# Huzo/Distributed-Machine-Learning-using-CNN-CIFAR-10-dataset-

Measured on AMD Instinct MI355X. Metric: images/sec (whole node) CIFAR-10 CNN training at 1/2/4/8 MI355X, higher is better.
Workload: dtype bf16; 1 GPU; global_batch=256, per_gpu_batch=256, parallelism=dp1, impl=fused+hipgraph, comm_dtype=bf16, graph_warmup_steps=256, steps_per_graph=32

## Files before the change

csrc/bindings/torch_ops.cpp:

```cpp
#include <torch/extension.h>
#include <c10/hip/HIPStream.h>
#include <c10/hip/HIPGuard.h>

#include <vector>

#include "../kernels/api.h"
#include "../kernels/api_comm.h"
#include "check.h"

namespace {

using namespace dmlc_bind;

uint8_t* xraw_ptr(const c10::optional<Tensor>& xraw, int64_t B) {
  if (!xraw.has_value()) return nullptr;
  check(*xraw, "xraw", at::kByte, {B, 3072});
  return xraw->data_ptr<uint8_t>();
}


void conv1_fwd(const Tensor& data, const Tensor& idx, const c10::optional<Tensor>& counter, int64_t period,
               int64_t cy, int64_t cx, const Tensor& w1f, const Tensor& b1, const Tensor& out, const Tensor& am,
               const c10::optional<Tensor>& amax, const c10::optional<Tensor>& xraw) {
  const int64_t B = out.size(0);
// ... 316 lines not shown
      TORCH_CHECK(P.ksplit == 1 && P.nvalid == P.N && P.N % 4 == 0 && P.ldc % 4 == 0 && !P.bias && !P.relu,
                  "gemm ", i, ": the fused SGD epilogue needs ksplit 1, full 16-B rows, no bias / ReLU");
      TORCH_CHECK(!bias.get(i).has_value(), "gemm ", i, ": the fused SGD epilogue takes no bias");
      check_min(*shadow, "shadow", at::kBFloat16, P.s_par + (int64_t)P.M * P.ldc);
      P.S = shadow->data_ptr();
      G.lr0 = (float)sched[0]; G.decay = (float)sched[1]; G.decay_steps = (float)sched[2];
      G.staircase = sched[3] != 0.0; G.warmup = (float)sched[4]; G.grad_scale = (float)sched[5];
    }
    P.A = A[i].data_ptr(); P.B = Bm[i].data_ptr(); P.C = C[i].data_ptr();
    P.bias = nullptr;
    const c10::optional<Tensor> bo = bias.get(i);
    if (bo.has_value()) {
      check_min(*bo, "bias", at::kFloat, P.nvalid);
      P.bias = bo->data_ptr<float>();
    }
  }
  for (int i = 0; i < n; ++i) {
    if (G.p[i].c_mode == 3) { G.p[i].A = A[i].data_ptr(); G.p[i].C = C[i].data_ptr(); G.p[i].bias = nullptr; }
  }
  c10::DeviceGuard guard(A[0].device());
  CHECK_HIP(dmlc_gemm_grouped(&G, stream_of(A[0])));
}

void head(const Tensor& h1part, const Tensor& b1, const Tensor& w2t, const Tensor& b2, const Tensor& w3t,
          const Tensor& b3, const Tensor& w3d, const Tensor& w2d, const Tensor& labels, const Tensor& idx,
          const c10::optional<Tensor>& counter, int64_t period, double inv_batch, bool relu_logits, bool train,
          const Tensor& h1, const Tensor& h2, const Tensor& dl, const Tensor& dh1, const Tensor& dh2,
          const Tensor& loss_part, const Tensor& correct_part, const c10::optional<Tensor>& logits_out,
          int64_t nvalid, const c10::optional<Tensor>& step, const c10::optional<Tensor>& step_copy) {
  TORCH_CHECK(h1part.dim() == 3 && h1part.size(2) == 384, "h1part must be [nsplit,B,384]");
  const int64_t nsplit = h1part.size(0), B = h1part.size(1);
  TORCH_CHECK(B % 16 == 0 && B > 0, "head: batch must be a positive multiple of 16");
  TORCH_CHECK(loss_part.numel() >= 1 && B % loss_part.numel() == 0, "head: loss partials must divide the batch");
  const int64_t rows = B / loss_part.numel();
  TORCH_CHECK(rows == 2 || rows == 4, "head: B / loss_part.numel() (rows per workgroup) must be 2 or 4");
  check(h1part, "h1part", at::kFloat, {nsplit, B, 384});
  check_numel(b1, "b1", at::kFloat, 384);
  check(w2t, "w2t", at::kBFloat16, {192, 384});
  check_numel(b2, "b2", at::kFloat, 192);
  check(w3t, "w3t", at::kBFloat16, {16, 192});
  check_numel(b3, "b3", at::kFloat, 10);
  check(w3d, "w3d", at::kBFloat16, {192, 32});
  check(w2d, "w2d", at::kBFloat16, {384, 192});
  dev(labels, "labels");
  TORCH_CHECK(labels.scalar_type() == at::kInt && labels.dim() == 1, "labels must be int32 [N]");
  check(loss_part, "loss_part", at::kFloat, {B / rows});
  check(correct_part, "correct_part", at::kInt, {B / rows});
  if (train) {
    check(h1, "h1", at::kBFloat16, {B, 384});
    check(h2, "h2", at::kBFloat16, {B, 192});
    check(dl, "dl", at::kBFloat16, {B, 16});
    check(dh1, "dh1", at::kBFloat16, {B, 384});
    check(dh2, "dh2", at::kBFloat16, {B, 192});
  }
  c10::DeviceGuard guard(h1part.device());
  DmlcHeadArgs a;
  a.h1part = h1part.data_ptr<float>(); a.nsplit = (int)nsplit;
  a.b1 = b1.data_ptr<float>(); a.w2t = w2t.data_ptr(); a.b2 = b2.data_ptr<float>();
  a.w3t = w3t.data_ptr(); a.b3 = b3.data_ptr<float>(); a.w3d = w3d.data_ptr(); a.w2d = w2d.data_ptr();
  a.labels = labels.data_ptr<int>(); a.src = index_src(idx, counter, period, B);
  check_order_fits(a.src, labels.size(0));
  if (nvalid < 0) nvalid = B;
  TORCH_CHECK(nvalid >= 1 && nvalid <= B, "head: nvalid must be in [1, B]");
  a.nvalid = (int)nvalid;
  a.B = (int)B; a.rows = (int)rows; a.inv_batch = (float)inv_batch; a.relu_logits = relu_logits; a.train = train;
  a.h1 = train ? h1.data_ptr() : nullptr; a.h2 = train ? h2.data_ptr() : nullptr; a.dl = train ? dl.data_ptr() : nullptr;
  a.dh1 = train ? dh1.data_ptr() : nullptr; a.dh2 = train ? dh2.data_ptr() : nullptr;
  a.loss_part = loss_part.data_ptr<float>(); a.correct_part = correct_part.data_ptr<int>();
  a.logits_out = nullptr;
  if (logits_out.has_value()) {
    check(*logits_out, "logits_out", at::kFloat, {B, 10});
    a.logits_out = logits_out->data_ptr<float>();
  }
  a.step = nullptr; a.step_copy = nullptr;
  TORCH_CHECK(step.has_value() == step_copy.has_value(), "head: step and step_copy go together");
  if (step.has_value()) {
    check_numel(*step, "step", at::kLong, 1);
    check_numel(*step_copy, "step_copy", at::kLong, 1);
    a.step = step->data_ptr<int64_t>(); a.step_copy = step_copy->data_ptr<int64_t>();
  }
  CHECK_HIP(dmlc_head(&a, stream_of(h1part)));
}

void fc_chain(const Tensor& p2, const Tensor& fc1n, const Tensor& h1part, const Tensor& b1, const Tensor& w2t,
              const Tensor& b2, const Tensor& w3t, const Tensor& b3, const Tensor& w3d, const Tensor& labels,
              const Tensor& idx, const c10::optional<Tensor>& counter, int64_t period, double inv_batch,
              bool relu_logits, const Tensor& h1, const Tensor& h2, const Tensor& dl, const Tensor& dh1,
              const Tensor& dh2, const Tensor& loss_part, const Tensor& correct_part, const Tensor& dp2,
              const Tensor& gw1, const Tensor& gw2, const Tensor& gw3, const Tensor& gb1, const Tensor& gb2,
              const Tensor& gb3, bool fuse_sgd, at::ArrayRef<double> sched, int64_t nvalid, const Tensor& step,
              const c10::optional<Tensor>& step_copy, const Tensor& sync, const Tensor& err, bool dw_tasks,
              const c10::optional<Tensor>& am2, const c10::optional<Tensor>& w2d, const c10::optional<Tensor>& dp1,
              const c10::optional<Tensor>& dy2, const c10::optional<Tensor>& fc2n) {
  const int64_t B = p2.size(0);
  TORCH_CHECK(B >= 16 && B <= 256 && B % 16 == 0, "fc_chain: batch must be a multiple of 16 in [16, 256]");
  check(p2, "p2", at::kBFloat16, {B, 2304});
  check(fc1n, "fc1n", at::kBFloat16, {2, 2304, 384});
  check(h1part, "h1part", at::kFloat, {8, B, 384});
  check_numel(b1, "b1", at::kFloat, 384);
  check(w2t, "w2t", at::kBFloat16, {192, 384});
  check_numel(b2, "b2", at::kFloat, 192);
  check(w3t, "w3t", at::kBFloat16, {16, 192});
  check_numel(b3, "b3", at::kFloat, 10);
  check(w3d, "w3d", at::kBFloat16, {192, 32});
  dev(labels, "labels");
  TORCH_CHECK(labels.scalar_type() == at::kInt && labels.dim() == 1, "labels must be int32 [N]");
  check(h1, "h1", at::kBFloat16, {B, 384});
  check(h2, "h2", at::kBFloat16, {B, 192});
  check(dl, "dl", at::kBFloat16, {B, 16});
  check(dh1, "dh1", at::kBFloat16, {B, 384});
  check(dh2, "dh2", at::kBFloat16, {B, 192});
  check(loss_part, "loss_part", at::kFloat, {B / 4});
  check(correct_part, "correct_part", at::kInt, {B / 4});
  check(dp2, "dp2", at::kBFloat16, {B, 2304});
  const bool g16 = gw1.scalar_type() == at::kBFloat16;
  TORCH_CHECK(!g16 || !fuse_sgd, "fc_chain: bf16 gradient views only without the fused SGD");
  const auto gt = g16 ? at::kBFloat16 : at::kFloat;
  check_numel(gw1, "gw1", gt, 2304 * 384);
  check_numel(gw2, "gw2", gt, 384 * 192);
  check_numel(gw3, "gw3", gt, 192 * 10);
  check_numel(gb1, "gb1", gt, 384);
  check_numel(gb2, "gb2", gt, 192);
  check_numel(gb3, "gb3", gt, 10);
  check_numel(step, "step", at::kLong, 1);
  check_min(sync, "sync", at::kInt, 212 * 32);
  check_min(err, "err", at::kInt, 1);
  TORCH_CHECK(sched.size() == 6, "fc_chain: sched = {lr0, decay, decay_steps, staircase, warmup, grad_scale}");
  if (nvalid < 0) nvalid = B;
  TORCH_CHECK(nvalid >= 1 && nvalid <= B, "fc_chain: nvalid must be in [1, B]");
  c10::DeviceGuard guard(p2.device());
  DmlcFcArgs a;
  memset(&a, 0, sizeof(a));
  a.B = (int)B; a.nvalid = (int)nvalid; a.mtiles = (int)((B + 63) / 64);
  a.p2 = p2.data_ptr(); a.w1 = fc1n.data_ptr(); a.h1part = h1part.data_ptr<float>();
  a.b1 = b1.data_ptr<float>(); a.w2t = w2t.data_ptr(); a.b2 = b2.data_ptr<float>();
  a.w3t = w3t.data_ptr(); a.b3 = b3.data_ptr<float>(); a.w3d = w3d.data_ptr();
  a.labels = labels.data_ptr<int>(); a.src = index_src(idx, counter, period, B);
  check_order_fits(a.src, labels.size(0));
  a.inv_batch = (float)inv_batch; a.relu_logits = relu_logits;
  a.h1 = h1.data_ptr(); a.h2 = h2.data_ptr(); a.dl = dl.data_ptr(); a.dh1 = dh1.data_ptr(); a.dh2 = dh2.data_ptr();
  a.loss_part = loss_part.data_ptr<float>(); a.correct_part = correct_part.data_ptr<int>();
  a.dp2 = dp2.data_ptr();
  a.gw1 = (float*)gw1.data_ptr(); a.gw2 = (float*)gw2.data_ptr(); a.gw3 = (float*)gw3.data_ptr();
  a.gb1 = (float*)gb1.data_ptr(); a.gb2 = (float*)gb2.data_ptr(); a.gb3 = (float*)gb3.data_ptr();
  a.grad_bf16 = g16 ? 1 : 0;
  a.fuse_sgd = fuse_sgd ? 1 : 0;
  a.dw_tasks = dw_tasks ? 1 : 0;
  if (fc2n.has_value()) {
    TORCH_CHECK(fuse_sgd && dw_tasks, "fc_chain: the fc SGD in the chain needs fuse_sgd and the dW tiles");
    check(*fc2n, "fc2n", at::kBFloat16, {384, 192});
    a.fuse_sgd = 2;
    a.mw2 = gw2.data_ptr<float>(); a.mw3 = gw3.data_ptr<float>();
    a.mb1 = gb1.data_ptr<float>(); a.mb2 = gb2.data_ptr<float>(); a.mb3 = gb3.data_ptr<float>();
    a.fc2n = fc2n->data_ptr(); a.fc2t = w2t.data_ptr(); a.fc3t = w3t.data_ptr(); a.fc3d = w3d.data_ptr();
  }
  a.lr0 = (float)sched[0]; a.decay = (float)sched[1]; a.decay_steps = (float)sched[2];
  a.staircase = sched[3] != 0.0; a.warmup = (float)sched[4]; a.grad_scale = (float)sched[5];
  a.step = step.data_ptr<int64_t>();
  a.step_copy = nullptr;
  if (step_copy.has_value()) {
    check_numel(*step_copy, "step_copy", at::kLong, 1);
    a.step_copy = step_copy->data_ptr<int64_t>();
  }
  a.sync = reinterpret_cast<unsigned int*>(sync.data_ptr<int>());
  a.err = reinterpret_cast<unsigned int*>(err.data_ptr<int>());
  const bool dg_on = am2.has_value();
  TORCH_CHECK(dg_on == w2d.has_value() && dg_on == dp1.has_value() && dg_on == dy2.has_value(),
              "fc_chain: am2, w2d, dp1, dy2 come together");
  DmlcConv2DgradArgs g;
  memset(&g, 0, sizeof(g));
  if (dg_on) {
    check(*am2, "am2", at::kByte, {B, 6, 6, 64});
    check(*w2d, "w2d", at::kBFloat16, {64, 1600});
    check(*dp1, "dp1", at::kBFloat16, {B, 12, 12, 64});
    check(*dy2, "dy2", at::kBFloat16, {B, 144, 64});
    g.dp2 = dp2.data_ptr(); g.am2 = am2->data_ptr<uint8_t>(); g.wd = w2d->data_ptr();
    g.dp1 = dp1->data_ptr(); g.dy2 = dy2->data_ptr(); g.B = (int)B;
    g.split = B <= 128 ? 1 : 0;
  }
  CHECK_HIP(dmlc_fc_chain(&a, dg_on ? &g : nullptr, stream_of(p2)));
}

static DmlcSgdArgs make_sgd(const Tensor& master, const Tensor& grad, int64_t mode, double grad_scale, at::IntArrayRef off,
         const Tensor& part1, const Tensor& partb1, const Tensor& part2, const Tensor& partb2, const Tensor& w1f,
         const Tensor& w2f, const Tensor& w2d, const Tensor& fc1n, const Tensor& fc2t, const Tensor& fc2n,
         const Tensor& fc3t, const Tensor& fc3d, const Tensor& step, double lr0, double decay, double decay_steps,
         bool staircase, const Tensor& ticket, const Tensor& loss_part, const Tensor& correct_part,
         const Tensor& stats, const c10::optional<Tensor>& w2f8, const c10::optional<Tensor>& amax_w,
         const c10::optional<Tensor>& scale_w, int64_t roles, bool finalize, int64_t batch,
         const c10::optional<Tensor>& bidx, const c10::optional<Tensor>& order, double warmup, bool fc1_fused,
         const c10::optional<Tensor>& step_rd, const c10::optional<Tensor>& xnext,
         const c10::optional<Tensor>& xdata) {
  TORCH_CHECK(roles >= 0 && roles <= 2, "sgd roles must be 0..2");
  TORCH_CHECK(warmup >= 0.0, "sgd: warmup must be >= 0");
  TORCH_CHECK(mode >= 0 && mode <= 3, "sgd mode must be 0..3");
  TORCH_CHECK(off.size() == 10, "off must have 10 entries");
  static const int64_t numel[10] = {4800, 64, 102400, 64, 884736, 384, 73728, 192, 1920, 10};
  for (int i = 0; i < 10; ++i) {
    TORCH_CHECK(off[i] >= 0 && (i == 0 || off[i] >= off[i - 1] + numel[i - 1]), "bad param offsets");
  }
  const int64_t end = off[9] + 10;
  check_min(master, "master", at::kFloat, end);
  const bool g16 = grad.scalar_type() == at::kBFloat16;
  check_min(grad, "grad", g16 ? at::kBFloat16 : at::kFloat, end);
  TORCH_CHECK(!g16 || mode == 1 || mode == 2, "sgd: a bf16 gradient only in modes 1 / 2 (data parallel)");
  const int64_t g1 = part1.size(0), g2 = part2.size(0);
  check(part1, "part1", at::kFloat, {g1, 80, 64});
  check(partb1, "partb1", at::kFloat, {g1, 64});
  check(part2, "part2", at::kFloat, {g2, 1600, 64});
  check(partb2, "partb2", at::kFloat, {g2, 64});
  TORCH_CHECK(loss_part.numel() >= 1, "loss partials missing");
  const int64_t B = batch;
  TORCH_CHECK(B >= 1 && B <= 4 * loss_part.numel(), "sgd: batch (valid rows) exceeds the head's rows");
  check(w1f, "w1f", at::kBFloat16, {64, 96});
  check(w2f, "w2f", at::kBFloat16, {64, 1600});
  check(w2d, "w2d", at::kBFloat16, {64, 1600});
  check(fc1n, "fc1n", at::kBFloat16, {2, 2304, 384});
  TORCH_CHECK(!fc1_fused || mode == 0, "sgd: fc1_fused only in mode 0 (single GPU)");
  check(fc2t, "fc2t", at::kBFloat16, {192, 384});
  check(fc2n, "fc2n", at::kBFloat16, {384, 192});
  check(fc3t, "fc3t", at::kBFloat16, {16, 192});
  check(fc3d, "fc3d", at::kBFloat16, {192, 32});
  check_numel(step, "step", at::kLong, 1);
  check_numel(ticket, "ticket", at::kInt, DMLC_TICKET_WORDS);
  dev(loss_part, "loss_part"); dev(correct_part, "correct_part");
  TORCH_CHECK(loss_part.scalar_type() == at::kFloat && correct_part.scalar_type() == at::kInt &&
                  loss_part.numel() == correct_part.numel(), "loss/correct partials mismatch");
  dev(stats, "stats");
  TORCH_CHECK(stats.scalar_type() == at::kFloat && stats.dim() == 2 && stats.size(1) == 4, "stats must be [R,4] fp32");
  DmlcSgdArgs a;
  a.master = master.data_ptr<float>();
  a.grad = g16 ? nullptr : grad.data_ptr<float>();
  a.grad16 = g16 ? grad.data_ptr() : nullptr;
  a.mode = (int)mode; a.grad_scale = (float)grad_scale;
  for (int i = 0; i < 10; ++i) a.off[i] = (int)off[i];
  a.part1 = part1.data_ptr<float>(); a.partb1 = partb1.data_ptr<float>(); a.g1 = (int)g1;
  a.part2 = part2.data_ptr(); a.g2 = (int)g2;
  a.partb2 = partb2.data_ptr<float>(); a.B = (int)B;
  a.w1f = w1f.data_ptr(); a.w2f = w2f.data_ptr(); a.w2d = w2d.data_ptr(); a.fc1n = fc1n.data_ptr();
  a.fc2t = fc2t.data_ptr(); a.fc2n = fc2n.data_ptr(); a.fc3t = fc3t.data_ptr(); a.fc3d = fc3d.data_ptr();
  a.step = step.data_ptr<int64_t>(); a.lr0 = (float)lr0;
  a.step_rd = a.step;
  if (step_rd.has_value()) {
    check_numel(*step_rd, "step_rd", at::kLong, 1);
    a.step_rd = step_rd->data_ptr<int64_t>();
  } a.decay = (float)decay;
  a.decay_steps = (float)decay_steps; a.staircase = staircase; a.warmup = (float)warmup; a.fc1_fused = fc1_fused ? 1 : 0;
  a.ticket = reinterpret_cast<unsigned int*>(ticket.data_ptr<int>());
  a.loss_part = loss_part.data_ptr<float>(); a.correct_part = correct_part.data_ptr<int>();
  a.nhead = (int)loss_part.numel();
  a.stats = stats.data_ptr<float>(); a.stats_len = (int)stats.size(0);
  a.w2f8 = nullptr; a.w2d8 = nullptr; a.amax_w = nullptr; a.scale_w = nullptr;
  a.roles = (int)roles; a.finalize = finalize ? 1 : 0;
  if (w2f8.has_value()) {
    TORCH_CHECK(amax_w.has_value() && scale_w.has_value(), "fp8 shadow needs amax_w and scale_w");
    if (w2f8->dim() == 3) check(*w2f8, "w2f8", at::kByte, {2, 64, 1600});
    else check(*w2f8, "w2f8", at::kByte, {64, 1600});
    check_numel(*amax_w, "amax_w", at::kFloat, 2 * 400);
    check_numel(*scale_w, "scale_w", at::kFloat, 2);
    a.w2f8 = w2f8->data_ptr<uint8_t>(); a.amax_w = amax_w->data_ptr<float>(); a.scale_w = scale_w->data_ptr<float>();
    if (w2f8->dim() == 3) a.w2d8 = a.w2f8 + 64 * 1600;
  }
  a.bidx = nullptr; a.bidx_n = 0;
  memset(&a.next, 0, sizeof(a.next));
  if (bidx.has_value()) {
    TORCH_CHECK(order.has_value(), "sgd: bidx needs the order descriptor");
    dev(*bidx, "bidx");
    TORCH_CHECK(bidx->scalar_type() == at::kInt && bidx->dim() == 1 && bidx->numel() >= 1 &&
                    bidx->numel() <= 4096, "bidx must be int32 [Bpad <= 4096]");
    TORCH_CHECK(!order->is_cuda() && order->scalar_type() == at::kLong && order->numel() == 6,
                "sgd: order must be the host int64 [6] descriptor");
    const int64_t* d = order->data_ptr<int64_t>();
    TORCH_CHECK(d[2] >= 1 && d[4] >= 1, "sgd: bad order descriptor");
    a.next = index_src(*order, step, d[0] / (d[2] * d[4]), bidx->numel());
    TORCH_CHECK(a.next.idx_base == nullptr, "sgd: order must be the host descriptor");
    a.bidx = bidx->data_ptr<int>(); a.bidx_n = (int)bidx->numel();
  }
  a.xnext = nullptr; a.xdata = nullptr;
  if (xnext.has_value()) {
    TORCH_CHECK(xdata.has_value() && a.bidx, "sgd: xnext needs the dataset and bidx");
    check(*xnext, "xnext", at::kByte, {a.bidx_n, 3072});
    check_data(*xdata);
    TORCH_CHECK(a.next.n <= xdata->size(0), "sgd: the order's rows exceed the dataset");
    a.xnext = xnext->data_ptr<uint8_t>(); a.xdata = xdata->data_ptr<uint8_t>();
  }
  return a;
}

#define DMLC_SGD_PARAMS                                                                                  \
  const Tensor &master, const Tensor &grad, int64_t mode, double grad_scale, at::IntArrayRef off,          \
      const Tensor &part1, const Tensor &partb1, const Tensor &part2, const Tensor &partb2, const Tensor &w1f, \
      const Tensor &w2f, const Tensor &w2d, const Tensor &fc1n, const Tensor &fc2t, const Tensor &fc2n,     \
      const Tensor &fc3t, const Tensor &fc3d, const Tensor &step, double lr0, double decay, double decay_steps, \
      bool staircase, const Tensor &ticket, const Tensor &loss_part, const Tensor &correct_part,            \
      const Tensor &stats, const c10::optional<Tensor> &w2f8, const c10::optional<Tensor> &amax_w,          \
      const c10::optional<Tensor> &scale_w, int64_t roles, bool finalize, int64_t batch,                    \
      const c10::optional<Tensor> &bidx, const c10::optional<Tensor> &order, double warmup, bool fc1_fused,  \
      const c10::optional<Tensor> &step_rd, const c10::optional<Tensor> &xnext, const c10::optional<Tensor> &xdata
#define DMLC_SGD_ARGS                                                                                     \
  master, grad, mode, grad_scale, off, part1, partb1, part2, partb2, w1f, w2f, w2d, fc1n, fc2t, fc2n, fc3t, fc3d, \
      step, lr0, decay, decay_steps, staircase, ticket, loss_part, correct_part, stats, w2f8, amax_w, scale_w,  \
      roles, finalize, batch, bidx, order, warmup, fc1_fused, step_rd, xnext, xdata

void xgmi_allreduce_sgd(int64_t ctx, int64_t blocks, bool bf16_wire, DMLC_SGD_PARAMS) {
  TORCH_CHECK(blocks >= 0 && blocks <= DMLC_XGMI_MAX_BLOCKS, "xgmi_allreduce_sgd: blocks must be in [0,512]");
  TORCH_CHECK(mode == 2 && roles == 0 && finalize && !fc1_fused && !w2f8.has_value() && step_rd.has_value(),
              "xgmi_allreduce_sgd: apply mode (2) over every role, bf16 shadows, the head's step copy");
  DmlcSgdArgs a = make_sgd(DMLC_SGD_ARGS);
  TORCH_CHECK(!a.grad16, "xgmi_allreduce_sgd: the exchange buffer is fp32");
  c10::DeviceGuard guard(master.device());
  CHECK_HIP(dmlc_xgmi_allreduce_sgd((int)ctx, (int)blocks, bf16_wire ? 1 : 0, &a, stream_of(master)));
}

void sgd(DMLC_SGD_PARAMS) {
  DmlcSgdArgs a = make_sgd(DMLC_SGD_ARGS);
  c10::DeviceGuard guard(master.device());
  CHECK_HIP(dmlc_sgd(&a, stream_of(master)));
}

void wgrad_sgd(const Tensor& data, const Tensor& idx, const c10::optional<Tensor>& counter, int64_t period, int64_t cy,
               int64_t cx, const Tensor& dp1, const Tensor& am1, const Tensor& p1, const Tensor& dy2,
               int64_t groups2, const Tensor& xraw, const Tensor& bar, DMLC_SGD_PARAMS,
               const c10::optional<at::TensorList> fc_acts, bool fc_sgd_done, const c10::optional<at::TensorList> fp8) {
  DmlcWgradArgs a = make_wgrad(data, idx, counter, period, cy, cx, dp1, am1, part1, partb1, p1, dy2, part2, partb2,
                               groups2, xraw, fp8);
  TORCH_CHECK((mode == 0 && fc1_fused && step_rd.has_value() && roles == 0 && finalize &&
               grad_scale == 1.0) || (mode == 1 && roles == 0),
              "wgrad_sgd: the single-GPU mode-0 step (fc1 epilogue, the head's step copy) or mode 1 (reduce only)");
  check_numel(bar, "bar", at::kInt, DMLC_WBAR_WORDS);
  a.sgd = make_sgd(DMLC_SGD_ARGS);
  a.apply = 1;
  a.bar = reinterpret_cast<unsigned int*>(bar.data_ptr<int>());
  a.helpers = (a.w1.B > 128 || !fc_acts.has_value()) ? 1 : 0;
  a.fc_in_launch = 0;
  a.fc_done = fc_sgd_done ? 1 : 0;
  TORCH_CHECK(!fc_sgd_done || (mode == 0 && !fc_acts.has_value()), "wgrad_sgd: fc_sgd_done is the chain's mode-0 step");
  memset(&a.fc, 0, sizeof(a.fc));
  if (fc_acts.has_value()) {
    const at::TensorList t = *fc_acts;
    TORCH_CHECK(t.size() == 6 && mode == 0 && fc1_fused, "wgrad_sgd: fc_acts = {p2, h1, h2, dl, dh1, dh2} in mode 0");
    const int64_t B = t[0].size(0);
    TORCH_CHECK(B >= 16 && B <= 256 && B % 16 == 0, "wgrad_sgd: fc tiles need a batch in [16, 256]");
    check(t[0], "p2", at::kBFloat16, {B, 2304});
    check(t[1], "h1", at::kBFloat16, {B, 384});
    check(t[2], "h2", at::kBFloat16, {B, 192});
    check(t[3], "dl", at::kBFloat16, {B, 16});
    check(t[4], "dh1", at::kBFloat16, {B, 384});
    check(t[5], "dh2", at::kBFloat16, {B, 192});
    check(fc2n, "fc2n", at::kBFloat16, {384, 192});
    check(fc2t, "fc2t", at::kBFloat16, {192, 384});
    DmlcFcArgs& f = a.fc;
    f.B = (int)B; f.nvalid = (int)B; f.mtiles = (int)((B + 63) / 64);
    f.p2 = t[0].data_ptr(); f.w1 = fc1n.data_ptr();
    f.h1 = t[1].data_ptr(); f.h2 = t[2].data_ptr(); f.dl = t[3].data_ptr(); f.dh1 = t[4].data_ptr();
    f.dh2 = t[5].data_ptr();
    float* m = master.data_ptr<float>();
    f.gw1 = m + off[4]; f.mb1 = m + off[5]; f.mw2 = m + off[6]; f.mb2 = m + off[7]; f.mw3 = m + off[8];
    f.mb3 = m + off[9];
    f.fc2n = fc2n.data_ptr(); f.fc2t = fc2t.data_ptr(); f.fc3t = fc3t.data_ptr(); f.fc3d = fc3d.data_ptr();
    f.fuse_sgd = 2; f.dw_tasks = 1;
    f.lr0 = (float)lr0; f.decay = (float)decay; f.decay_steps = (float)decay_steps; f.staircase = staircase;
    f.warmup = (float)warmup; f.grad_scale = (float)grad_scale;
    f.err = a.bar + 10 * 32;
    a.fc_in_launch = 1;
  }
  c10::DeviceGuard guard(dp1.device());
  CHECK_HIP(dmlc_wgrad(&a, stream_of(dp1)));
}

}

TORCH_LIBRARY(dmlc, m) {
  m.def("conv1_fwd(Tensor data, Tensor idx, Tensor? counter, int period, int cy, int cx, Tensor w1f, Tensor b1, "
        "Tensor(a!) out, Tensor(b!) am, Tensor(c!)? amax=None, Tensor(d!)? xraw=None) -> ()");
  m.def("conv2_fwd_fp8(Tensor inp, Tensor w8, Tensor b2, Tensor amax_x, Tensor scale_w, Tensor? counter, "
        "Tensor(a!) out, Tensor(b!) am, Tensor(c!)? x8out=None, Tensor(d!)? sx_out=None) -> ()");
  m.def("fp8_roundtrip(Tensor x, Tensor(a!) y, float scale) -> ()");
  m.def("conv2_fwd(Tensor inp, Tensor w2f, Tensor b2, Tensor(a!) out, Tensor(b!) am) -> ()");
  m.def("conv12_fwd(Tensor data, Tensor idx, Tensor? counter, int period, int cy, int cx, Tensor w1f, Tensor b1, "
        "Tensor(a!) p1, Tensor(b!) am1, Tensor w2f, Tensor b2, Tensor(c!) p2, Tensor(d!) am2, "
        "Tensor(e!)? xraw=None, bool xraw_in=False, Tensor(f!)? split_flags=None, Tensor(g!)? err=None) -> ()");
  m.def("conv2_dgrad(Tensor dp2, Tensor am2, Tensor w2d, Tensor(a!) dp1, Tensor(b!) dy2) -> ()");
  m.def("conv1_fwd_split(Tensor data, Tensor idx, Tensor? counter, int period, int cy, int cx, Tensor w1f, Tensor b1, "
        "Tensor(a!) out, Tensor(b!) am, Tensor(c!)? xraw, int nsplit) -> ()");
  m.def("conv2_fwd_split(Tensor inp, Tensor w2f, Tensor b2, Tensor(a!) out, Tensor(b!) am) -> ()");
  m.def("conv2_dgrad_split(Tensor dp2, Tensor am2, Tensor w2d, Tensor(a!) dp1, Tensor(b!) dy2) -> ()");
  m.def("conv2_dgrad_fp8(Tensor dp2, Tensor am2, Tensor w2d8, Tensor scale_w, Tensor(a!) dp1, Tensor(b!) dy2, "
        "Tensor(c!)? dy8out=None, Tensor(d!)? sy_img=None) -> ()");
  m.def("wgrad(Tensor data, Tensor idx, Tensor? counter, int period, int cy, int cx, Tensor dp1, Tensor am1, "
        "Tensor(a!) part1, Tensor(b!) partb1, Tensor p1, Tensor dy2, Tensor(c!) part2, Tensor(d!) partb2, "
        "int groups2, Tensor? xraw=None, Tensor[]? fp8=None) -> ()");
  m.def("gemm_grouped(Tensor[] A, Tensor[] B, Tensor(a!)[] C, Tensor?[] bias, int[] params, Tensor? step=None, "
        "Tensor(b!)? shadow=None, float[] sched=[]) -> ()");
  m.def("head(Tensor h1part, Tensor b1, Tensor w2t, Tensor b2, Tensor w3t, Tensor b3, Tensor w3d, Tensor w2d, "
        "Tensor labels, Tensor idx, Tensor? counter, int period, float inv_batch, bool relu_logits, bool train, "
        "Tensor(a!) h1, Tensor(b!) h2, Tensor(c!) dl, Tensor(d!) dh1, Tensor(e!) dh2, Tensor(f!) loss_part, "
        "Tensor(g!) correct_part, Tensor(h!)? logits_out, int nvalid=-1, Tensor? step=None, Tensor(i!)? step_copy=None) -> ()");
  m.def("fc_chain(Tensor p2, Tensor(a!) fc1n, Tensor(b!) h1part, Tensor b1, Tensor w2t, Tensor b2, Tensor w3t, "
        "Tensor b3, Tensor w3d, Tensor labels, Tensor idx, Tensor? counter, int period, float inv_batch, "
        "bool relu_logits, Tensor(c!) h1, Tensor(d!) h2, Tensor(e!) dl, Tensor(f!) dh1, Tensor(g!) dh2, "
        "Tensor(h!) loss_part, Tensor(i!) correct_part, Tensor(j!) dp2, Tensor(k!) gw1, Tensor(l!) gw2, "
        "Tensor(m!) gw3, Tensor(n!) gb1, Tensor(o!) gb2, Tensor(p!) gb3, bool fuse_sgd, float[] sched, "
        "int nvalid, Tensor step, Tensor(q!)? step_copy, Tensor(r!) sync, Tensor(s!) err, bool dw_tasks=True, "
        "Tensor? am2=None, Tensor? w2d=None, Tensor(t!)? dp1=None, Tensor(u!)? dy2=None, Tensor(v!)? fc2n=None) -> ()");
  m.def("wgrad_sgd(Tensor data, Tensor idx, Tensor? counter, int period, int cy, int cx, Tensor dp1, Tensor am1, "
        "Tensor p1, Tensor dy2, int groups2, Tensor xraw, Tensor(z!) bar, "
        "Tensor(a!) master, Tensor(b!) grad, int mode, float grad_scale, int[] off, Tensor(r!) part1, Tensor(s!) partb1, "
        "Tensor(t!) part2, Tensor(u!) partb2, Tensor(c!) w1f, Tensor(d!) w2f, Tensor(e!) w2d, Tensor(f!) fc1n, "
        "Tensor(g!) fc2t, Tensor(h!) fc2n, Tensor(i!) fc3t, Tensor(j!) fc3d, Tensor(k!) step, float lr0, float decay, "
        "float decay_steps, bool staircase, Tensor(l!) ticket, Tensor loss_part, Tensor correct_part, "
        "Tensor(m!) stats, Tensor(n!)? w2f8, Tensor(o!)? amax_w, Tensor(p!)? scale_w, int roles, "
        "bool finalize, int batch, Tensor(q!)? bidx=None, Tensor? order=None, float warmup=0.0, "
        "bool fc1_fused=False, Tensor? step_rd=None, Tensor(v!)? xnext=None, Tensor? xdata=None, "
        "Tensor[]? fc_acts=None, bool fc_sgd_done=False, Tensor[]? fp8=None) -> ()");
  m.def("sgd(Tensor(a!) master, Tensor(b!) grad, int mode, float grad_scale, int[] off, Tensor part1, Tensor partb1, "
        "Tensor part2, Tensor partb2, Tensor(c!) w1f, Tensor(d!) w2f, Tensor(e!) w2d, Tensor(f!) fc1n, "
        "Tensor(g!) fc2t, Tensor(h!) fc2n, Tensor(i!) fc3t, Tensor(j!) fc3d, Tensor(k!) step, float lr0, float decay, "
        "float decay_steps, bool staircase, Tensor(l!) ticket, Tensor loss_part, Tensor correct_part, "
        "Tensor(m!) stats, Tensor(n!)? w2f8, Tensor(o!)? amax_w, Tensor(p!)? scale_w, int roles, "
        "bool finalize, int batch, Tensor(q!)? bidx=None, Tensor? order=None, float warmup=0.0, "
        "bool fc1_fused=False, Tensor? step_rd=None, Tensor(v!)? xnext=None, Tensor? xdata=None) -> ()");
  m.def("xgmi_allreduce_sgd(int ctx, int blocks, bool bf16_wire, Tensor(a!) master, Tensor(b!) grad, int mode, "
        "float grad_scale, int[] off, Tensor part1, Tensor partb1, "
        "Tensor part2, Tensor partb2, Tensor(c!) w1f, Tensor(d!) w2f, Tensor(e!) w2d, Tensor(f!) fc1n, "
        "Tensor(g!) fc2t, Tensor(h!) fc2n, Tensor(i!) fc3t, Tensor(j!) fc3d, Tensor(k!) step, float lr0, float decay, "
        "float decay_steps, bool staircase, Tensor(l!) ticket, Tensor loss_part, Tensor correct_part, "
        "Tensor(m!) stats, Tensor(n!)? w2f8, Tensor(o!)? amax_w, Tensor(p!)? scale_w, int roles, "
        "bool finalize, int batch, Tensor(q!)? bidx=None, Tensor? order=None, float warmup=0.0, "
        "bool fc1_fused=False, Tensor? step_rd=None, Tensor(v!)? xnext=None, Tensor? xdata=None) -> ()");
}

TORCH_LIBRARY_IMPL(dmlc, CUDA, m) {
  m.impl("conv1_fwd", &conv1_fwd);
  m.impl("conv2_fwd", &conv2_fwd);
  m.impl("conv12_fwd", &conv12_fwd);
  m.impl("conv2_fwd_fp8", &conv2_fwd_fp8);
  m.impl("fp8_roundtrip", &fp8_roundtrip);
  m.impl("conv2_dgrad", &conv2_dgrad);
  m.impl("conv1_fwd_split", &conv1_fwd_split);
  m.impl("conv2_fwd_split", &conv2_fwd_split);
  m.impl("conv2_dgrad_split", &conv2_dgrad_split);
  m.impl("conv2_dgrad_fp8", &conv2_dgrad_fp8);
  m.impl("wgrad", &wgrad);
  m.impl("gemm_grouped", &gemm_grouped);
  m.impl("head", &head);
  m.impl("fc_chain", &fc_chain);
  m.impl("sgd", &sgd);
  m.impl("xgmi_allreduce_sgd", &xgmi_allreduce_sgd);
  m.impl("wgrad_sgd", &wgrad_sgd);
}
```

csrc/kernels/api.h:

```cpp
#pragma once
#include <hip/hip_runtime.h>
#include <stdint.h>

#define DMLC_TICKET_WORDS (9 * 32)

extern "C" {

struct DmlcIndexSrc {
  const int* idx_base;
  const int64_t* counter;
  int period;
  int n, half_bits, world, rank, bvalid;
  uint32_t seed;
};

struct DmlcConv1FwdArgs {
  const uint8_t* data;
  DmlcIndexSrc src;
  int B, cy, cx;
  const void* w;
  const float* bias;
  void* out;
  uint8_t* am;
  float* amax;
// ... 117 lines not shown
  int B, nvalid, mtiles;
  const void* p2;
  void* w1;
  float* h1part;
  const float* b1;
  const void* w2t; const float* b2;
  const void* w3t; const float* b3;
  const void* w3d;
  const int* labels;
  DmlcIndexSrc src;
  float inv_batch; int relu_logits;
  void* h1; void* h2; void* dl; void* dh1; void* dh2;
  float* loss_part; int* correct_part;
  void* dp2;
  float* gw1;
  float* gw2; float* gw3; float* gb1; float* gb2; float* gb3;
  int fuse_sgd;
  float* mw2; float* mw3; float* mb1; float* mb2; float* mb3;
  void* fc2n; void* fc2t; void* fc3t; void* fc3d;
  int dw_tasks;
  float lr0, decay, decay_steps, warmup, grad_scale; int staircase;
  const int64_t* step; int64_t* step_copy;
  unsigned int* sync;
  unsigned int* err;
  int grad_bf16;
};

struct DmlcSgdArgs {
  float* master;
  float* grad;
  int mode;
  float grad_scale;
  int off[10];
  const float* part1; const float* partb1; int g1;
  const void* part2; int g2;
  const float* partb2; int B;
  void* w1f; void* w2f; void* w2d; void* fc1n; void* fc2t; void* fc2n; void* fc3t; void* fc3d;
  int64_t* step; float lr0; float decay; float decay_steps; int staircase;
  const int64_t* step_rd;
  float warmup;
  unsigned int* ticket;
  const float* loss_part; const int* correct_part; int nhead;
  float* stats; int stats_len;
  int nblocks;
  uint8_t* w2f8; float* amax_w; float* scale_w;
  uint8_t* w2d8;
  int roles;
  int finalize;
  int* bidx; int bidx_n;
  DmlcIndexSrc next;
  int fc1_fused;
  uint8_t* xnext; const uint8_t* xdata;
  void* grad16;
};

#define DMLC_WBAR_WORDS (20 * 32)
struct DmlcWgradArgs {
  DmlcConv1WgradArgs w1;
  DmlcConv2WgradArgs w2;
  int apply;
  unsigned int* bar;
  int helpers;
  DmlcSgdArgs sgd;
  int fc_in_launch;
  DmlcFcArgs fc;
  int fc_done;
};

hipError_t dmlc_conv1_fwd(const DmlcConv1FwdArgs* a, hipStream_t s);
hipError_t dmlc_conv2_fwd(const DmlcConv2FwdArgs* a, hipStream_t s);
hipError_t dmlc_conv12_fwd(const DmlcConv1FwdArgs* a1, const DmlcConv2FwdArgs* a2, hipStream_t s);
hipError_t dmlc_conv1_fwd_split(const DmlcConv1FwdArgs* a, int nsplit, hipStream_t s);
hipError_t dmlc_conv12_fwd_split(const DmlcConv1FwdArgs* a1, const DmlcConv2FwdArgs* a2, unsigned* flags,
                                 unsigned* err, hipStream_t s);
hipError_t dmlc_conv2_fwd_split(const DmlcConv2FwdArgs* a, hipStream_t s);
hipError_t dmlc_conv2_dgrad_split(const DmlcConv2DgradArgs* a, hipStream_t s);
hipError_t dmlc_conv2_fwd_fp8(const DmlcConv2FwdFp8Args* a, hipStream_t s);
hipError_t dmlc_conv2_dgrad_fp8(const DmlcConv2DgradFp8Args* a, hipStream_t s);
hipError_t dmlc_fp8_roundtrip(const float* x, float* y, int n, float scale, hipStream_t s);
hipError_t dmlc_conv2_dgrad(const DmlcConv2DgradArgs* a, hipStream_t s);
hipError_t dmlc_wgrad(const DmlcWgradArgs* a, hipStream_t s);
hipError_t dmlc_gemm_grouped(DmlcGemmGroup* g, hipStream_t s);
hipError_t dmlc_fc_chain(const DmlcFcArgs* a, const DmlcConv2DgradArgs* dg, hipStream_t s);
hipError_t dmlc_head(const DmlcHeadArgs* a, hipStream_t s);
hipError_t dmlc_sgd(DmlcSgdArgs* a, hipStream_t s);

}
```

csrc/kernels/cnn_fc.hip:

```cpp
#include <string.h>

#include "fc_common.h"
#include "conv2_core.h"
#include "split_common.h"

namespace dmlc {

constexpr int W2_LD = 384, H1_LD = 392, H2_LD = 200, DL_LD = 40;
DEV int w2swz(int row, int col) {
  return row * W2_LD + (((col >> 3) ^ (2 * (row & 3) + 8 * ((row >> 3) & 1))) << 3) + (col & 7);
}
struct HL {
  static constexpr int W2 = 0;
  static constexpr int H1 = W2 + 192 * W2_LD * 2;
  static constexpr int H2 = H1 + (FC_RB + 1) * H1_LD * 2;
  static constexpr int DH2 = H2 + (FC_RB + 1) * H2_LD * 2;
  static constexpr int DL = DH2 + (FC_RB + 1) * H2_LD * 2;
  static constexpr int LG = DL + (FC_RB + 1) * DL_LD * 2;
  static constexpr int BYTES = LG + 16 * 17 * 4;
};
constexpr int FC_LDS = L_DP2_END > HL::BYTES ? L_DP2_END : HL::BYTES;
static_assert(FC_LDS <= 160 * 1024, "fc chain LDS exceeds a CU");
constexpr int FC_LDS_ALL = FC_LDS > (int)DG_LDS ? FC_LDS : (int)DG_LDS;
static_assert(FT == NT && FC_LDS_ALL <= 160 * 1024, "the dgrad runs in the chain's workgroups");
static_assert(FT == SP_NT && SP_LDS <= (size_t)FC_LDS_ALL, "... and so does the split dgrad");
static_assert(L_FWD_B + FC_KS * 64 * 2 <= FC_LDS && L_RED + 8 * 64 * 4 <= FC_LDS, "task images");

struct FwdRegs { uint4 a[5], b[5]; };
DEV void fwd_issue(const DmlcFcArgs& a, int t, bool has, int parity, FwdRegs& R, int tid) {
  const int s = t % FC_S, nt = (t / FC_S) % 6, mt = t / (6 * FC_S);
  const bf16* W1 = W1S(a) + (parity ? 884736 : 0);
  const int k0 = s * FC_KS;
#pragma unroll
  for (int i = 0; i < 5; ++i) {
    const int c = tid + i * FT;
    const int ra = c / 36, ka = c - ra * 36;
    const int rowa = 64 * mt + ra;
    const bool oka = has && c < 64 * 36 && rowa < a.B;
    R.a[i] = load_sel(reinterpret_cast<const uint4*>(P2(a) + (size_t)rowa * 2304 + k0 + 8 * ka),
                      reinterpret_cast<const uint4*>(P2(a)), oka);
    const int kb = c >> 3, cb = c & 7;
    const bool okb = has && c < FC_KS * 8;
    R.b[i] = load_sel(reinterpret_cast<const uint4*>(W1 + (size_t)(k0 + kb) * 384 + 64 * nt + 8 * cb),
                      reinterpret_cast<const uint4*>(W1), okb);
  }
}
DEV void fwd_task(const DmlcFcArgs& a, int t, const FwdRegs& R, char* smem, int tid) {
  bf16* sa = reinterpret_cast<bf16*>(smem + L_FWD_A);
  bf16* sb = reinterpret_cast<bf16*>(smem + L_FWD_B);
  const int s = t % FC_S, nt = (t / FC_S) % 6, mt = t / (6 * FC_S);
#pragma unroll
  for (int i = 0; i < 5; ++i) {
    const int c = tid + i * FT;
    if (c < 64 * 36) {
      const int ra = c / 36, ka = c - ra * 36;
      *reinterpret_cast<uint4*>(sa + ra * KST_A + 8 * ka) = R.a[i];
    }
    if (c < FC_KS * 8) *reinterpret_cast<uint4*>(sb + mz(c >> 3, 8 * (c & 7))) = R.b[i];
  }
  __syncthreads();
  const int w = wave_id(), lane = tid & 63, g = lane >> 4, li = lane & 15;
  const int h = w >> 2, wm = (w >> 1) & 1, wn = w & 1;
  Acc acc;
  acc.zero();
  const int kb = h ? 5 : 0, ke = h ? 9 : 5;
  for (int kk = kb; kk < ke; ++kk)
    acc.mma(kfrag(sa, KST_A, 32 * wm, kk, g, li), kfrag(sa, KST_A, 32 * wm + 16, kk, g, li),
            mfrag(sb, 32 * wn, kk, g, li), mfrag(sb, 32 * wn + 16, kk, g, li));
  __syncthreads();
  float* ct = reinterpret_cast<float*>(smem);
  if (h == 1) acc.to_lds(ct, CT_LD, 32 * wm, 32 * wn, g, li);
  __syncthreads();
  if (h == 0) acc.add_lds(ct, CT_LD, 32 * wm, 32 * wn, g, li);
  __syncthreads();
  const rsrc_t out = buf_rsrc(a.h1part);
#pragma unroll
  for (int u = 0; u < 2; ++u) {
    const int e = tid + u * FT, rr = e >> 4, cc = (e & 15) * 4;
    const int row = 64 * mt + rr;
    if (row < a.B) {
      const f32x4 v = *reinterpret_cast<const f32x4*>(ct + rr * CT_LD + cc);
      st_sc1(out, (uint32_t)(((size_t)s * a.B + row) * 384 + 64 * nt + cc) * 4, v);
    }
  }
  publish(cntA(a, mt, nt));
}

DEV bf16x4 relu_mask4(const f32x4& acc, const bf16x4& h) {
  return pack4((float)h[0] > 0.f ? acc[0] : 0.f, (float)h[1] > 0.f ? acc[1] : 0.f,
               (float)h[2] > 0.f ? acc[2] : 0.f, (float)h[3] > 0.f ? acc[3] : 0.f);
}

DEV void head_task(const DmlcFcArgs& a, int hb, char* smem, int tid) {
  bf16* w2s = reinterpret_cast<bf16*>(smem + HL::W2);
  bf16* h1s = reinterpret_cast<bf16*>(smem + HL::H1);
  bf16* h2s = reinterpret_cast<bf16*>(smem + HL::H2);
  bf16* dh2s = reinterpret_cast<bf16*>(smem + HL::DH2);
  bf16* dls = reinterpret_cast<bf16*>(smem + HL::DL);
  const int lane = tid & 63, w = wave_id(), g = lane >> 4, li = lane & 15, q = li >> 2, p = li & 3;
  constexpr int RB = FC_RB;
  const int r0 = hb * RB, mt = r0 >> 6;
  const bool rv = li < RB;
  const int rr = rv ? li : RB;
  DMLC_STAMP(DMLC_TK_HEAD, 0);
  DMLC_STAMP(DMLC_TK_CONV2_FWD, 0);

  int label = 0;
  if (w == 7 && lane < RB) label = a.labels[batch_index(a.src, a.B, r0 + lane)];
  {
    constexpr int WCH = 192 * 48 / FT;
    uint4 wv[WCH];
#pragma unroll
    for (int i = 0; i < WCH; ++i) wv[i] = *(reinterpret_cast<const uint4*>(a.w2t) + tid + i * FT);
#pragma unroll
    for (int i = 0; i < WCH; ++i) {
      const int c = tid + i * FT, n2 = c / 48, k8 = c - n2 * 48;
      *reinterpret_cast<uint4*>(w2s + w2swz(n2, k8 * 8)) = wv[i];
    }
  }
  float4 b2v[2];
  bf16x8 w3d[2];
#pragma unroll
  for (int j = 0; j < 2; ++j) {
    const int nt = w + 8 * j;
    const bool ok = nt < 12;
    b2v[j] = ok ? *reinterpret_cast<const float4*>(a.b2 + 16 * nt + 4 * g) : make_float4(0.f, 0.f, 0.f, 0.f);
    w3d[j] = ok ? glb_b128(reinterpret_cast<const bf16*>(a.w3d) + (16 * nt + li) * 32 + 8 * g) : bf16x8{};
  }
  bf16x8 w3f[6];
  float b3v[4] = {0.f, 0.f, 0.f, 0.f};
  if (w == 7) {
    const bf16* W = reinterpret_cast<const bf16*>(a.w3t) + li * 192 + 8 * g;
#pragma unroll
    for (int ks = 0; ks < 6; ++ks) w3f[ks] = glb_b128(W + ks * 32);
#pragma unroll
    for (int i = 0; i < 4; ++i) b3v[i] = load_sel(a.b3 + 4 * g + i, a.b3, 4 * g + i < 10);
  }
  const bool act = tid < RB * 96;
  const int ec = act ? tid : 0, r = ec / 96, n = (ec - r * 96) * 4;
  const float4 b1v = *reinterpret_cast<const float4*>(a.b1 + n);
  if (tid < 96) *reinterpret_cast<bf16x4*>(h1s + RB * H1_LD + tid * 4) = pack4(0.f, 0.f, 0.f, 0.f);
  else if (tid < 144) *reinterpret_cast<bf16x4*>(h2s + RB * H2_LD + (tid - 96) * 4) = pack4(0.f, 0.f, 0.f, 0.f);
  else if (tid < 192) *reinterpret_cast<bf16x4*>(dh2s + RB * H2_LD + (tid - 144) * 4) = pack4(0.f, 0.f, 0.f, 0.f);
  else if (tid < 200) *reinterpret_cast<bf16x4*>(dls + RB * DL_LD + (tid - 192) * 4) = pack4(0.f, 0.f, 0.f, 0.f);
  else if (tid < 200 + 2 * RB)
    *reinterpret_cast<uint4*>(dls + ((tid - 200) >> 1) * DL_LD + 16 + 8 * ((tid - 200) & 1)) = make_uint4(0, 0, 0, 0);

  DMLC_STAMP(DMLC_TK_HEAD, 1);
  consume(seamA(a, mt), a.err);
  DMLC_STAMP(DMLC_TK_HEAD, 2);
  {
    const rsrc_t part = buf_rsrc(a.h1part);
    float4 v[FC_S];
#pragma unroll
    for (int s = 0; s < FC_S; ++s)
      v[s] = ld_sc1(part, (uint32_t)(((size_t)s * a.B + r0 + r) * 384 + n) * 4);
    float4 acc = b1v;
#pragma unroll
    for (int s = 0; s < FC_S; ++s) { acc.x += v[s].x; acc.y += v[s].y; acc.z += v[s].z; acc.w += v[s].w; }
    if (act)
      *reinterpret_cast<bf16x4*>(h1s + r * H1_LD + n) =
          pack4(fmaxf(acc.x, 0.f), fmaxf(acc.y, 0.f), fmaxf(acc.z, 0.f), fmaxf(acc.w, 0.f));
  }
  lds_barrier();
  DMLC_STAMP(DMLC_TK_HEAD, 3);

#pragma unroll
  for (int j = 0; j < 2; ++j) {
    const int nt = w + 8 * j;
    if (nt >= 12) break;
    f32x4 acc = zero4();
#pragma unroll
    for (int ks = 0; ks < 12; ++ks)
      acc = mfma16(lds_b128(w2s + w2swz(16 * nt + li, 8 * g + 32 * ks)), lds_b128(h1s + rr * H1_LD + ks * 32 + 8 * g), acc);
    const float4 bb = b2v[j];
    const bf16x4 o = pack4(fmaxf(acc[0] + bb.x, 0.f), fmaxf(acc[1] + bb.y, 0.f), fmaxf(acc[2] + bb.z, 0.f),
                           fmaxf(acc[3] + bb.w, 0.f));
    if (rv) *reinterpret_cast<bf16x4*>(h2s + li * H2_LD + 16 * nt + 4 * g) = o;
  }
  lds_barrier();

  DMLC_STAMP(DMLC_TK_CONV2_FWD, 1);
  if (w == 7) {
    f32x4 acc = zero4();
#pragma unroll
    for (int ks = 0; ks < 6; ++ks) acc = mfma16(w3f[ks], lds_b128(h2s + rr * H2_LD + ks * 32 + 8 * g), acc);
    float v[4];
    float m = -INFINITY;
    int am = 16;
#pragma unroll
    for (int i = 0; i < 4; ++i) {
      v[i] = acc[i] + b3v[i];
      if (a.relu_logits) v[i] = fmaxf(v[i], 0.f);
      if (4 * g + i < 10 && v[i] > m) { m = v[i]; am = 4 * g + i; }
    }
#pragma unroll
    for (int o = 16; o <= 32; o <<= 1) {
      const float m2 = __shfl_xor(m, o);
      const int a2 = __shfl_xor(am, o);
      if (m2 > m || (m2 == m && a2 < am)) { m = m2; am = a2; }
    }
    float se = 0.f;
#pragma unroll
    for (int i = 0; i < 4; ++i) se += 4 * g + i < 10 ? __expf(v[i] - m) : 0.f;
    se += __shfl_xor(se, 16);
    se += __shfl_xor(se, 32);
    const float lse = m + __logf(se);
    const int lab = __shfl(label, li);
    const bool rowok = li < RB;
    const float vr = rowok && r0 + li < a.nvalid ? 1.f : 0.f;
    float loss = 0.f;
#pragma unroll
    for (int i = 0; i < 4; ++i) if (4 * g + i == lab) loss = vr * (lse - v[i]);
    const float corr = g == 0 ? vr * (am == lab ? 1.f : 0.f) : 0.f;
    if (rowok) {
      bf16x4 d4;
#pragma unroll
      for (int i = 0; i < 4; ++i) {
        const int c = 4 * g + i;
        float d = 0.f;
        if (c < 10) {
          d = (__expf(v[i] - lse) - (c == lab ? 1.f : 0.f)) * a.inv_batch * vr;
          if (a.relu_logits && !(v[i] > 0.f)) d = 0.f;
        }
        d4[i] = (bf16)d;
      }
      *reinterpret_cast<bf16x4*>(dls + li * DL_LD + 4 * g) = d4;
    }
    const float ls = wave_sum(rowok ? loss : 0.f), cs = wave_sum(corr);
    if (lane == 0) {
      a.loss_part[hb] = ls;
      a.correct_part[hb] = (int)(cs + 0.5f);
    }
  }
  lds_barrier();

  DMLC_STAMP(DMLC_TK_CONV2_FWD, 2);
#pragma unroll
  for (int j = 0; j < 2; ++j) {
    const int nt = w + 8 * j;
    if (nt >= 12) break;
    const f32x4 acc = mfma16(w3d[j], lds_b128(dls + rr * DL_LD + 8 * g), zero4());
    const int nn = 16 * nt + 4 * g;
    const bf16x4 o = relu_mask4(acc, *reinterpret_cast<const bf16x4*>(h2s + rr * H2_LD + nn));
    if (rv) *reinterpret_cast<bf16x4*>(dh2s + li * H2_LD + nn) = o;
  }
  lds_barrier();

  DMLC_STAMP(DMLC_TK_CONV2_FWD, 3);
  f32x4 dacc[3];
  bf16x4 hm[3];
#pragma unroll
  for (int j = 0; j < 3; ++j) {
    const int k0 = 16 * (w + 8 * j);
    f32x4 acc = zero4();
#pragma unroll
    for (int ks = 0; ks < 6; ++ks) {
      const bf16x8 af = tr_frag(w2s + w2swz(32 * ks + 8 * g + q, k0 + 4 * p), w2s + w2swz(32 * ks + 8 * g + 4 + q, k0 + 4 * p));
      acc = mfma16(af, lds_b128(dh2s + rr * H2_LD + ks * 32 + 8 * g), acc);
    }
    dacc[j] = acc;
    hm[j] = *reinterpret_cast<const bf16x4*>(h1s + rr * H1_LD + k0 + 4 * g);
  }
  __syncthreads();
  bf16* d1 = reinterpret_cast<bf16*>(smem + HL::W2);
#pragma unroll
  for (int j = 0; j < 3; ++j) {
    const int k0 = 16 * (w + 8 * j);
    if (rv) *reinterpret_cast<bf16x4*>(d1 + li * 384 + k0 + 4 * g) = relu_mask4(dacc[j], hm[j]);
  }
  lds_barrier();
  DMLC_STAMP(DMLC_TK_HEAD, 4);

  const rsrc_t rh1 = buf_rsrc(a.h1), rh2 = buf_rsrc(a.h2), rdh2 = buf_rsrc(a.dh2), rdl = buf_rsrc(a.dl),
               rdh1 = buf_rsrc(a.dh1);
  for (int c = tid; c < RB * 146; c += FT) {
    const int rw = c / 146, qq = c - rw * 146, b = r0 + rw;
    if (qq < 48) st16(rh1, (uint32_t)(b * 384 + 8 * qq) * 2, *reinterpret_cast<const uint4*>(h1s + rw * H1_LD + 8 * qq));
    else if (qq < 72) st16(rh2, (uint32_t)(b * 192 + 8 * (qq - 48)) * 2, *reinterpret_cast<const uint4*>(h2s + rw * H2_LD + 8 * (qq - 48)));
    else if (qq < 96) st16(rdh2, (uint32_t)(b * 192 + 8 * (qq - 72)) * 2, *reinterpret_cast<const uint4*>(dh2s + rw * H2_LD + 8 * (qq - 72)));
    else if (qq < 98) st16(rdl, (uint32_t)(b * 16 + 8 * (qq - 96)) * 2, *reinterpret_cast<const uint4*>(dls + rw * DL_LD + 8 * (qq - 96)));
    else st16(rdh1, (uint32_t)(b * 384 + 8 * (qq - 98)) * 2, *reinterpret_cast<const uint4*>(d1 + rw * 384 + 8 * (qq - 98)));
  }
  publish(cntB(a, mt, hb & 3));
  DMLC_STAMP(DMLC_TK_HEAD, 5);
}


#ifdef DMLC_EAGER_ARGS
#define late_fc() a
#define late_dg() dg
#else
#define late_fc() late_kernarg<DmlcFcArgs>(0)
#define late_dg() late_kernarg<DmlcConv2DgradArgs>(kernarg_second<DmlcFcArgs, DmlcConv2DgradArgs>())
#endif
__global__ __launch_bounds__(FT, 1) void k_fc_chain(DmlcFcArgs a, DmlcConv2DgradArgs dg) {
  extern __shared__ __attribute__((aligned(16))) char smem[];
  const int tid = threadIdx.x, blk = blockIdx.x;
  const int H = a.B / FC_RB;
  const int64_t step = a.step ? *a.step : 0;
  const int parity = (int)(step & 1);
  if (blk == 0 && tid == 0 && a.step_copy) *a.step_copy = step;
  __shared__ unsigned s_epoch;
  unsigned e0 = 0;
  if (tid == 0) e0 = ld_relaxed(epochW(a));
  if (blk < H) {
    head_task(a, blk, smem, tid);
    if (tid == 0) s_epoch = e0;
    const DmlcFcArgs& L = late_fc();
    const int G = FC_BLOCKS - H, nc = ctask_count(L);
    for (int t = G + blk; t < nc; t += H) {
      __syncthreads();
      PreRegs R;
      const CTask T = ctask(L, t);
      pre_issue(L, T, parity, R, tid);
      pre_store(L, T, R, smem, tid);
      c_task(L, T, R, step, smem, tid, s_epoch);
    }
    DMLC_STAMP(DMLC_TK_HEAD, 6);
  } else {
    DMLC_STAMP(DMLC_TK_GEMM, 0);
    const int j = blk - H;
    const int na = a.mtiles * 6 * FC_S;
    const bool has_a = j < na;
    if (has_a) {
      FwdRegs F;
      fwd_issue(a, j, true, parity, F, tid);
      fwd_task(a, j, F, smem, tid);
    }
    if (tid == 0) s_epoch = e0;
    DMLC_STAMP(DMLC_TK_GEMM, 1);
    const DmlcFcArgs& L = late_fc();
    const CTask T = ctask(L, j);
    if (T.kind >= 0) {
      PreRegs R;
      pre_issue(L, T, parity, R, tid);
      __syncthreads();
      pre_store(L, T, R, smem, tid);
      DMLC_STAMP(DMLC_TK_GEMM, 2);
      c_task(L, T, R, step, smem, tid, s_epoch);
      DMLC_STAMP(DMLC_TK_GEMM, 5);
    }
  }
  __syncthreads();
  const unsigned epoch = s_epoch;
  const DmlcFcArgs& L = late_fc();
  if (tid == 0) {
    wait_vm_all();
    if (last_arrival(L.sync + 32 * 10, blk, FC_BLOCKS)) {
      for (int w = SY_A; w < SY_D; ++w)
        __hip_atomic_store(L.sync + 32 * w, 0u, __ATOMIC_RELAXED, __HIP_MEMORY_SCOPE_AGENT);
      for (int k = 0; k < 72; ++k)
        __hip_atomic_store(cntD(L, epoch + 1, 0, 0) + 32 * k, 0u, __ATOMIC_RELAXED, __HIP_MEMORY_SCOPE_AGENT);
      __hip_atomic_store(epochW(L), epoch + 1, __ATOMIC_RELAXED, __HIP_MEMORY_SCOPE_AGENT);
    }
  }
  const DmlcConv2DgradArgs& D = late_dg();
  if (D.split) {
    if (blk < 2 * D.B) {
      int b, h;
      split_index<2>(blk, b, h);
      conv2_dgrad_split_image<true>(D, b, h, smem, seamD(L, epoch, b >> 6), L.err);
    }
  } else if (blk < D.B) {
    conv2_dgrad_image<true>(D, blk, smem, seamD(L, epoch, blk >> 6), L.err);
  }
  if (blk < H) DMLC_STAMP(DMLC_TK_HEAD, 7);
  else DMLC_STAMP(DMLC_TK_GEMM, 6);
}

}

using namespace dmlc;

extern "C" hipError_t dmlc_fc_chain(const DmlcFcArgs* a, const DmlcConv2DgradArgs* dg, hipStream_t s) {
  if (a->B < 16 || a->B > 256 || a->B % 16 != 0 || a->mtiles != (a->B + 63) / 64 || !a->sync || !a->err)
    return hipErrorInvalidValue;
  DmlcConv2DgradArgs d;
  memset(&d, 0, sizeof(d));
  if (dg) {
    if (dg->B != a->B || dg->dp2 != a->dp2 || !dg->am2 || !dg->wd || !dg->dp1 || !dg->dy2) return hipErrorInvalidValue;
    if (dg->split && (2 * dg->B > FC_BLOCKS || dg->B % 8)) return hipErrorInvalidValue;
    d = *dg;
  }
  static int cus = 0;
  if (!cus) {
    int dev = 0;
    if (hipGetDevice(&dev) != hipSuccess || hipDeviceGetAttribute(&cus, hipDeviceAttributeMultiprocessorCount, dev) != hipSuccess)
      return hipErrorInvalidValue;
  }
  if (cus < FC_BLOCKS) return hipErrorInvalidValue;
  DMLC_LDS_OPTIN(&k_fc_chain, FC_LDS_ALL);
  hipLaunchKernelGGL(k_fc_chain, dim3(FC_BLOCKS), dim3(FT), d.B ? FC_LDS_ALL : FC_LDS, s, *a, d);
  return hipGetLastError();
}
```

csrc/kernels/cnn_wgrad.hip:

```cpp
#include "w1_common.h"
#include "sgd_common.h"
#include "fc_common.h"

namespace dmlc {

constexpr size_t W1_LDS = (size_t)(W1_DYT + W1_XS + 9216) * 2 + 3072 + 9216;
static_assert(W1_FL_BYTES <= (W1_DYT + W1_XS) * 2, "flush buffer over dY1 + planes");

DEV void conv1_wgrad_block(const DmlcConv1WgradArgs& a, const int grp, char* smem, bool coh = false) {
  bf16* dyt = reinterpret_cast<bf16*>(smem);
  bf16* xs = dyt + W1_DYT;
  bf16* dps = xs + W1_XS;
  uint8_t* img = reinterpret_cast<uint8_t*>(dps + 9216);
  uint8_t* ams = img + 3072;
  const int tid = threadIdx.x, lane = tid & 63, w = wave_id();
  const int g = lane >> 4, li = lane & 15;
  const int ch = w & 1, ks = w >> 1;
  const int G = a.g1, b0 = grp, last = grp < a.B ? grp + (a.B - 1 - grp) / G * G : grp;
  DMLC_STAMP(DMLC_TK_W1, 0);

  w1_ones_plane15(xs, tid);

  f32x4 acc[2][5];
#pragma unroll
  for (int h = 0; h < 2; ++h)
#pragma unroll
    for (int t = 0; t < 5; ++t) acc[h][t] = zero4();

  const int cI = tid % 192, cD2 = 1024 + (tid & 127), cA1 = 512 + (tid & 63);
  uint4 vI, vD0, vD1, vD2, vA0, vA1;
  auto load = [&](int idx, int bb) {
    const uint4* si = reinterpret_cast<const uint4*>(a.xraw ? a.xraw + (size_t)bb * 3072 : a.data + (size_t)idx * 3072);
    const uint4* sd = reinterpret_cast<const uint4*>(reinterpret_cast<const bf16*>(a.dp1) + (size_t)bb * 9216);
    const uint4* sa = reinterpret_cast<const uint4*>(a.am1 + (size_t)bb * 9216);
    vI = si[cI];
    vD0 = sd[tid]; vD1 = sd[tid + 512]; vD2 = sd[cD2];
    vA0 = sa[tid]; vA1 = sa[cA1];
  };
  auto row_index = [&](int bb) { return a.xraw ? 0 : batch_index(a.src, a.B, bb); };
  load(row_index(b0 < last ? b0 : last), b0 < last ? b0 : last);
  int nidx = row_index(b0 + G < last ? b0 + G : last);
  for (int b = b0; b < a.B; b += G) {
    lds_barrier();
    reinterpret_cast<uint4*>(img)[cI] = vI;
    reinterpret_cast<uint4*>(dps)[tid] = vD0;
    reinterpret_cast<uint4*>(dps)[tid + 512] = vD1;
    reinterpret_cast<uint4*>(dps)[cD2] = vD2;
    reinterpret_cast<uint4*>(ams)[tid] = vA0;
    reinterpret_cast<uint4*>(ams)[cA1] = vA1;
    w1_zero_dy(dyt, tid);
    load(nidx, b + G < last ? b + G : last);
    nidx = row_index(b + 2 * G < last ? b + 2 * G : last);
    lds_barrier();
    if (b == b0) DMLC_STAMP(DMLC_TK_W1, 1);
    if (b == b0 + G) DMLC_STAMP(DMLC_TK_W1, 6);
    w1_planes(xs, img, a.cy, a.cx, tid);
    w1_pool_bwd(dyt, dps, ams, w, lane);
    if (b == b0) DMLC_STAMP(DMLC_TK_W1, 2);
    if (b == b0 + G) DMLC_STAMP(DMLC_TK_W1, 7);
    w1_mfma(dyt, xs, acc, ks, ch, g, li);
    if (b == b0) DMLC_STAMP(DMLC_TK_W1, 5);
  }
  __syncthreads();
  DMLC_STAMP(DMLC_TK_W1, 3);
  w1_flush(smem, acc, a.part1 + (size_t)grp * 80 * 64, a.partb1 + grp * 64, ks, ch, lane, tid, coh);
  DMLC_STAMP(DMLC_TK_W1, 4);
}

constexpr int W2T = 512;
constexpr int W2_LD = 64;
DEV int w2_dy_col(int row, int col) { return col ^ (16 * (((row >> 1) & 1) | ((row >> 2) & 2))); }
constexpr int W2_DY = 160 * W2_LD;
constexpr int W2_LDX = 16;
constexpr int W2_XT = 256 * W2_LDX;
constexpr int W2_ST = 68;
constexpr size_t W2_LDS_MAIN = (size_t)(W2_XT + W2_DY) * 2;
constexpr size_t W2_LDS_ST = (size_t)(W2T / 64) * 16 * W2_ST * 4;
constexpr size_t W2_LDS = W2_LDS_MAIN > W2_LDS_ST ? W2_LDS_MAIN : W2_LDS_ST;

DEV void w2_block_pos(const DmlcConv2WgradArgs& a, int blk, int base, int& c4, int& grp) {
  const bool xcd = a.g2 % 8 == 0 && base % 8 == 0;
  c4 = xcd ? (blk >> 3) & 3 : blk & 3;
  grp = xcd ? (blk & 7) + 8 * (blk >> 5) : blk >> 2;
}

typedef int w8x32 __attribute__((ext_vector_type(8)));
typedef int w8x2 __attribute__((ext_vector_type(2)));
constexpr int W8_XROWS = 272;
constexpr int W8_XIMG = W8_XROWS * 16;
constexpr int W8_YIMG = 192 * 64;
constexpr int W8_XU = 2 * W8_XIMG, W8_BUF = 2 * (W8_XIMG + W8_YIMG);
constexpr size_t W8_LDS = 2 * (size_t)W8_BUF + 64 * 4;
DEV int w8_ychunk(int r, int ct) { return ct ^ (((r >> 2) & 1) | (((r >> 3) & 1) << 1)); }
DEV w8x2 tr8(const uint8_t* p) { return __builtin_amdgcn_ds_read_tr8_b64_v2i32((LDS_AS w8x2*)(p)); }
DEV f32x4 mfma8(const w8x32& a, const w8x32& b, const f32x4& c, int sb) {
  return __builtin_amdgcn_mfma_scale_f32_16x16x128_f8f6f4(a, b, c, 0, 0, 0, 127, 0, sb);
}

DEV void w2_fp8_main(const DmlcConv2WgradArgs& a, int c4, int grp, char* smem, f32x4 (&acc)[13], float (&bsum)[8]) {
  uint8_t* lds = reinterpret_cast<uint8_t*>(smem);
  float* btile = reinterpret_cast<float*>(smem + 2 * W8_BUF);
  const int tid = threadIdx.x, lane = tid & 63, w = wave_id();
  const int g = lane >> 4, q = (lane & 15) >> 1, p = lane & 1, half = (lane >> 4) & 1;
  const int G = a.g2, nimg = grp < a.B ? (a.B - 1 - grp) / G + 1 : 0, nunits = (nimg + 1) >> 1;
  const bool bias = c4 == 0 && w >= 4;
  for (int i = tid; i < 2 * W8_BUF / 16; i += W2T) reinterpret_cast<uint4*>(lds)[i] = make_uint4(0u, 0u, 0u, 0u);

  uint4 vx, vy[3];
  float syv[2];
  int ey[2];
  auto img_of = [&](int u, int i) { return grp + G * (2 * u + i); };
  auto load = [&](int u, uint4& vx, uint4 (&vy)[3], float (&syv)[2]) __attribute__((always_inline)) {
#pragma unroll
    for (int i = 0; i < 2; ++i) {
      const int b = img_of(u, i);
      syv[i] = load_sel(a.sy_img + b, a.sy_img, b < a.B);
    }
    {
      const int i = tid >= 144, px = tid - 144 * i, b = img_of(u, i);
      vx = load_sel(reinterpret_cast<const uint4*>(a.x8 + ((size_t)b * 144 + px) * 64 + 16 * c4),
                    reinterpret_cast<const uint4*>(a.x8), tid < 288 && b < a.B);
    }
#pragma unroll
    for (int m = 0; m < 3; ++m) {
      const int s = tid + 512 * m, i = s >= 576, k = s - 576 * i, b = img_of(u, i);
// ... 3 lines not shown
  };
  auto store = [&](int buf, const uint4& vx, const uint4 (&vy)[3]) __attribute__((always_inline)) {
    uint8_t* X8 = lds + buf * W8_BUF;
    uint8_t* Y8 = X8 + W8_XU;
    if (tid < 288) {
      const int i = tid >= 144, px = tid - 144 * i, y = px / 12, x = px - 12 * y;
      *reinterpret_cast<uint4*>(X8 + i * W8_XIMG + ((y + 2) * 16 + x + 2) * 16) = vx;
    }
#pragma unroll
    for (int m = 0; m < 3; ++m) {
      if (m == 2 && tid >= 128) break;
      const int s = tid + 512 * m, i = s >= 576, k = s - 576 * i, px = k >> 2, y = px / 12, x = px - 12 * y;
      const int r = i * 192 + y * 16 + x;
      *reinterpret_cast<uint4*>(Y8 + r * 64 + 16 * w8_ychunk(r, k & 3)) = vy[m];
    }
  };
  auto scales = [&](const float (&syv)[2]) __attribute__((always_inline)) {
#pragma unroll
    for (int i = 0; i < 2; ++i) ey[i] = syv[i] > 0.f ? 127 - (int)log2f(syv[i]) : 127;
  };
  const int f = ((q >> 2) & 1) | ((g & 1) << 1);
  const int yl = (8 * g + q) * 64 + 8 * p, xl = (8 * g + q) * 16 + 8 * p;
  int xt[4];
#pragma unroll
  for (int t = 0; t < 3; ++t) xt[t] = xl + ((3 * w + t) / 5 * 16 + (3 * w + t) % 5) * 16;
  xt[3] = xl + (4 * 16 + 4) * 16;
  const w8x32 ones = {0x38383838, 0x38383838, 0x38383838, 0x38383838,
                      0x38383838, 0x38383838, 0x38383838, 0x38383838};
  f32x4 accb = zero4();
  __syncthreads();
  if (nunits > 0) load(0, vx, vy, syv);
  for (int u = 0; u < nunits; ++u) {
    const int buf = u & 1;
    store(buf, vx, vy);
    scales(syv);
    if (u + 1 < nunits) load(u + 1, vx, vy, syv);
    lds_barrier();
    if (u == 0) DMLC_STAMP(DMLC_TK_W2, 1);
    const uint8_t* Y8 = lds + buf * W8_BUF + W8_XU + yl;
    const uint8_t* X8 = lds + buf * W8_BUF;
#pragma unroll
    for (int c = 0; c < 3; ++c) {
      w8x32 bf[4], af[4];
#pragma unroll
      for (int j = 0; j < 4; ++j) {
        const int img = c == 2 || (c == 1 && j >= 2);
#pragma unroll
        for (int ct = 0; ct < 4; ++ct) {
          const w8x2 v = tr8(Y8 + 16 * (ct ^ f) + c * 8192 + j * 2048);
          bf[ct][2 * j] = v.x; bf[ct][2 * j + 1] = v.y;
        }
#pragma unroll
        for (int t = 0; t < 4; ++t) {
          if (t == 3 && w >= 4) break;
          const w8x2 v = tr8(X8 + xt[t] + c * 2048 + j * 512 + img * (W8_XIMG - 192 * 16));
          af[t][2 * j] = v.x; af[t][2 * j + 1] = v.y;
        }
      }
      const int sb = c == 0 ? ey[0] : c == 2 ? ey[1] : lane >= 32 ? ey[1] : ey[0];
#pragma unroll
      for (int t = 0; t < 3; ++t)
#pragma unroll
        for (int ct = 0; ct < 4; ++ct) acc[4 * t + ct] = mfma8(af[t], bf[ct], acc[4 * t + ct], sb);
      if (w < 4) {
        const w8x32 bw = w == 0 ? bf[0] : w == 1 ? bf[1] : w == 2 ? bf[2] : bf[3];
        acc[12] = mfma8(af[3], bw, acc[12], sb);
      } else if (bias) {
        const w8x32 bw = w == 4 ? bf[0] : w == 5 ? bf[1] : w == 6 ? bf[2] : bf[3];
        accb = mfma8(ones, bw, accb, sb);
      }
    }
    if (u == 0) DMLC_STAMP(DMLC_TK_W2, 4);
  }
  const float inv = 1.f / a.sx[0];
#pragma unroll
  for (int j = 0; j < 13; ++j) acc[j] *= inv;
  __syncthreads();
  if (bias && lane < 16) btile[16 * (w - 4) + lane] = accb[0];
  __syncthreads();
#pragma unroll
  for (int j = 0; j < 8; ++j) bsum[j] = c4 == 0 && tid < 8 ? btile[8 * tid + j] : 0.f;
}

DEV void conv2_wgrad_block(const DmlcConv2WgradArgs& a, const int blk, const int base, char* smem, bool coh = false) {
  bf16* xt = reinterpret_cast<bf16*>(smem);
  bf16* dyt = xt + W2_XT;
  const int tid = threadIdx.x, lane = tid & 63, w = wave_id();
  const int g = lane >> 4, li = lane & 15, q = li >> 2, p = li & 3;
  int c4, grp;
  w2_block_pos(a, blk, base, c4, grp);
  const int G = a.g2, b0 = grp, last = grp < a.B ? grp + (a.B - 1 - grp) / G * G : grp;
  DMLC_STAMP(DMLC_TK_W2, 0);

  f32x4 acc[13];
#pragma unroll
  for (int j = 0; j < 13; ++j) acc[j] = zero4();
  float bsum[8] = {0.f, 0.f, 0.f, 0.f, 0.f, 0.f, 0.f, 0.f};
  if (a.x8) {
    w2_fp8_main(a, c4, grp, smem, acc, bsum);
  } else {
  *reinterpret_cast<bf16x8*>(xt + tid * 8) = bf16x8{};
  if (tid < 128) *reinterpret_cast<bf16x8*>(dyt + (144 + (tid >> 3)) * W2_LD + (tid & 7) * 8) = bf16x8{};

  const int kx = tid % 288, pxl = kx >> 1, xy = pxl / 12;
  bf16* xdst = xt + ((xy + 2) * 16 + pxl - xy * 12 + 2) * W2_LDX + 8 * (kx & 1);
  const int kd[3] = {tid, tid + 512, 1024 + (tid & 127)};
  uint4 vx, vd[3];
  auto load = [&](int b) {
    const uint4* x = reinterpret_cast<const uint4*>(reinterpret_cast<const bf16*>(a.p1) + (size_t)b * 9216);
    const uint4* d = reinterpret_cast<const uint4*>(reinterpret_cast<const bf16*>(a.dy2) + (size_t)b * 9216);
    vx = x[pxl * 8 + 2 * c4 + (kx & 1)];
#pragma unroll
    for (int i = 0; i < 3; ++i) vd[i] = d[kd[i]];
  };

  int xa[5], xb[5];
#pragma unroll
  for (int s = 0; s < 5; ++s) {
    const int cA = min(32 * s + 8 * g + q, 143), cB = min(32 * s + 8 * g + q + 4, 143);
    xa[s] = ((cA / 12) * 16 + cA % 12) * W2_LDX + 4 * p;
    xb[s] = ((cB / 12) * 16 + cB % 12) * W2_LDX + 4 * p;
  }
  int toff[3];
#pragma unroll
  for (int j = 0; j < 3; ++j) toff[j] = ((3 * w + j) / 5 * 16 + (3 * w + j) % 5) * W2_LDX;
  constexpr int T24 = (4 * 16 + 4) * W2_LDX;

  load(b0 < last ? b0 : last);
  for (int b = b0; b < a.B; b += G) {
    lds_barrier();
    *reinterpret_cast<uint4*>(xdst) = vx;
#pragma unroll
    for (int i = 0; i < 3; ++i) {
      const int k = kd[i];
      *reinterpret_cast<uint4*>(dyt + (k >> 3) * W2_LD + w2_dy_col(k >> 3, (k & 7) * 8)) = vd[i];
      if (c4 == 0 && (i < 2 || tid < 128)) {
        const uint32_t d4[4] = {vd[i].x, vd[i].y, vd[i].z, vd[i].w};
#pragma unroll
        for (int j = 0; j < 4; ++j) { bsum[2 * j] += bf16_lo(d4[j]); bsum[2 * j + 1] += bf16_hi(d4[j]); }
      }
    }
    load(b + G < last ? b + G : last);
    lds_barrier();
    if (b == b0) DMLC_STAMP(DMLC_TK_W2, 1);
    bf16x8 BF[2][4], AF[2][4];
    auto frags = [&](int s, bf16x8 (&bf)[4], bf16x8 (&af)[4]) __attribute__((always_inline)) {
      const int rA = 32 * s + 8 * g + q, rB = rA + 4;
#pragma unroll
      for (int ct = 0; ct < 4; ++ct)
        bf[ct] = tr_frag(dyt + rA * W2_LD + w2_dy_col(rA, 16 * ct + 4 * p), dyt + rB * W2_LD + w2_dy_col(rB, 16 * ct + 4 * p));
#pragma unroll
      for (int j = 0; j < 3; ++j) af[j] = tr_frag(xt + xa[s] + toff[j], xt + xb[s] + toff[j]);
      if (w < 4) af[3] = tr_frag(xt + xa[s] + T24, xt + xb[s] + T24);
    };
    frags(0, BF[0], AF[0]);
#pragma unroll
    for (int s = 0; s < 5; ++s) {
      const int cur = s & 1;
      wait_lds();
      __builtin_amdgcn_sched_barrier(0);
      if (s + 1 < 5) frags(s + 1, BF[cur ^ 1], AF[cur ^ 1]);
      __builtin_amdgcn_sched_barrier(0);
#pragma unroll
      for (int j = 0; j < 3; ++j)
#pragma unroll
        for (int ct = 0; ct < 4; ++ct) acc[4 * j + ct] = mfma16(AF[cur][j], BF[cur][ct], acc[4 * j + ct]);
      if (w < 4) {
        const bf16x8 bw = w == 0 ? BF[cur][0] : w == 1 ? BF[cur][1] : w == 2 ? BF[cur][2] : BF[cur][3];
        acc[12] = mfma16(AF[cur][3], bw, acc[12]);
      }
      __builtin_amdgcn_sched_barrier(0);
    }
    if (b == b0) DMLC_STAMP(DMLC_TK_W2, 4);
  }
  }
  DMLC_STAMP(DMLC_TK_W2, 2);
  const size_t slab0 = (size_t)grp * 1600 * 64;
  auto put4 = [&](size_t e, const f32x4& v) {
    if (coh) st_sc1(buf_rsrc(a.part2), (uint32_t)(slab0 + e) * 4, v);
    else st_maybe_nt<kNtDefault>(reinterpret_cast<f32x4*>(reinterpret_cast<float*>(a.part2) + slab0 + e), v);
  };
  auto put1 = [&](size_t e, float v) {
    if (coh) st_sc1(buf_rsrc(a.part2), (uint32_t)(slab0 + e) * 4, v);
    else reinterpret_cast<float*>(a.part2)[slab0 + e] = v;
  };
  __syncthreads();
  if (c4 == 0) {
    float* red = reinterpret_cast<float*>(smem);
    block_chunk_sum(bsum, red, tid);
    __syncthreads();
    if (tid < 64) {
      float sb = 0.f;
#pragma unroll
      for (int k = 0; k < W2T / 64; ++k) sb += red[k * 64 + tid];
      if (coh) st_sc1(buf_rsrc(a.partb2), (uint32_t)(grp * 64 + tid) * 4, sb);
      else a.partb2[grp * 64 + tid] = sb;
    }
    __syncthreads();
  }
  DMLC_STAMP(DMLC_TK_W2, 5);
  float* st = reinterpret_cast<float*>(smem) + w * 16 * W2_ST;
#pragma unroll
  for (int j = 0; j < 3; ++j) {
#pragma unroll
    for (int ct = 0; ct < 4; ++ct)
#pragma unroll
      for (int i = 0; i < 4; ++i) st[(4 * g + i) * W2_ST + 16 * ct + li] = acc[4 * j + ct][i];
    lds_barrier();
#pragma unroll
    for (int k = 0; k < 4; ++k) {
      const int row = 4 * k + (lane >> 4), c16 = lane & 15;
      const f32x4 v = *reinterpret_cast<const f32x4*>(st + row * W2_ST + 4 * c16);
// ... 10 lines not shown

DEV unsigned* wbar(unsigned* b, int k) { return b + 32 * k; }

struct W2Fp8 { float sw; int nxt, slot; float* red; };
DEV float w2_fp8_scale(const DmlcSgdArgs& s, int64_t step) {
  const float* src = s.amax_w + (size_t)(step & 1) * C2_BLOCKS;
  float m = 0.f;
  for (int i = threadIdx.x & 63; i < C2_BLOCKS; i += 64) m = fmaxf(m, src[i]);
#pragma unroll
  for (int o = 32; o > 0; o >>= 1) m = fmaxf(m, __shfl_xor(m, o));
  return 224.f / fmaxf(m, 1e-20f);
}
DEV void w2_fp8_put(const DmlcWgradArgs& A, int slot, int nxt, float m, float* red) {
#pragma unroll
  for (int o = 32; o > 0; o >>= 1) m = fmaxf(m, __shfl_xor(m, o));
  if ((threadIdx.x & 63) == 0) red[threadIdx.x >> 6] = m;
  __syncthreads();
  if (threadIdx.x == 0) {
    float t = red[0];
    for (int k = 1; k < W2T / 64; ++k) t = fmaxf(t, red[k]);
    A.sgd.amax_w[(size_t)nxt * C2_BLOCKS + slot] = t;
  }
  __syncthreads();
}

DEV void conv2_reduce(const DmlcWgradArgs& A, int c4, int f_begin, int f_end, float lr, const W2Fp8& f8) {
  const DmlcSgdArgs& s = A.sgd;
  const int tid = threadIdx.x, sp = tid & 3, n = A.w2.g2;
  float wmax = 0.f;
  const rsrc_t part = buf_rsrc(A.w2.part2);
  for (int f0 = f_begin; f0 < f_end; f0 += W2T / 4) {
    const int f = f0 + (tid >> 2);
    const bool ok = f < f_end;
    const int fc = ok ? f : f_begin;
    const int krow = (fc >> 8) * 64 + 16 * c4 + ((fc >> 4) & 15), co = 4 * (fc & 15);
    const size_t e = (size_t)krow * 64 + co;
    const float4 w0 = *reinterpret_cast<const float4*>(s.master + s.off[2] + e);
    float4 acc = make_float4(0.f, 0.f, 0.f, 0.f);
    for (int q = sp; q < n; q += 8 * C2_SPLIT) {
      float4 v[8];
#pragma unroll
      for (int u = 0; u < 8; ++u)
        v[u] = ld_sc1(part, (uint32_t)((size_t)(q + u * C2_SPLIT < n ? q + u * C2_SPLIT : 0) * 102400 + e) * 4);
#pragma unroll
      for (int u = 0; u < 8; ++u) acc = add4(acc, q + u * C2_SPLIT < n ? v[u] : make_float4(0.f, 0.f, 0.f, 0.f));
    }
    float4 o[3];
#pragma unroll
    for (int j = 0; j < 3; ++j)
      o[j] = make_float4(__shfl_down(acc.x, j + 1), __shfl_down(acc.y, j + 1), __shfl_down(acc.z, j + 1),
                         __shfl_down(acc.w, j + 1));
    if (sp == 0 && ok) {
      const float4 t = add4(add4(add4(acc, o[0]), o[1]), o[2]);
      if (s.mode == 1) {
        grad_st4(s, s.off[2] + e, t);
      } else {
        const float4 w = sgd4(s.master + s.off[2] + e, w0, t, lr, s.grad_scale, true);
        conv2_shadow4(s, krow, co, w);
        if (s.w2f8) {
          const float sw = f8.sw;
          const uint32_t q = pk_fp8x4(w.x * sw, w.y * sw, w.z * sw, w.w * sw);
          uint8_t* w8 = s.w2f8 + krow;
          w8[(co + 0) * 1600] = (uint8_t)q; w8[(co + 1) * 1600] = (uint8_t)(q >> 8);
          w8[(co + 2) * 1600] = (uint8_t)(q >> 16); w8[(co + 3) * 1600] = (uint8_t)(q >> 24);
          if (s.w2d8)
            *reinterpret_cast<uint32_t*>(s.w2d8 + (size_t)(krow & 63) * 1600 + (24 - (krow >> 6)) * 64 + co) = q;
          wmax = fmaxf(wmax, fmaxf(fmaxf(fabsf(w.x), fabsf(w.y)), fmaxf(fabsf(w.z), fabsf(w.w))));
        }
      }
    }
  }
  if (s.w2f8 && s.mode == 0) w2_fp8_put(A, f8.slot, f8.nxt, wmax, f8.red);
}

DEV bool w2_helpers(const DmlcWgradArgs& A) { return A.helpers && A.w1.g1 >= 4 * A.w2.g2; }
DEV void w2_chunk(const DmlcWgradArgs& A, int grp, int& b, int& m, int& e) {
  const int per = (6400 + A.w2.g2 - 1) / A.w2.g2;
  b = grp * per;
  e = min(b + per, 6400);
  m = w2_helpers(A) ? min(b + (per + 1) / 2, e) : e;
}
DEV unsigned* w2_claim(const DmlcWgradArgs& A, int c4, int grp) { return A.bar + 11 * 32 + c4 * A.w2.g2 + grp; }

DEV void conv2_apply(const DmlcWgradArgs& A, int c4, int grp, char* smem, unsigned g0, int64_t step) {
  const DmlcSgdArgs& s = A.sgd;
  const int tid = threadIdx.x, n = A.w2.g2;
  int* flag = reinterpret_cast<int*>(smem);
  wait_vm_all();
  __syncthreads();
  if (tid == 0) {
    bar_arrive(wbar(A.bar, 2 + c4), wbar(A.bar, 6 + c4), g0, (unsigned)n);
    bar_wait(wbar(A.bar, 6 + c4), g0, wbar(A.bar, 10));
  }
  __syncthreads();
  DMLC_STAMP(DMLC_TK_W2, 6);
  const float lr = lr_of(s, step);
  int b, m, e;
  w2_chunk(A, grp, b, m, e);
  const int slot = 2 * (c4 * n + grp), nxt = (int)((step & 1) ^ 1);
  W2Fp8 f8 = {s.w2f8 ? w2_fp8_scale(s, step) : 0.f, nxt, slot, reinterpret_cast<float*>(smem + 64)};
  if (s.w2f8 && s.mode == 0 && c4 == 0 && grp == 0) {
    for (int i = 8 * n + tid; i < C2_BLOCKS; i += W2T) s.amax_w[(size_t)nxt * C2_BLOCKS + i] = 0.f;
    if (tid == 0) { s.scale_w[0] = f8.sw; s.scale_w[1] = f8.sw; }
  }
  conv2_reduce(A, c4, b, m, lr, f8);
  if (m < e) {
    if (tid == 0)
      flag[0] = __hip_atomic_fetch_max(w2_claim(A, c4, grp), g0 + 1u, __ATOMIC_RELAXED, __HIP_MEMORY_SCOPE_AGENT) < g0 + 1u;
    __syncthreads();
    f8.slot = slot + 1;
    if (flag[0]) DMLC_STAMP(DMLC_TK_HEAD, 6);
    if (flag[0]) conv2_reduce(A, c4, m, e, lr, f8);
    __syncthreads();
  } else if (s.w2f8 && s.mode == 0 && tid == 0) {
    s.amax_w[(size_t)nxt * C2_BLOCKS + slot + 1] = 0.f;
  }
  if (c4 == 0 && grp == 0) conv_bias(s, 1, lr, reinterpret_cast<float4*>(smem), tid, true);
  DMLC_STAMP(DMLC_TK_W2, 7);
}

DEV void conv2_help(const DmlcWgradArgs& A, int j, char* smem, unsigned hg0, int64_t step) {
  int c4, grp;
  w2_block_pos(A.w2, j, A.w1.g1, c4, grp);
  int* flag = reinterpret_cast<int*>(smem);
  __syncthreads();
  if (threadIdx.x == 0) {
    unsigned gen = hg0;
    for (int it = 0; it < 64 && (gen = bar_gen(wbar(A.bar, 6 + c4))) == hg0; ++it) __builtin_amdgcn_s_sleep(2);
    flag[0] = gen != hg0 &&
              __hip_atomic_fetch_max(w2_claim(A, c4, grp), gen, __ATOMIC_RELAXED, __HIP_MEMORY_SCOPE_AGENT) < gen;
  }
  __syncthreads();
  if (flag[0]) {
    DMLC_STAMP(DMLC_TK_SGD, 5);
    int b, m, e;
    w2_chunk(A, grp, b, m, e);
    const W2Fp8 f8 = {A.sgd.w2f8 ? w2_fp8_scale(A.sgd, step) : 0.f, (int)((step & 1) ^ 1),
                      2 * (c4 * A.w2.g2 + grp) + 1, reinterpret_cast<float*>(smem + 64)};
    conv2_reduce(A, c4, m, e, lr_of(A.sgd, step), f8);
  }
}

DEV void conv1_arrive(const DmlcWgradArgs& A, unsigned g0) {
  wait_vm_all();
  __syncthreads();
  if (threadIdx.x == 0) bar_arrive(wbar(A.bar, 0), wbar(A.bar, 1), g0, (unsigned)A.w1.g1);
}
DEV void conv1_apply(const DmlcWgradArgs& A, int grp, char* smem, unsigned g0, int64_t step, bool arrived = false) {
  const DmlcSgdArgs& s = A.sgd;
  const int tid = threadIdx.x, n = A.w1.g1;
  float4* lds = reinterpret_cast<float4*>(smem);
  if (!arrived) conv1_arrive(A, g0);
  else __syncthreads();
  const float lr = lr_of(s, step);
  const int nfc = s.mode == 1 || A.fc_in_launch || A.fc_done ? 0 : fc_role_count(s);
  for (int r = grp; r < nfc; r += n) {
    fc_role(s, r, lr, step, lds, tid);
    lds_barrier();
  }
  if (s.mode == 0 && grp == 0 && tid < 64) publish_step(s, step, lr, tid);
  if (s.mode == 0 && s.bidx) {
    const int r = grp * W1T + tid;
    if (r < s.bidx_n) s.bidx[r] = order_row(s.next, step + 1, r);
  }
  DMLC_STAMP(DMLC_TK_SGD, 0);
  if (tid == 0) bar_wait(wbar(A.bar, 1), g0, wbar(A.bar, 10));
  __syncthreads();
  DMLC_STAMP(DMLC_TK_SGD, 1);
  const int per = (1200 + n - 1) / n, ol = tid & 15, sp = tid >> 4;
  const rsrc_t part1 = buf_rsrc(A.w1.part1);
  for (int f0 = 0; f0 < per; f0 += 16) {
    const int oo = f0 + ol, o = grp * per + oo;
    const bool ok = oo < per && o < 1200;
    const int oc = ok ? o : 0, row = oc >> 4, co = 4 * (oc & 15);
    const int ci = row % 3, khw = row / 3, kh = khw / 5, kw = khw - kh * 5;
    const uint32_t p = (uint32_t)(kh * 16 + kw * 3 + ci) * 64 + co;
    const size_t e = (size_t)row * 64 + co;
    const float4 w0 = *reinterpret_cast<const float4*>(s.master + s.off[0] + e);
    float4 acc = make_float4(0.f, 0.f, 0.f, 0.f);
    for (int q = sp; q < n; q += C1_LOADS * C1_SPLIT) {
      float4 v[C1_LOADS];
#pragma unroll
      for (int u = 0; u < C1_LOADS; ++u)
        v[u] = ld_sc1(part1, (p + (uint32_t)(q + u * C1_SPLIT < n ? q + u * C1_SPLIT : 0) * 80 * 64) * 4);
#pragma unroll
      for (int u = 0; u < C1_LOADS; ++u) acc = add4(acc, q + u * C1_SPLIT < n ? v[u] : make_float4(0.f, 0.f, 0.f, 0.f));
    }
    lds[tid] = acc;
    lds_barrier();
    if (tid < 16 && ok) {
      float4 t = lds[ol];
#pragma unroll
      for (int k = 1; k < C1_SPLIT; ++k) t = add4(t, lds[k * 16 + ol]);
      if (s.mode == 1) grad_st4(s, s.off[0] + e, t);
      else conv1_shadow4(s, row, co, sgd4(s.master + s.off[0] + e, w0, t, lr, s.grad_scale, true));
    }
    lds_barrier();
  }
#ifndef DMLC_C1_BIAS_ON_1
  if (grp == n - 1) conv_bias(s, 0, lr, lds, tid, true);
#else
  if (grp == (n > 1 ? 1 : 0)) conv_bias(s, 0, lr, lds, tid, true);
#endif
  DMLC_STAMP(DMLC_TK_SGD, 2);
}

#ifdef DMLC_EAGER_ARGS
#define late_args() a
#else
#define late_args() late_kernarg<DmlcWgradArgs>(0)
#endif

constexpr size_t WG_LDS = W1_LDS > W2_LDS ? W1_LDS : W2_LDS;
static_assert(WG_LDS >= W8_LDS, "the fp8 conv2 body's double buffer fits the launch's LDS");
static_assert(WG_LDS >= (size_t)L_RED + 8 * 64 * 4 && WG_LDS >= 40960 + 64 * 136 * 2,
              "the fc dW tiles reuse the weight-gradient launch's LDS");
static_assert(W1T == FT, "the fc dW tiles run with the weight-gradient launch's block size");
static_assert(WG_LDS >= SGD_LDS4 * 16, "apply mode reuses the block's LDS for the SGD roles");
__global__ __launch_bounds__(W1T, 1) void k_wgrad(DmlcWgradArgs a) {
  extern __shared__ __attribute__((aligned(16))) char smem[];
  const bool conv1 = (int)blockIdx.x < a.w1.g1;
  int c4 = 0, grp = 0;
  if (!conv1) w2_block_pos(a.w2, blockIdx.x - a.w1.g1, a.w1.g1, c4, grp);
  unsigned g0 = 0, hg0 = 0;
  int64_t step = 0;
  const bool helper = a.apply && conv1 && w2_helpers(a) && (int)blockIdx.x < 4 * a.w2.g2;
  if (a.apply) {
    if (threadIdx.x == 0) g0 = bar_gen(wbar(a.bar, conv1 ? 1 : 6 + c4));
    if (helper && threadIdx.x == 0) {
      int hc4, hgrp;
      w2_block_pos(a.w2, blockIdx.x, a.w1.g1, hc4, hgrp);
      hg0 = bar_gen(wbar(a.bar, 6 + hc4));
    }
    step = *a.sgd.step_rd;
  }
  if (conv1) {
    conv1_wgrad_block(a.w1, blockIdx.x, smem, a.apply != 0);
    const DmlcWgradArgs& L = late_args();
    if (a.apply && L.fc_in_launch) {
      const int parity = (int)(step & 1);
      if (blockIdx.x >= FC_DW_TASKS) conv1_arrive(L, g0);
      for (int d = blockIdx.x; d < FC_DW_TASKS; d += L.w1.g1) {
        const CTask T = dw_ctask(d);
        PreRegs R;
        pre_issue(L.fc, T, parity, R, threadIdx.x);
        const bool first = d == (int)blockIdx.x;
        dw_task<false>(L.fc, T, R, step, smem, threadIdx.x, [&]() {
          if (first) conv1_arrive(L, g0);
        });
      }
      DMLC_STAMP(DMLC_TK_SGD, 3);
      conv1_apply(L, blockIdx.x, smem, g0, step, true);
    } else if (a.apply) {
      conv1_apply(L, blockIdx.x, smem, g0, step);
    }
    if (helper) conv2_help(L, blockIdx.x, smem, hg0, step);
    if (a.apply && L.sgd.mode == 0 && L.sgd.xnext)
      for (int r = blockIdx.x; r < L.sgd.bidx_n; r += L.w1.g1) copy_next_row(L.sgd, step, r, threadIdx.x);
    DMLC_STAMP(DMLC_TK_SGD, 4);
  } else {
    conv2_wgrad_block(a.w2, blockIdx.x - a.w1.g1, a.w1.g1, smem, a.apply != 0);
    if (a.apply) conv2_apply(late_args(), c4, grp, smem, g0, step);
  }
}
static_assert(W1T == W2T, "k_wgrad runs both bodies with one block size");

}

using namespace dmlc;

extern "C" {

hipError_t dmlc_wgrad(const DmlcWgradArgs* a, hipStream_t s) {
  DMLC_LDS_OPTIN(&k_wgrad, WG_LDS);
  const int blocks = a->w1.g1 + 4 * a->w2.g2;
  if (a->apply) {
    static int cus = 0;
    if (!cus) {
      int dev = 0;
      if (hipGetDevice(&dev) != hipSuccess || hipDeviceGetAttribute(&cus, hipDeviceAttributeMultiprocessorCount, dev) != hipSuccess)
        return hipErrorInvalidValue;
    }
    const DmlcSgdArgs& g = a->sgd;
    const bool ok_mode = g.mode == 0 ? (g.step_rd != g.step && g.fc1_fused && (!g.w2f8 || (g.amax_w && g.scale_w) ) &&
                                        8 * a->w2.g2 <= 400)
                                     : g.mode == 1;
    if (a->fc_in_launch && (g.mode != 0 || !g.fc1_fused || a->fc.fuse_sgd != 2 || a->fc.B < 16 || a->fc.B > 256 ||
                            !a->fc.p2 || !a->fc.dh1 || !a->fc.mw2 || !a->fc.fc2t))
      return hipErrorInvalidValue;
    if (a->w1.g1 < 1 || a->w1.g1 > cus || 4 * a->w2.g2 > cus || !a->bar || !a->w1.xraw ||
        !ok_mode || g.part1 != a->w1.part1 ||
        g.part2 != a->w2.part2 || g.g1 != a->w1.g1 || g.g2 != a->w2.g2 || g.bidx_n > a->w1.g1 * W1T)
      return hipErrorInvalidValue;
  }
  hipLaunchKernelGGL(k_wgrad, dim3(blocks), dim3(W1T), WG_LDS, s, *a);
  return hipGetLastError();
}

}
```

csrc/kernels/common.h:

```cpp
#pragma once
#include <hip/hip_runtime.h>
#include <stdint.h>

namespace dmlc {

typedef __bf16 bf16;
typedef __bf16 bf16x8 __attribute__((ext_vector_type(8)));
typedef __bf16 bf16x4 __attribute__((ext_vector_type(4)));
typedef short s16x4 __attribute__((ext_vector_type(4)));
typedef short s16x8 __attribute__((ext_vector_type(8)));
typedef float f32x4 __attribute__((ext_vector_type(4)));

#define DEV static __device__ __forceinline__
#define MDEV __device__ __forceinline__
#define LDS_AS __attribute__((address_space(3)))

DEV f32x4 mfma16(const bf16x8& a, const bf16x8& b, const f32x4& c) {
  return __builtin_amdgcn_mfma_f32_16x16x32_bf16(a, b, c, 0, 0, 0);
}

DEV f32x4 zero4() { f32x4 z = {0.f, 0.f, 0.f, 0.f}; return z; }

DEV int wave_id() { return __builtin_amdgcn_readfirstlane(threadIdx.x >> 6); }

// ... 88 lines not shown
constexpr int kLdPol = 0;
#else
constexpr int kLdPol = kSC1;
#endif
DEV float4 ld_sc1(rsrc_t r, uint32_t off) {
  const f32x4 v = __builtin_bit_cast(f32x4, __builtin_amdgcn_raw_buffer_load_b128(r, off, 0, kLdPol));
  return make_float4(v[0], v[1], v[2], v[3]);
}
DEV void wait_vm_all() { __builtin_amdgcn_s_waitcnt(0x0F70); }

#ifdef DMLC_NO_WT_STORES
constexpr bool kWtStores = false;
#else
constexpr bool kWtStores = true;
#endif
DEV const void* uni(const void* p) {
  const uint64_t v = reinterpret_cast<uint64_t>(p);
  const uint32_t lo = __builtin_amdgcn_readfirstlane((uint32_t)v), hi = __builtin_amdgcn_readfirstlane((uint32_t)(v >> 32));
  return reinterpret_cast<const void*>(((uint64_t)hi << 32) | lo);
}
DEV void st_out16(void* base, uint32_t byte_off, const uint4& v) {
  if constexpr (kWtStores)
    __builtin_amdgcn_raw_buffer_store_b128(__builtin_bit_cast(u32x4, v), buf_rsrc(base), byte_off, 0, kSC1);
  else
    st_maybe_nt<kNtDefault>(reinterpret_cast<uint4*>(reinterpret_cast<char*>(base) + byte_off), v);
}
DEV void st_out8(void* base, uint32_t byte_off, const uint2& v) {
  if constexpr (kWtStores)
    __builtin_amdgcn_raw_buffer_store_b64(__builtin_bit_cast(u32x2, v), buf_rsrc(base), byte_off, 0, kSC1);
  else
    st_maybe_nt<kNtDefault>(reinterpret_cast<uint2*>(reinterpret_cast<char*>(base) + byte_off), v);
}

#ifndef DMLC_SPIN_LIMIT
#define DMLC_SPIN_LIMIT (1u << 20)
#endif

DEV unsigned bar_gen(unsigned* gen) { return __hip_atomic_load(gen, __ATOMIC_RELAXED, __HIP_MEMORY_SCOPE_AGENT); }
DEV void bar_arrive(unsigned* cnt, unsigned* gen, unsigned g0, unsigned n) {
  if (__hip_atomic_fetch_add(cnt, 1u, __ATOMIC_RELAXED, __HIP_MEMORY_SCOPE_AGENT) == n - 1) {
    __hip_atomic_store(cnt, 0u, __ATOMIC_RELAXED, __HIP_MEMORY_SCOPE_AGENT);
    __hip_atomic_store(gen, g0 + 1u, __ATOMIC_RELAXED, __HIP_MEMORY_SCOPE_AGENT);
  }
}
DEV void bar_wait(unsigned* gen, unsigned g0, unsigned* err) {
  for (unsigned it = 0; bar_gen(gen) == g0; ++it) {
    if (it >= DMLC_SPIN_LIMIT) {
      __hip_atomic_fetch_or(err, 1u, __ATOMIC_RELAXED, __HIP_MEMORY_SCOPE_AGENT);
      break;
    }
    __builtin_amdgcn_s_sleep(2);
  }
}

DEV float wave_sum(float v) {
#pragma unroll
  for (int o = 32; o > 0; o >>= 1) v += __shfl_xor(v, o);
  return v;
}

DEV bool last_arrival(unsigned int* tk, int blk, int nblk) {
  const int g = blk & 7;
  const unsigned gsize = (unsigned)((nblk - g + 7) >> 3);
  unsigned int* gc = tk + g * 32;
  if (__hip_atomic_fetch_add(gc, 1u, __ATOMIC_RELAXED, __HIP_MEMORY_SCOPE_AGENT) != gsize - 1) return false;
  __hip_atomic_store(gc, 0u, __ATOMIC_RELAXED, __HIP_MEMORY_SCOPE_AGENT);
  const unsigned ngroups = (unsigned)(nblk < 8 ? nblk : 8);
  unsigned int* top = tk + 8 * 32;
  if (__hip_atomic_fetch_add(top, 1u, __ATOMIC_RELAXED, __HIP_MEMORY_SCOPE_AGENT) != ngroups - 1) return false;
  __hip_atomic_store(top, 0u, __ATOMIC_RELAXED, __HIP_MEMORY_SCOPE_AGENT);
  return true;
}

struct Seam { unsigned* p; int n; unsigned target; };
DEV void seam_wait(const Seam& s, int lane, unsigned* err, unsigned errbit, int lane_target = -1) {
  const bool on = lane < s.n;
  unsigned* q = s.p + 32 * (on ? lane : 0);
  const unsigned t = lane_target >= 0 ? (unsigned)lane_target : s.target;
  for (unsigned it = 0;; ++it) {
    const bool ok = !on || __hip_atomic_load(q, __ATOMIC_RELAXED, __HIP_MEMORY_SCOPE_AGENT) >= t;
    if (__all(ok)) break;
    if (it >= DMLC_SPIN_LIMIT) {
      if (lane == 0) __hip_atomic_fetch_or(err, errbit, __ATOMIC_RELAXED, __HIP_MEMORY_SCOPE_AGENT);
      break;
    }
    __builtin_amdgcn_s_sleep(1);
  }
}

DEV uint32_t mix32(uint32_t x) {
  x ^= x >> 16; x *= 0x7feb352du;
  x ^= x >> 15; x *= 0x846ca68bu;
  x ^= x >> 16;
  return x;
}

DEV uint32_t order_perm(uint32_t pos, uint32_t n, int half_bits, uint32_t seed, uint32_t epoch) {
  const uint32_t ek = mix32(mix32(seed ^ 0x5bd1e995u) ^ mix32(epoch * 0x85ebca77u + 0x632be5abu));
  const uint32_t mask = (1u << half_bits) - 1u;
  uint32_t x = pos;
  do {
    uint32_t l = x >> half_bits, r = x & mask;
#pragma unroll
    for (int k = 0; k < 4; ++k) {
      const uint32_t t = l ^ (mix32(r ^ (ek + (uint32_t)k * 0x9e3779b9u)) & mask);
      l = r;
      r = t;
    }
    x = (l << half_bits) | r;
  } while (x >= n);
  return x;
}

template <class Src>
DEV int order_row(const Src& s, int64_t step, int b) {
  const uint32_t epoch = (uint32_t)(step / s.period);
  const int64_t j = step - (int64_t)epoch * s.period;
  const int bb = b < s.bvalid ? b : s.bvalid - 1;
  const uint32_t pos = (uint32_t)((j * s.world + s.rank) * s.bvalid + bb);
  return (int)order_perm(pos, (uint32_t)s.n, s.half_bits, s.seed, epoch);
}

template <class Src>
DEV int batch_index(const Src& s, int B, int b) {
  if (s.idx_base) {
    int row = 0;
    if (s.counter) row = (int)(*s.counter % (int64_t)s.period);
    return s.idx_base[row * B + b];
  }
  return order_row(s, *s.counter, b);
}

DEV int swz128(int pix, int chunk) { return pix * 64 + ((chunk ^ (pix & 7)) << 3); }
DEV int swzpad(int pix, int chunk) { return pix * 64 + ((chunk ^ ((pix + 4 * (pix >> 4)) & 7)) << 3); }

inline hipError_t lds_optin(const void* f, size_t bytes, bool& done) {
  if (done) return hipSuccess;
  const hipError_t e = hipFuncSetAttribute(f, hipFuncAttributeMaxDynamicSharedMemorySize, (int)bytes);
  done = e == hipSuccess;
  return e;
}
#define DMLC_LDS_OPTIN(fn, bytes)                                                                   \
  do {                                                                                              \
    static bool optin_done_ = false;                                                                \
    const hipError_t optin_e_ = ::dmlc::lds_optin(reinterpret_cast<const void*>(fn), (bytes), optin_done_); \
    if (optin_e_ != hipSuccess) return optin_e_;                                                    \
  } while (0)

}

#define DMLC_TK_CONV1_FWD 0
#define DMLC_TK_CONV2_FWD 1
#define DMLC_TK_GEMM 2
#define DMLC_TK_HEAD 3
#define DMLC_TK_DGRAD 4
#define DMLC_TK_W1 5
#define DMLC_TK_W2 6
#define DMLC_TK_SGD 7
#define DMLC_TK_N 8
#define DMLC_TK_BLOCKS 1024
#define DMLC_TK_SLOTS 8
#ifdef DMLC_TIMING
extern __device__ unsigned long long dmlc_timing_buf[DMLC_TK_N * DMLC_TK_BLOCKS * DMLC_TK_SLOTS];
#define DMLC_STAMP(k, slot)                                                                          \
  do {                                                                                               \
    if (threadIdx.x == 0 && blockIdx.x < DMLC_TK_BLOCKS)                                             \
// ... 31 lines not shown
```

csrc/kernels/conv2_core.h:

```cpp
#pragma once
#include "w1_common.h"

namespace dmlc {


constexpr int WS_ELEMS = 64 * 320;
constexpr size_t WS_BYTES = 2 * WS_ELEMS * 2;

DEV void ws_dma(const bf16* Wg, int kh, bf16* buf, int w, int lane) {
#pragma unroll
  for (int i = 0; i < 5; ++i) {
    const int j = w * 5 + i;
    const int P = j * 64 + lane, row = P / 40, pc = P - row * 40, lc = pc ^ (row & 7);
    __builtin_amdgcn_global_load_lds(Wg + row * 1600 + kh * 320 + lc * 8, (LDS_AS void*)(buf + j * 512), 16, 0, 0);
  }
}

DEV const bf16* slice_buf(const bf16* s0, const bf16* ws, int kh) { return kh == 0 ? s0 : ws + (kh & 1) * WS_ELEMS; }

struct Slice5 { uint4 a, b, c, d, e; };
DEV uint4 ws_chunk(const bf16* Wg, int kh, int w, int lane, int i) {
  const int P = (w * 5 + i) * 64 + lane, row = P / 40, pc = P - row * 40, lc = pc ^ (row & 7);
  return *reinterpret_cast<const uint4*>(Wg + row * 1600 + kh * 320 + lc * 8);
}
DEV Slice5 ws_fetch(const bf16* Wg, int kh, int w, int lane) {
  return Slice5{ws_chunk(Wg, kh, w, lane, 0), ws_chunk(Wg, kh, w, lane, 1), ws_chunk(Wg, kh, w, lane, 2),
                ws_chunk(Wg, kh, w, lane, 3), ws_chunk(Wg, kh, w, lane, 4)};
}
DEV void ws_put(bf16* buf, int w, int lane, Slice5 v) {
  uint4* p = reinterpret_cast<uint4*>(buf) + w * 5 * 64 + lane;
  p[0] = v.a; p[64] = v.b; p[128] = v.c; p[192] = v.d; p[256] = v.e;
}

template <bool EXTRA>
DEV void conv2_core(const bf16* Wg, const bf16* xin, bf16* ws, f32x4 (&acc)[2][2], f32x4& accx, int pg, int cp,
                    int xsel, int g, int li, int tid, const bf16* s0, int tk = -1) {
  constexpr int NPX = EXTRA ? 3 : 2;
  const int w = wave_id(), lane = tid & 63, sw = li & 7;
  int xo[NPX][8][2];
#pragma unroll
  for (int t = 0; t < NPX; ++t) {
    const int px = 16 * (t < 2 ? pg + 4 * t : 8) + li;
    const int y = px / 12, x = px - y * 12;
    const int pb = y * 16 + x, key0 = (x + 4 * y) & 7;
#pragma unroll
    for (int d = 0; d < 8; ++d)
#pragma unroll
      for (int s = 0; s < 2; ++s) xo[t][d][s] = pb * 64 + (((4 * s + g) ^ ((key0 + d) & 7)) << 3);
  }
  int ao[2];
#pragma unroll
  for (int s = 0; s < 2; ++s) ao[s] = (32 * cp + li) * 320 + (((4 * s + g) ^ sw) << 3);
#pragma unroll
  for (int t = 0; t < 2; ++t) { acc[0][t] = zero4(); acc[1][t] = zero4(); }
  accx = zero4();
  if (!s0) ws_dma(Wg, 0, ws, w, lane);
  const bf16* sb0 = s0 ? s0 : ws;
  __syncthreads();
  auto load_chunk = [&](int kh, int j, bf16x8& a0, bf16x8& a1, bf16x8 (&bx)[NPX]) {
    const int kw = j >> 1, s = j & 1;
    const bf16* wr = slice_buf(sb0, ws, kh) + kw * 64 + ao[s];
    a0 = lds_b128(wr);
    a1 = lds_b128(wr + 16 * 320);
#pragma unroll
    for (int t = 0; t < NPX; ++t) bx[t] = lds_b128(xin + xo[t][(kw + 4 * kh) & 7][s] + (kh * 16 + kw) * 64);
  };
#pragma unroll
  for (int kh = 0; kh < 5; ++kh) {
    if (kh < 4) ws_dma(Wg, kh + 1, ws + ((kh + 1) & 1) * WS_ELEMS, w, lane);
    bf16x8 A0[2], A1[2], BX[2][NPX];
    load_chunk(kh, 0, A0[0], A1[0], BX[0]);
#pragma unroll
    for (int j = 0; j < 10; ++j) {
      const int cur = j & 1;
      wait_lds();
      __builtin_amdgcn_sched_barrier(0);
      if (j + 1 < 10) load_chunk(kh, j + 1, A0[cur ^ 1], A1[cur ^ 1], BX[cur ^ 1]);
      __builtin_amdgcn_sched_barrier(0);
#pragma unroll
      for (int t = 0; t < 2; ++t) {
        acc[0][t] = mfma16(A0[cur], BX[cur][t], acc[0][t]);
        acc[1][t] = mfma16(A1[cur], BX[cur][t], acc[1][t]);
      }
      if constexpr (EXTRA) accx = mfma16(xsel ? A1[cur] : A0[cur], BX[cur][NPX - 1], accx);
      __builtin_amdgcn_sched_barrier(0);
    }
    if (kh < 4) __syncthreads();
    if (tk >= 0 && (kh == 0 || kh == 2)) DMLC_STAMP(tk, 5 + kh / 2);
  }
  if (tk >= 0) DMLC_STAMP(tk, 7);
}

template <class F>
DEV void conv2_tiles(const bf16* Wg, const bf16* xin, bf16* ws, int w, int g, int li, int tid, const bf16* s0,
                     F&& fn, int tk = -1) {
  const int cp = w & 1, pg = w >> 1;
  f32x4 acc[2][2], accx;
  if (w < 4) {
    conv2_core<true>(Wg, xin, ws, acc, accx, pg, cp, pg, g, li, tid, s0, tk);
    fn(2 * cp + pg, 8, accx);
  } else {
    conv2_core<false>(Wg, xin, ws, acc, accx, pg, cp, 0, g, li, tid, s0, tk);
  }
#pragma unroll
  for (int t = 0; t < 2; ++t) { fn(2 * cp, pg + 4 * t, acc[0][t]); fn(2 * cp + 1, pg + 4 * t, acc[1][t]); }
}

constexpr size_t DG_LDS = (C2_XIN + C2_OUT) * 2 + 2304 * 3 + WS_BYTES;

template <bool IN_LAUNCH>
DEV void conv2_dgrad_image(const DmlcConv2DgradArgs& a, int b, char* smem, Seam seam = Seam{nullptr, 0, 0u},
                           unsigned* err = nullptr) {
  bf16* dyp = reinterpret_cast<bf16*>(smem);
  bf16* outs = dyp + C2_XIN;
  bf16* dp2 = outs + C2_OUT;
  uint8_t* am2 = reinterpret_cast<uint8_t*>(dp2 + 2304);
  bf16* ws = reinterpret_cast<bf16*>(am2 + 2304);
  const int tid = threadIdx.x, lane = tid & 63, w = wave_id();
  const int g = lane >> 4, li = lane & 15;
  DMLC_STAMP(DMLC_TK_DGRAD, 0);
  if (!IN_LAUNCH) stage16<288>(dp2, reinterpret_cast<const bf16*>(a.dp2) + (size_t)b * 2304, tid);
  stage16<144>(am2, a.am2 + (size_t)b * 2304, tid);
  const Slice5 s0v = ws_fetch(reinterpret_cast<const bf16*>(a.wd), 0, w, lane);
  bf16* dy2 = reinterpret_cast<bf16*>(a.dy2) + (size_t)b * 9216;

  for (int s = tid; s < 2048; s += NT) {
    const int pix = s >> 3, c = s & 7;
    const int r = pix >> 4, col = pix & 15;
    if (r < 2 || r >= 14 || col < 2 || col >= 14) *reinterpret_cast<bf16x8*>(dyp + swzpad(pix, c)) = bf16x8{};
  }
  if (IN_LAUNCH) {
    if (tid < 64) seam_wait(seam, tid, err, 2u);
    lds_barrier();
    if (tid < 288)
      reinterpret_cast<uint4*>(dp2)[tid] = __builtin_bit_cast(
          uint4, __builtin_amdgcn_raw_buffer_load_b128(buf_rsrc(a.dp2), (uint32_t)(b * 2304 + 8 * tid) * 2, 0, kSC1));
  }
  lds_barrier();
  DMLC_STAMP(DMLC_TK_DGRAD, 1);
  static_assert(36 * 8 <= NT, "one pool-bwd task per thread");
  const int win = tid >> 3, pc = tid & 7, py = win / 6, px = win - py * 6;
  bf16x8 dv[4];
  if (tid < 36 * 8) {
    float o[4][8];
    pool_bwd_2x2<6>(dp2, am2, py, px, pc, o);
#pragma unroll
    for (int k = 0; k < 4; ++k) {
      const int y = 2 * py + (k >> 1), x = 2 * px + (k & 1);
      dv[k] = to_bf16x8(o[k]);
      *reinterpret_cast<bf16x8*>(dyp + swzpad((y + 2) * 16 + x + 2, pc)) = dv[k];
    }
  }
  ws_put(ws, w, lane, s0v);
  if (tid < 36 * 8) {
#pragma unroll
    for (int k = 0; k < 4; ++k) {
      const int y = 2 * py + (k >> 1), x = 2 * px + (k & 1);
      st_out16(dy2, (uint32_t)((y * 12 + x) * 64 + pc * 8) * 2, __builtin_bit_cast(uint4, dv[k]));
    }
  }
  lds_barrier();
  DMLC_STAMP(DMLC_TK_DGRAD, 2);

  conv2_tiles(reinterpret_cast<const bf16*>(a.wd), dyp, ws, w, g, li, tid, ws, [&](int ct, int t, const f32x4& acc) {
    const int px = 16 * t + li, cb = 16 * ct + 4 * g;
    const bf16x4 v = pack4(acc[0], acc[1], acc[2], acc[3]);
    *reinterpret_cast<bf16x4*>(outs + swz128(px, cb >> 3) + ((cb >> 2) & 1) * 4) = v;
  });
  __syncthreads();
  DMLC_STAMP(DMLC_TK_DGRAD, 3);
  bf16* dp1 = reinterpret_cast<bf16*>(a.dp1) + (size_t)b * 9216;
  for (int s = tid; s < 1152; s += NT) {
    const int p = s >> 3, c = s & 7;
    st_out16(dp1, (uint32_t)(p * 64 + c * 8) * 2, __builtin_bit_cast(uint4, lds_b128(outs + swz128(p, c))));
  }
  DMLC_STAMP(DMLC_TK_DGRAD, 4);
}

}
```

csrc/kernels/sgd_common.h:

```cpp
#pragma once
#include "common.h"
#include "api.h"

namespace dmlc {

constexpr int SEG_NUMEL[10] = {4800, 64, 102400, 64, 884736, 384, 73728, 192, 1920, 10};
constexpr int C2_SPLIT = 4, C2_ROWS = 256 / C2_SPLIT / 16;
constexpr int C2_BLOCKS = 1600 / C2_ROWS;
constexpr int C1_SPLIT = 32;
constexpr int C1_LOADS = 5;
constexpr int C1_BLOCKS = 150;
constexpr int FC_F4_PER_THREAD = 4;
constexpr int FC2_ROWS = 64, FC2_COLS = 48;
constexpr int FC2_BLOCKS = (384 / FC2_ROWS) * (192 / FC2_COLS);
constexpr int FC_TAIL = 192 + 1920 + 10;
constexpr int FC_TAIL_BLOCKS = (FC_TAIL + 255) / 256;
constexpr int SGD_LDS4 = 512;
static_assert(FC2_COLS * (FC2_ROWS + 8) * 2 / 16 <= SGD_LDS4, "fc2 transpose tile exceeds the role LDS");

__host__ __device__ inline int fc1_first(const DmlcSgdArgs& a) { return a.fc1_fused ? a.off[5] : a.off[4]; }
__host__ __device__ inline int fc1_blocks(const DmlcSgdArgs& a) {
  return ((a.off[6] - fc1_first(a)) / 4 + 256 * FC_F4_PER_THREAD - 1) / (256 * FC_F4_PER_THREAD);
}
__host__ __device__ inline int fc_role_count(const DmlcSgdArgs& a) { return fc1_blocks(a) + FC2_BLOCKS + FC_TAIL_BLOCKS; }
// ... 109 lines not shown
#pragma unroll
  for (int u = 0; u < FC_F4_PER_THREAD; ++u) {
    const int i = i4[u] * 4;
    if (i4[u] >= end4) continue;
    float4 v = w[u];
    if (apply) {
      v.x -= f * g[u].x; v.y -= f * g[u].y; v.z -= f * g[u].z; v.w -= f * g[u].w;
      reinterpret_cast<float4*>(a.master)[i4[u]] = v;
    }
    if (i < a.off[5])
      *reinterpret_cast<bf16x4*>(shadow + (i - a.off[4])) = pack4(v.x, v.y, v.z, v.w);
  }
}

DEV void fc2_block(const DmlcSgdArgs& a, int blk, float lr, bf16* tl , int tid) {
  constexpr int LD = FC2_ROWS + 8, C4 = FC2_COLS / 4;
  constexpr int F4 = FC2_ROWS * C4 / 256;
  const bool apply = a.mode != 3, act = tid < 256;
  const float f = lr * a.grad_scale;
  const int k0 = (blk / (192 / FC2_COLS)) * FC2_ROWS, n0 = (blk % (192 / FC2_COLS)) * FC2_COLS;
  if (act) {
    float4 w[F4], g[F4];
#pragma unroll
    for (int u = 0; u < F4; ++u) {
      const int j4 = u * 256 + tid, kk = j4 / C4, n = n0 + 4 * (j4 - kk * C4);
      const size_t e = (size_t)a.off[6] + (size_t)(k0 + kk) * 192 + n;
      w[u] = *reinterpret_cast<const float4*>(a.master + e);
      g[u] = grad_ld4(a, e);
    }
#pragma unroll
    for (int u = 0; u < F4; ++u) {
      const int j4 = u * 256 + tid, kk = j4 / C4, nn = 4 * (j4 - kk * C4);
      float4 v = w[u];
      if (apply) {
        v.x -= f * g[u].x; v.y -= f * g[u].y; v.z -= f * g[u].z; v.w -= f * g[u].w;
        *reinterpret_cast<float4*>(a.master + a.off[6] + (size_t)(k0 + kk) * 192 + n0 + nn) = v;
      }
      *reinterpret_cast<bf16x4*>(reinterpret_cast<bf16*>(a.fc2n) + (size_t)(k0 + kk) * 192 + n0 + nn) =
          pack4(v.x, v.y, v.z, v.w);
      tl[(nn + 0) * LD + kk] = (bf16)v.x; tl[(nn + 1) * LD + kk] = (bf16)v.y;
      tl[(nn + 2) * LD + kk] = (bf16)v.z; tl[(nn + 3) * LD + kk] = (bf16)v.w;
    }
  }
  lds_barrier();
  if (!act) return;
  for (int c = tid; c < FC2_COLS * (FC2_ROWS / 8); c += 256) {
    const int nn = c / (FC2_ROWS / 8), k8 = c - nn * (FC2_ROWS / 8);
    *reinterpret_cast<bf16x8*>(reinterpret_cast<bf16*>(a.fc2t) + (size_t)(n0 + nn) * 384 + k0 + 8 * k8) =
        *reinterpret_cast<const bf16x8*>(tl + nn * LD + 8 * k8);
  }
}

DEV void fc_tail_block(const DmlcSgdArgs& a, int blk, float lr, int tid) {
  if (tid >= 256) return;
  const int j = blk * 256 + tid;
  if (j >= FC_TAIL) return;
  const int i = a.off[7] + j;
  float v = a.master[i];
  if (a.mode != 3) {
    v -= lr * a.grad_scale * grad_ld1(a, i);
    a.master[i] = v;
  }
  if (i >= a.off[8] && i < a.off[8] + 1920) {
    const int q = i - a.off[8], k = q / 10, n = q - k * 10;
    reinterpret_cast<bf16*>(a.fc3t)[n * 192 + k] = (bf16)v;
    reinterpret_cast<bf16*>(a.fc3d)[k * 32 + n] = (bf16)v;
  }
}

DEV void fc_role(const DmlcSgdArgs& a, int r, float lr, int64_t step, float4* lds, int tid) {
  const int nfc1 = fc1_blocks(a);
  if (r < nfc1) fc1_block(a, r, lr, step, tid);
  else if ((r -= nfc1) < FC2_BLOCKS) fc2_block(a, r, lr, reinterpret_cast<bf16*>(lds), tid);
  else fc_tail_block(a, r - FC2_BLOCKS, lr, tid);
}

DEV void copy_next_row(const DmlcSgdArgs& a, int64_t step, int row, int tid) {
  if (tid >= 192) return;
  const int src = order_row(a.next, step + 1, row);
  reinterpret_cast<uint4*>(a.xnext + (size_t)row * 3072)[tid] =
      reinterpret_cast<const uint4*>(a.xdata + (size_t)src * 3072)[tid];
}

DEV void publish_step(const DmlcSgdArgs& a, int64_t step, float lr, int lane) {
  float loss = 0.f, corr = 0.f;
  for (int q = lane; q < a.nhead; q += 64) { loss += a.loss_part[q]; corr += (float)a.correct_part[q]; }
  loss = wave_sum(loss);
  corr = wave_sum(corr);
  if (lane == 0) {
    float* st = a.stats + (size_t)(step % a.stats_len) * 4;
    st[0] = (float)(step + 1);
    st[1] = loss / (float)a.B;
    st[2] = corr / (float)a.B;
    st[3] = lr;
    *a.step = step + 1;
  }
}

}
```

distributed-machine-learning-using-cnn-cifar-10-dataset-_amd/_build.py:

```python
from __future__ import annotations

import concurrent.futures as cf
import glob
import hashlib
import os
import shutil
import subprocess
import sys
import sysconfig

PKG_DIR = os.path.dirname(os.path.abspath(__file__))
REPO = os.path.dirname(PKG_DIR)
CSRC = os.path.join(REPO, "csrc")
LIB_DIR = os.path.join(PKG_DIR, "_lib")
OBJ_DIR = os.path.join(REPO, "build", "obj")
ARCH = os.environ.get("PYTORCH_ROCM_ARCH", "gfx950")
ROCM = os.environ.get("ROCM_PATH", "/opt/rocm")

TIMING = os.environ.get("DMLC_TIMING") == "1"
_VAR = os.environ.get("DMLC_VARIANT", "")
VARIANT, VARIANT_FLAGS = (_VAR.split(":", 1)[0], _VAR.split(":", 1)[1].split()) if _VAR else ("", [])
_SUFFIX = "_timing" if TIMING else (f"_{VARIANT}" if VARIANT else "")
HIP_LIB = os.path.join(LIB_DIR, f"libdmlc_hip{_SUFFIX}.so")
RT_LIB = os.path.join(LIB_DIR, "_dmlc_rt" + (sysconfig.get_config_var("EXT_SUFFIX") or ".so"))


def _torch_paths():
    import torch.utils.cpp_extension as ce
    import torch
    inc = ce.include_paths()
    lib = os.path.join(os.path.dirname(torch.__file__), "lib")
    abi = int(torch._C._GLIBCXX_USE_CXX11_ABI)
    return inc, lib, abi


def _hash(paths, flags) -> str:
    h = hashlib.sha256()
    for p in sorted(paths):
        with open(p, "rb") as f:
            h.update(p.encode())
            h.update(f.read())
    h.update(" ".join(flags).encode())
    return h.hexdigest()[:16]


def _run(cmd):
    if os.environ.get("DMLC_BUILD_VERBOSE"):
        print(" ".join(cmd), flush=True)
    r = subprocess.run(cmd, stdout=subprocess.PIPE, stderr=subprocess.STDOUT, text=True)
    if r.returncode != 0:
        raise RuntimeError(f"build command failed ({r.returncode}):\n{' '.join(cmd)}\n{r.stdout}")
    return r.stdout


def _compile(src, deps, out, cmd_prefix, flags):
    stamp = out + ".stamp"
    key = _hash([src] + deps, cmd_prefix + flags)
    if os.path.exists(out) and os.path.exists(stamp) and open(stamp).read() == key:
        return False
    os.makedirs(os.path.dirname(out), exist_ok=True)
    _run(cmd_prefix + flags + ["-c", src, "-o", out])
    with open(stamp, "w") as f:
        f.write(key)
    return True


def _link(objs, out, cmd):
    stamp = out + ".stamp"
    key = _hash(objs, cmd)
    if os.path.exists(out) and os.path.exists(stamp) and open(stamp).read() == key:
        return False
    tmp = out + ".tmp"
    _run(cmd + objs + ["-o", tmp])
    os.replace(tmp, out)
    with open(stamp, "w") as f:
        f.write(key)
    return True


def build(hip: bool = True, rt: bool = True, jobs: int | None = None) -> dict:
    inc, torch_lib, abi = _torch_paths()
    py_inc = sysconfig.get_paths()["include"]
    jobs = jobs or min(8, os.cpu_count() or 4)
    os.makedirs(LIB_DIR, exist_ok=True)
    torch_flags = ["-std=c++17", "-O2", "-fPIC", f"-D_GLIBCXX_USE_CXX11_ABI={abi}", "-D__HIP_PLATFORM_AMD__",
                   "-DUSE_ROCM", "-DTORCH_EXTENSION_NAME=dmlc", f"-I{ROCM}/include", f"-I{py_inc}"]
    torch_flags += [f"-I{p}" for p in inc]
    torch_link = [f"-L{torch_lib}", f"-Wl,-rpath,{torch_lib}", "-lc10", "-ltorch_cpu", "-ltorch"]
    headers = glob.glob(os.path.join(CSRC, "kernels", "*.h"))
    out = {"hip": None, "rt": None}
    jobs_list = []
    hip_objs, rt_objs = [], []
    if hip:
        hipcc = os.path.join(ROCM, "bin", "hipcc")
        hip_flags = ["-std=c++17", "-O3", "-fPIC", f"--offload-arch={ARCH}", "-munsafe-fp-atomics"]
        if TIMING:
            hip_flags += ["-DDMLC_TIMING", "-fgpu-rdc"]
        hip_flags += VARIANT_FLAGS
        for src in sorted(glob.glob(os.path.join(CSRC, "kernels", "*.hip"))):
            o = os.path.join(OBJ_DIR, os.path.basename(src) + (f"{_SUFFIX.replace('_', '.')}.o" if _SUFFIX else ".o"))
            hip_objs.append(o)
            jobs_list.append((src, headers, o, [hipcc], hip_flags))
        bheaders = headers + glob.glob(os.path.join(CSRC, "bindings", "*.h"))
        for bsrc in sorted(glob.glob(os.path.join(CSRC, "bindings", "*.cpp"))):
            o = os.path.join(OBJ_DIR, os.path.basename(bsrc) + ".o")
            hip_objs.append(o)
            jobs_list.append((bsrc, bheaders, o, ["g++"], torch_flags))
    if rt:
        rt_headers = glob.glob(os.path.join(CSRC, "runtime", "*.h"))
        import pybind11
        rt_flags = ["-std=c++17", "-O3", "-fPIC", "-fvisibility=hidden", f"-I{py_inc}",
                    f"-I{pybind11.get_include()}"]
        for src in sorted(glob.glob(os.path.join(CSRC, "runtime", "*.cpp"))):
            o = os.path.join(OBJ_DIR, "rt_" + os.path.basename(src) + ".o")
            rt_objs.append(o)
            jobs_list.append((src, rt_headers, o, ["g++"], rt_flags))
    with cf.ThreadPoolExecutor(jobs) as ex:
        futs = [ex.submit(_compile, *j) for j in jobs_list]
        for f in futs:
            f.result()
    if hip:
        hipcc = os.path.join(ROCM, "bin", "hipcc")
        _link(hip_objs, HIP_LIB, [hipcc, "-shared", "-fPIC", f"--offload-arch={ARCH}"]
              + (["-fgpu-rdc"] if TIMING else []) + torch_link
              + [f"-L{torch_lib}", "-lc10_hip", "-ltorch_hip"])
        out["hip"] = HIP_LIB
    if rt and rt_objs:
        _link(rt_objs, RT_LIB, ["g++", "-shared", "-fPIC", "-pthread"])
        out["rt"] = RT_LIB
    return out


def clean():
    shutil.rmtree(OBJ_DIR, ignore_errors=True)
    shutil.rmtree(LIB_DIR, ignore_errors=True)


if __name__ == "__main__":
    if "--clean" in sys.argv:
        clean()
    print(build())
```

distributed-machine-learning-using-cnn-cifar-10-dataset-_amd/engine/fused.py:

```python
from __future__ import annotations

import math
import os
from typing import Dict, List, Optional

import torch

from .. import config as C
from ..parallel.dist import quiesce_for_capture
from ..data.order import OrderSpec
from ..models import cifar_cnn as M
from ..ops import _ext

OPS = None


def _ops():
    global OPS
    if OPS is None:
        _ext.hip()
        OPS = torch.ops.dmlc
    return OPS


SEG_OFF = [s.offset for s in M.PARAM_SPECS]


def head_rows(B: int) -> int:
    return 2 if B <= 256 else 4


VARIANT_DEFAULTS = {
    "split_fwd": False,
    "fc_fused": None,
    "fc_dgrad": None,
    "fc_dw_in_wgrad": None,
    "fc1_epilogue": True,
    "wgrad_sgd": True,
    "wgrad_sgd_fp8": False,
    "fp8_dgrad": True,
    "fp8_wgrad": True,
    "comm_sgd": False,
    "xraw_prefetch": True,
    "fwd12_split": True,
    "fc_sgd_in_chain": None,
    "grad16": True,
}
TICKET_WORDS = 9 * 32
WBAR_WORDS = 20 * 32
SEG = {M.short(s.name): s for s in M.PARAM_SPECS}


def _gemm_params(M_, N_, K_, lda, a_kmajor, ldb, b_kmajor, ldc, c_mode, ksplit=1, relu=0, nvalid=None, b_par=0,
                 s_par=0):
    return [M_, N_, K_, lda, a_kmajor, ldb, b_kmajor, ldc, c_mode, ksplit, relu, N_ if nvalid is None else nvalid,
            b_par, s_par]


FC1_NUMEL = 2304 * 384


class FusedCifarEngine:

    def __init__(self, batch_size: int, data: torch.Tensor, labels: torch.Tensor, *, device=None,
                 flat_params: Optional[torch.Tensor] = None, lr: float = C.LEARNING_RATE,
                 lr_decay: float = C.LR_DECAY, decay_steps: float = C.NUM_GENS_TO_WAIT, staircase: bool = True,
                 relu_logits: bool = True, crop_offset=(4, 4), world_size: int = 1, rank: int = 0,
                 process_group=None, seed: int = 0, fc1_split: Optional[int] = None, g1: Optional[int] = None,
                 g2: Optional[int] = None, stats_len: int = 4096, comm_dtype: str = "fp32",
                 capture_comm: Optional[bool] = None, dtype: str = "bf16", allreduce: str = "auto",
                 dp_schedule: str = "serial", dp_force: bool = False, warmup_steps: int = 0,
                 conv_split: Optional[int] = None, conv1_split: Optional[int] = None,
                 dgrad_split: Optional[int] = None, variant: Optional[dict] = None):
        unknown = set(variant or {}) - set(VARIANT_DEFAULTS)
        if unknown:
            raise ValueError(f"unknown engine variant keys {sorted(unknown)}")
        V = dict(VARIANT_DEFAULTS, **(variant or {}))
        self.variant = V
        ops = _ops()
        self.ops = ops
        self.device = torch.device(device or "cuda")
        dev = self.device
        Bv = int(batch_size)
        if Bv < 1:
            raise ValueError("batch size must be >= 1")
        B = -(-Bv // 16) * 16
        self.B, self.Bv = B, Bv
        self.world_size, self.rank, self.pg = world_size, rank, process_group
        self.dp = world_size > 1 or dp_force
        self.lr0, self.decay, self.decay_steps, self.staircase = lr, lr_decay, decay_steps, staircase
        self.warmup = float(warmup_steps)
        self.relu_logits = relu_logits
        self.cy, self.cx = crop_offset
        self.comm_dtype = comm_dtype
        if capture_comm is None:
            capture_comm = self.dp and self._pg_backend() == "nccl"
        self.capture_comm = bool(capture_comm)
        self.seed = seed
        if dtype not in ("bf16", "fp8"):
            raise ValueError("fused engine dtype must be bf16 or fp8")
        self.dtype = dtype

        assert data.dtype == torch.uint8 and tuple(data.shape[1:]) == (32, 32, 3)
        self.data = data.to(dev).contiguous()
        self.labels = labels.to(dev, torch.int32).contiguous()
        self.n_data = self.data.shape[0]
        self.order = OrderSpec(self.n_data, Bv, world_size, rank, seed)
        self.period = self.order.period
        self.order_desc = self.order.descriptor()
        self.bidx = torch.zeros(B, dtype=torch.int32, device=dev)
        self.xraw = torch.zeros(B, 3072, dtype=torch.uint8, device=dev)

        if flat_params is None:
            flat_params = M.init_flat_params(torch.Generator().manual_seed(seed))
        self.master = flat_params.to(dev, torch.float32).contiguous().clone()
        self.xgmi, self.comm_info = None, {"allreduce": "rccl" if self.dp else "none"}
        self._buckets = {True: (M.FC_BUCKET_OFFSET, self.master.numel() - M.FC_BUCKET_OFFSET),
                         False: (0, M.FC_BUCKET_OFFSET)}
        if world_size > 1 and dev.type == "cuda" and comm_dtype in ("fp32", "bf16") and allreduce != "rccl":
            from ..parallel import xgmi as X
            pattern = ([(0, self.master.numel())] if dp_schedule == "serial"
                       else [self._buckets[True], self._buckets[False]])
            self.xgmi, self.comm_info = X.select(self.master.numel(), rank, world_size, dev, pattern,
                                                 mode=allreduce, group=process_group, wire=comm_dtype,
                                                 captured=self.capture_comm)
        elif dp_force and world_size == 1 and allreduce == "xgmi" and dev.type == "cuda":
            from ..parallel import xgmi as X
            self.xgmi = X.XgmiAllReduce(self.master.numel(), 0, 1, None, wire=comm_dtype)
            self.comm_info = {"allreduce": "xgmi", "wire": comm_dtype}
        if self.xgmi is not None:
            self.grad = self.xgmi.buf[:self.master.numel()]
            self.grad.zero_()
# ... 33 lines not shown
        self.p1, self.am1 = z(B, 12, 12, 64), z(B, 12, 12, 64, dt=torch.uint8)
        self.p2, self.am2 = z(B, 6, 6, 64), z(B, 6, 6, 64, dt=torch.uint8)
        self.h1part = z(self.fc1_split, B, 384, dt=torch.float32)
        self.h1, self.h2, self.dl = z(B, 384), z(B, 192), z(B, 16)
        self.dh1, self.dh2 = z(B, 384), z(B, 192)
        self.dp2 = z(B, 6, 6, 64)
        self.dp1, self.dy2 = z(B, 12, 12, 64), z(B, 144, 64)
        self.part2, self.partb2 = z(self.g2, 1600, 64, dt=torch.float32), z(self.g2, 64, dt=torch.float32)
        self.part1, self.partb1 = z(self.g1, 80, 64, dt=torch.float32), z(self.g1, 64, dt=torch.float32)
        local_ = int(os.environ.get("LOCAL_WORLD_SIZE", world_size))
        ndev_ = torch.cuda.device_count() if dev.type == "cuda" else 0
        cus = torch.cuda.get_device_properties(dev).multi_processor_count if dev.type == "cuda" else 0
        fc_ok = B <= 256 and cus >= 256 and local_ <= max(1, ndev_)
        self.fc_fused = (fc_ok if V["fc_fused"] is None else bool(V["fc_fused"]) and fc_ok) \
            and os.environ.get("DMLC_FC_FUSED", "1") != "0"
        self.h1part8 = z(8, B, 384, dt=torch.float32) if self.fc_fused else None
        self.fc_sync = torch.zeros(212 * 32, dtype=torch.int32, device=dev)
        self._fc_src = None
        hr = 4 if self.fc_fused else head_rows(B)
        self.loss_part = z(B // hr, dt=torch.float32)
        self.correct_part = z(B // hr, dt=torch.int32)
        self.step_t = torch.zeros(1, dtype=torch.int64, device=dev)
        self.step_sgd = torch.zeros(1, dtype=torch.int64, device=dev)
        self.ticket = torch.zeros(TICKET_WORDS, dtype=torch.int32, device=dev)
        self.stats = torch.zeros(stats_len, 4, dtype=torch.float32, device=dev)
        self.logits_buf = z(B, 10, dt=torch.float32)

        p = {k: self.master[s.offset:s.offset + s.numel] for k, s in SEG.items()}
        self.pv = p
        gv = {k: self.grad[s.offset:s.offset + s.numel] for k, s in SEG.items()}
        self.gv = gv
        self.grad16 = None
        if (self.dp and comm_dtype == "bf16" and self.xgmi is None and self.fc_fused and bool(V["grad16"])):
            self.grad16 = torch.zeros(self.master.numel(), dtype=torch.bfloat16, device=dev)
        self.gv_chain = ({k: self.grad16[s.offset:s.offset + s.numel] for k, s in SEG.items()}
                         if self.grad16 is not None else gv)

        self._fc1_fwd = dict(A=[self.p2.view(B, 2304)], B=[self.fc1n], C=[self.h1part], bias=[None],
                             params=_gemm_params(B, 384, 2304, 2304, 1, 384, 0, 384, 2, self.fc1_split,
                                                 b_par=FC1_NUMEL))
        self._fc_bwd = dict(
            A=[self.dh1, self.p2.view(B, 2304), self.h1, self.h2, self.dh1, self.dh2, self.dl],
            B=[self.fc1n, self.dh1, self.dh2, self.dl, self.dh1, self.dh2, self.dl],
            C=[self.dp2.view(B, 2304), gv["full_weight_1"], gv["full_weight_2"], gv["full_weight_3"],
               gv["full_bias_1"], gv["full_bias_2"], gv["full_bias_3"]],
            bias=[None] * 7,
            params=(_gemm_params(B, 2304, 384, 384, 1, 384, 1, 2304, 1, b_par=FC1_NUMEL)
                    + _gemm_params(2304, 384, B, 2304, 0, 384, 0, 384, 0)
                    + _gemm_params(384, 192, B, 384, 0, 192, 0, 192, 0)
                    + _gemm_params(192, 16, B, 192, 0, 16, 0, 10, 0, nvalid=10)
                    + _gemm_params(384, 8, B, 384, 0, 8, 0, 1, 3, nvalid=384)
                    + _gemm_params(192, 8, B, 192, 0, 8, 0, 1, 3, nvalid=192)
                    + _gemm_params(16, 8, B, 16, 0, 8, 0, 1, 3, nvalid=10)))
        fb = self._fc_bwd
        self.fc1_epilogue = not self.dp and bool(V["fc1_epilogue"])
        in_launch = (1 <= self.g1 <= cus and 4 * self.g2 <= cus and bool(V["wgrad_sgd"])
                     and os.environ.get("DMLC_WGRAD_SGD", "1") != "0")
        self.wgrad_apply = in_launch and self.fc1_epilogue and (not self.fp8 or bool(V["wgrad_sgd_fp8"]))
        local = int(os.environ.get("LOCAL_WORLD_SIZE", world_size))
        ndev = torch.cuda.device_count() if dev.type == "cuda" else 0
        reduce_ok = in_launch and self.dp and local <= max(1, ndev)
        self._grad_in_launch = in_launch and (self.wgrad_apply or reduce_ok)
        self.wgrad_reduce = self.dp and self._grad_in_launch
        self.comm_sgd = self.xgmi is not None and not self.fp8 and bool(V["comm_sgd"])
        share = max(1, -(-int(os.environ.get("LOCAL_WORLD_SIZE", world_size)) // max(1, ndev)))
        self._comm_blocks = 512 if share == 1 else max(32, 128 // share)
        self.xraw_prefetch = self.fused_fwd and not self.fp8 and self.conv_split == 1 and bool(V["xraw_prefetch"])
        self.fwd12_split = (self.conv_split == 2 and self.conv1_split == 2 and not self.fp8
                            and B * 2 <= cus and local_ <= max(1, ndev_) and bool(V["fwd12_split"])
                            and os.environ.get("DMLC_FWD12_SPLIT", "1") != "0")
        self.c12_flags = torch.zeros(32 * 2 * B if self.fwd12_split else 1, dtype=torch.int32, device=dev)
        self.wbar = torch.zeros(WBAR_WORDS, dtype=torch.int32, device=dev)
        self._err_host = (torch.zeros(1, dtype=torch.int32).pin_memory() if dev.type == "cuda"
                          else torch.zeros(1, dtype=torch.int32))
        fdg = V["fc_dgrad"]
        self.fc_dgrad = self.fc_fused and not self.fp8_dgrad and (bool(fdg) if fdg is not None else True)
        self._dgrad_done = False
        fdw = V["fc_dw_in_wgrad"]
        self.fc_dw_in_wgrad = (self.fc_fused and self.wgrad_apply
                               and (bool(fdw) if fdw is not None else not self.fc_dgrad))
        fsc = V["fc_sgd_in_chain"]
        self.fc_sgd_in_chain = (self.fc_fused and self.wgrad_apply and not self.fc_dw_in_wgrad
                                and (bool(fsc) if fsc is not None else B < 256))
        self._fc_bwd_sgd = dict(fb, C=[fb["C"][0], p["full_weight_1"]] + fb["C"][2:],
                                params=fb["params"][:14] + _gemm_params(2304, 384, B, 2304, 0, 384, 0, 384, 4,
                                                                        s_par=FC1_NUMEL)
                                + fb["params"][28:])

        self.graphs: List[torch.cuda.CUDAGraph] = []
        self.chains: Dict[int, Optional[torch.cuda.CUDAGraph]] = {}
        self.comm_stream = torch.cuda.Stream(device=dev) if self.dp else None
        assert dp_schedule in ("overlap", "serial"), dp_schedule
        self.dp_schedule = dp_schedule
        self._captured_schedule = None
        if self.dp:
            self.comm_info.update(schedule=dp_schedule, backend=self._backend(),
                                  captured_comm=bool(self.capture_comm or self.xgmi is not None),
                                  grad_dtype="bf16" if self.grad16 is not None else "fp32")
        self.host_step = 0
        self._sync_bidx()
        self.refresh_shadows()

    @staticmethod
    def _pick_fc1_split(B: int) -> int:
        tiles = max(1, math.ceil(B / 64)) * 6
        for s in (8, 4, 2):
            if tiles * s <= 450:
                return s
        return 1

    def refresh_shadows(self):
        if self.fp8:
            s = self.host_step & 1
            w2 = self.master[SEG["conv2_kernel"].offset:SEG["conv2_kernel"].offset + SEG["conv2_kernel"].numel]
            self.amax_w[s] = w2.abs().max()
            self.amax_w[s ^ 1] = 0.0
        self._sgd(mode=3)

    def set_step(self, step: int):
        old = int(self.step_t.item())
        if (old ^ int(step)) & 1:
            self.fc1n[int(step) & 1].copy_(self.fc1n[old & 1])
        self.step_t.fill_(int(step))
        self.step_sgd.fill_(int(step))
        self.host_step = int(step)
        self._sync_bidx()

    def _sync_bidx(self):
        self.bidx.copy_(self._padded(self.batch_indices(self.host_step)))
        self._sync_xraw()

    def _sync_xraw(self):
        if getattr(self, "xraw_prefetch", False):
            self.xraw.copy_(self.data.index_select(0, self.bidx.long()).view(self.B, 3072))

    def epoch_permutation(self, epoch: int) -> torch.Tensor:
        return self.order.epoch_shard(epoch).to(torch.int32)

    def batch_indices(self, step: int) -> torch.Tensor:
        return self.order.batch(step).to(torch.int32)

    def _padded(self, idx: torch.Tensor) -> torch.Tensor:
        idx = idx.to(self.device, torch.int32).reshape(-1)
        if idx.numel() == self.B:
            return idx.contiguous()
        assert 1 <= idx.numel() <= self.B, idx.numel()
        return torch.cat([idx, idx[-1:].expand(self.B - idx.numel())]).contiguous()

    def _forward(self, idx, counter, period, train=True, logits_out=None):
        o, p = self.ops, self.pv
        if self.fwd12_split:
            o.conv12_fwd(self.data, idx, counter, period, self.cy, self.cx, self.w1f, p["conv1_bias"], self.p1,
                         self.am1, self.w2f, p["conv2_bias"], self.p2, self.am2, self.xraw if train else None, False,
                         self.c12_flags, self.wbar[10 * 32:10 * 32 + 1])
        elif self.conv_split == 2 and not self.fp8:
            o.conv1_fwd_split(self.data, idx, counter, period, self.cy, self.cx, self.w1f, p["conv1_bias"], self.p1,
                              self.am1, self.xraw if train else None, self.conv1_split)
            o.conv2_fwd_split(self.p1, self.w2f, p["conv2_bias"], self.p2, self.am2)
        elif self.fused_fwd and not self.fp8:
            pre = train and self.xraw_prefetch and idx is self.bidx
            o.conv12_fwd(self.data, idx, counter, period, self.cy, self.cx, self.w1f, p["conv1_bias"], self.p1,
                         self.am1, self.w2f, p["conv2_bias"], self.p2, self.am2, self.xraw if train else None, pre)
        else:
            o.conv1_fwd(self.data, idx, counter, period, self.cy, self.cx, self.w1f, p["conv1_bias"], self.p1,
                        self.am1, self.amax_x if self.fp8 else None, self.xraw if train else None)
        if self.fp8:
            o.conv2_fwd_fp8(self.p1, self.w2f8[0], p["conv2_bias"], self.amax_x, self.scale_w, counter, self.p2, self.am2,
                            *((self.p1f8, self.sx8) if train and self.fp8_wgrad else (None, None)))
        elif not self.fused_fwd and self.conv_split == 1:
            o.conv2_fwd(self.p1, self.w2f, p["conv2_bias"], self.p2, self.am2)
        if train and self.fc_fused:
            self._fc_src = (idx, counter, period)
            return
        self._gemm(self._fc1_fwd)
        o.head(self.h1part, p["full_bias_1"], self.fc2t, p["full_bias_2"], self.fc3t, p["full_bias_3"], self.fc3d,
               self.fc2n, self.labels, idx, counter, period, 1.0 / (self.Bv * self.world_size), self.relu_logits,
               train, self.h1, self.h2, self.dl, self.dh1, self.dh2, self.loss_part, self.correct_part, logits_out,
               self.Bv, self.step_t, self.step_sgd)

    def _gemm(self, f, sgd: bool = False):
        if sgd:
            sched = [self.lr0, self.decay, self.decay_steps, 1.0 if self.staircase else 0.0, self.warmup, 1.0]
            self.ops.gemm_grouped(f["A"], f["B"], f["C"], f["bias"], f["params"], self.step_t, self.fc1n, sched)
        else:
            self.ops.gemm_grouped(f["A"], f["B"], f["C"], f["bias"], f["params"], self.step_t)

    def _fc_backward(self, fused_sgd: bool = False):
        if self.fc_fused:
            self._fc_chain(fused_sgd)
            return
        self._gemm(self._fc_bwd_sgd if fused_sgd else self._fc_bwd, sgd=fused_sgd)

    def _fc_chain(self, fused_sgd: bool):
        if self._fc_src is None:
            raise RuntimeError("_fc_chain must follow a training _forward")
        if self._dgrad_done:
            raise RuntimeError("the previous fc chain's conv backward never ran")
        idx, counter, period = self._fc_src
        self._fc_src = None
        p, gv = self.pv, self.gv
        sched = [self.lr0, self.decay, self.decay_steps, 1.0 if self.staircase else 0.0, self.warmup, 1.0]
        all_sgd = fused_sgd and self.fc_sgd_in_chain
        if not fused_sgd:
            gv = self.gv_chain
        g = p if all_sgd else gv
        self.ops.fc_chain(self.p2.view(self.B, 2304), self.fc1n, self.h1part8, p["full_bias_1"], self.fc2t,
                          p["full_bias_2"], self.fc3t, p["full_bias_3"], self.fc3d, self.labels, idx, counter, period,
                          1.0 / (self.Bv * self.world_size), self.relu_logits, self.h1, self.h2, self.dl, self.dh1,
                          self.dh2, self.loss_part, self.correct_part, self.dp2.view(self.B, 2304),
                          p["full_weight_1"] if fused_sgd else gv["full_weight_1"], g["full_weight_2"],
                          g["full_weight_3"], g["full_bias_1"], g["full_bias_2"], g["full_bias_3"], fused_sgd,
                          sched, self.Bv, self.step_t, self.step_sgd, self.fc_sync, self.wbar[10 * 32:10 * 32 + 1],
                          not (fused_sgd and self.fc_dw_in_wgrad),
                          *((self.am2, self.w2d, self.dp1, self.dy2) if self.fc_dgrad else (None, None, None, None)),
                          self.fc2n if all_sgd else None)
        self._dgrad_done = self.fc_dgrad

    def _conv_backward(self, src=None, apply: bool = False, reduce: bool = False):
        o = self.ops
        idx, counter, period = src or (self.bidx, None, 1)
        assert not apply or (self.wgrad_apply and src is None), "apply mode: the training step only"
        assert not reduce or self._grad_in_launch
        if self._dgrad_done:
            self._dgrad_done = False
        elif self.fp8_dgrad:
            o.conv2_dgrad_fp8(self.dp2, self.am2, self.w2f8[1], self.scale_w, self.dp1, self.dy2,
                              *((self.dy2f8, self.sy_img) if self.fp8_wgrad else (None, None)))
        elif self.dgrad_split == 2:
            o.conv2_dgrad_split(self.dp2, self.am2, self.w2d, self.dp1, self.dy2)
        else:
            o.conv2_dgrad(self.dp2, self.am2, self.w2d, self.dp1, self.dy2)
        if apply or reduce:
            fc_acts = None
            if apply and self.fc_dw_in_wgrad:
                fc_acts = [self.p2.view(self.B, 2304), self.h1, self.h2, self.dl, self.dh1, self.dh2]
            o.wgrad_sgd(self.data, idx, counter, period, self.cy, self.cx, self.dp1, self.am1, self.p1, self.dy2,
                        self.groups2, self.xraw, self.wbar,
                        *(self._sgd_args(mode=0, fc1_fused=True) if apply else self._sgd_args(mode=1)),
                        fc_acts=fc_acts, fc_sgd_done=bool(apply and self.fc_sgd_in_chain), **self._w8)
            return
        o.wgrad(self.data, idx, counter, period, self.cy, self.cx, self.dp1, self.am1,
                self.part1, self.partb1, self.p1, self.dy2, self.part2, self.partb2, self.groups2, self.xraw,
                **self._w8)

    def _sgd_args(self, mode: int, scale: float = 1.0, roles: int = 0, finalize: bool = True,
                  fc1_fused: bool = False) -> tuple:
        gflat = self.grad16 if (self.grad16 is not None and mode in (1, 2)) else self.grad
        return (self.master, gflat, mode, scale, SEG_OFF, self.part1, self.partb1, self.part2, self.partb2,
                self.w1f, self.w2f, self.w2d, self.fc1n, self.fc2t, self.fc2n, self.fc3t, self.fc3d,
                self.step_t, self.lr0, self.decay, self.decay_steps, self.staircase, self.ticket,
                self.loss_part, self.correct_part, self.stats,
                *((self.w2f8, self.amax_w, self.scale_w) if self.fp8 else (None, None, None)),
                roles, finalize, self.Bv, self.bidx, self.order_desc, self.warmup, fc1_fused,
                None if mode == 3 else self.step_sgd,
                *((self.xraw, self.data) if self.xraw_prefetch and mode in (0, 2) and finalize else (None, None)))

    def _sgd(self, mode: int, scale: float = 1.0, roles: int = 0, finalize: bool = True, fc1_fused: bool = False):
        self.ops.sgd(*self._sgd_args(mode, scale, roles, finalize, fc1_fused))

    @property
    def barriers_in_use(self) -> bool:
        return bool(self.wgrad_apply or self._grad_in_launch or self.fc_fused or self.fwd12_split)

    def queue_error_copy(self):
        if self.barriers_in_use:
            self._err_host.copy_(self.wbar[10 * 32:10 * 32 + 1], non_blocking=True)

    def check_barriers(self, cached: bool = False):
        if not self.barriers_in_use:
            return
        e = int(self._err_host[0]) if cached else int(self.wbar[10 * 32].item())
        if e != 0:
            mode = "apply" if self.wgrad_apply else "reduce"
            parts = []
            if e & 1:
                parts.append(f"k_wgrad ({mode} mode): a sub-grid barrier timed out; rerun with DMLC_WGRAD_SGD=0")
            if e & 2:
                parts.append("k_fc_chain / k_conv12_fwd_split: a hand-off wait timed out; rerun with "
                             "DMLC_FC_FUSED=0 / DMLC_FWD12_SPLIT=0")
            if self.fwd12_split:
                self.c12_flags.zero_()
            raise RuntimeError("; ".join(parts) + f" (blocks not co-resident, error word {e})")

    def _allreduce(self, t: torch.Tensor):
        import torch.distributed as dist
        if t.dtype == torch.bfloat16:
            dist.all_reduce(t, group=self.pg)
        elif self.comm_dtype == "bf16":
            tb = t.to(torch.bfloat16)
            dist.all_reduce(tb, group=self.pg)
            t.copy_(tb)
        else:
            dist.all_reduce(t, group=self.pg)

    def _allreduce_bucket(self, fc: bool):
        off, n = self._buckets[fc]
        if self.xgmi is not None:
            self.xgmi.all_reduce(off, n)
        elif fc or self.grad16 is not None:
            self._allreduce(self._wire_grad()[off:off + n])
        else:
            import torch.distributed as dist
            dist.all_reduce(self.grad[off:off + n], group=self.pg)

    def _wire_grad(self) -> torch.Tensor:
        return self.grad16 if self.grad16 is not None else self.grad

    def check_comm(self):
        self.check_barriers()
        if self.xgmi is not None:
            self.xgmi.check()

    def _pg_backend(self) -> str:
        import torch.distributed as dist
        return dist.get_backend(self.pg) if dist.is_available() and dist.is_initialized() else "none"

    def _backend(self) -> str:
        if self.xgmi is not None:
            return "xgmi"
        if not self.dp:
            return "none"
        return self._pg_backend()

    def _seg_compute_a(self):
        self._forward(self.bidx, None, 1, train=True)
        self._fc_backward()

    def _seg_forward(self):
        self._forward(self.bidx, None, 1, train=True)

    def _seg_fc(self):
        self._fc_backward()

    def _seg_compute_b(self):
        if self.wgrad_reduce:
            self._conv_backward(reduce=True)
            return
        self._seg_compute_b_launch()

    def _seg_compute_b_launch(self):
        self._conv_backward()
        self._sgd(mode=1 if self.dp else 0)

    def _seg_apply(self):
        self._sgd(mode=2, scale=1.0)

    def _seg_apply_fc(self):
        self._sgd(mode=2, scale=1.0, roles=2, finalize=False)

    def _seg_apply_conv(self):
        self._sgd(mode=2, scale=1.0, roles=1, finalize=True)

    def compute_gradients(self, idx: Optional[torch.Tensor] = None, check: bool = True):
        g = self._compute_gradients(idx)
        if check:
            self.check_barriers()
        return g if self.grad16 is None else self.grad16.float()

    def _compute_gradients(self, idx: Optional[torch.Tensor] = None):
        if idx is None:
            self._seg_compute_a()
            if self._grad_in_launch:
                self._conv_backward(reduce=True)
                return self.grad
            self._conv_backward()
        else:
            ids = self._padded(idx)
            self._forward(ids, None, 1, train=True)
            self._fc_backward()
            if self._grad_in_launch:
                self._conv_backward(src=(ids, None, 1), reduce=True)
                self._sync_xraw()
                return self.grad
            self._conv_backward(src=(ids, None, 1))
            self._sync_xraw()
        self._sgd(mode=1)
        return self.grad

    def _reset_step_state(self):
        self._fc_src = None
        self._dgrad_done = False
        self._pending_comm = None
        if self.fwd12_split and not torch.cuda.is_current_stream_capturing():
            self.c12_flags.zero_()

    def _eager_step(self):
        try:
            self._eager_step_body()
        except BaseException:
            self._reset_step_state()
            raise
        if not torch.cuda.is_current_stream_capturing():
            self._join_comm()

    def _eager_step_body(self):
        if not self.dp:
            if self.fc1_epilogue:
                self._forward(self.bidx, None, 1, train=True)
                self._fc_backward(fused_sgd=True)
                if self.wgrad_apply:
                    self._conv_backward(apply=True)
                    return
                self._conv_backward()
                self._sgd(mode=0, fc1_fused=True)
                return
            self._seg_compute_a()
            self._seg_compute_b()
            return
        if self.dp_schedule == "serial":
            self._serial_dp_step([self._seg_compute_ab, self._seg_apply])
            return
        self._dp_step([self._seg_forward, self._seg_fc, self._seg_compute_b_launch, self._seg_apply_fc,
                       self._seg_apply_conv])

    def _seg_compute_ab(self):
        self._seg_compute_a()
        self._seg_compute_b()

    def _serial_dp_step(self, seg):
        seg[0]()
        n = self.master.numel()
        if self.comm_sgd:
            self.xgmi.all_reduce_sgd(self._sgd_args(mode=2), blocks=self._comm_blocks)
            return
        if self.xgmi is not None:
            self.xgmi.all_reduce(0, n)
        else:
            self._allreduce(self._wire_grad()[:n])
        seg[1]()

    def _dp_step(self, seg):
        main = torch.cuda.current_stream(self.device)
        seg[0]()
        self._join_comm()
        seg[1]()
        ev_fc = torch.cuda.Event()
        ev_fc.record(main)
        self.comm_stream.wait_event(ev_fc)
        with torch.cuda.stream(self.comm_stream):
            self._allreduce_bucket(fc=True)
        seg[2]()
        ev_wg = torch.cuda.Event()
        ev_wg.record(main)
        self.comm_stream.wait_event(ev_wg)
        ev_conv, ev_done = torch.cuda.Event(), torch.cuda.Event()
        with torch.cuda.stream(self.comm_stream):
            self._allreduce_bucket(fc=False)
            ev_conv.record(self.comm_stream)
            seg[3]()
            ev_done.record(self.comm_stream)
        main.wait_event(ev_conv)
        seg[4]()
        self._pending_comm = ev_done

    def _join_comm(self):
        ev = getattr(self, "_pending_comm", None)
        if ev is not None:
            torch.cuda.current_stream(self.device).wait_event(ev)
            self._pending_comm = None

    @property
    def single_graph(self) -> bool:
        return not self.dp or self.capture_comm or self.xgmi is not None

    def capture(self, steps_per_graph: int = 8):
        quiesce_for_capture(self.device, self.pg if self.dp else None)
        self._reset_step_state()
        self.graphs, self.chains = [], {}
        pool = torch.cuda.graph_pool_handle()
        if self.single_graph:
            segs = [lambda: self._steps_joined(1)]
        elif self.dp_schedule == "serial":
            segs = [self._seg_compute_ab, self._seg_apply]
        else:
            segs = [self._seg_forward, self._seg_fc, self._seg_compute_b_launch, self._seg_apply_fc,
                    self._seg_apply_conv]
        self._captured_schedule = self.dp_schedule
        for fn in segs:
            self.graphs.append(self._capture_one(fn, pool))
        if self.single_graph:
            k = 2
# ... 161 lines not shown
```

Baseline: 3.610 million images/sec.

## Fuse fc chain, conv2 dgrad and wgrad+SGD into one persistent backward kernel

Adds a k_backward kernel that runs the fc chain, per-image conv2 dgrad and the conv wgrad/SGD roles in a single launch. Per-image dY2/dP1 readiness is signalled through a hand-off word array, so wgrad blocks can start as soon as their images are ready instead of waiting at a kernel boundary. It is enabled by default on single-GPU runs with batch sizes in (128, 256]. This removes a launch and the serialisation between the two kernels, but needs all blocks to be co-resident and relies on write-through stores and spin waits, which risk timeouts.

```diff
diff --git a/csrc/bindings/torch_ops.cpp b/csrc/bindings/torch_ops.cpp
--- a/csrc/bindings/torch_ops.cpp
+++ b/csrc/bindings/torch_ops.cpp
@@ -422,16 +422,23 @@
   CHECK_HIP(dmlc_head(&a, stream_of(h1part)));
 }
 
-void fc_chain(const Tensor& p2, const Tensor& fc1n, const Tensor& h1part, const Tensor& b1, const Tensor& w2t,
-              const Tensor& b2, const Tensor& w3t, const Tensor& b3, const Tensor& w3d, const Tensor& labels,
-              const Tensor& idx, const c10::optional<Tensor>& counter, int64_t period, double inv_batch,
-              bool relu_logits, const Tensor& h1, const Tensor& h2, const Tensor& dl, const Tensor& dh1,
-              const Tensor& dh2, const Tensor& loss_part, const Tensor& correct_part, const Tensor& dp2,
-              const Tensor& gw1, const Tensor& gw2, const Tensor& gw3, const Tensor& gb1, const Tensor& gb2,
-              const Tensor& gb3, bool fuse_sgd, at::ArrayRef<double> sched, int64_t nvalid, const Tensor& step,
-              const c10::optional<Tensor>& step_copy, const Tensor& sync, const Tensor& err, bool dw_tasks,
-              const c10::optional<Tensor>& am2, const c10::optional<Tensor>& w2d, const c10::optional<Tensor>& dp1,
-              const c10::optional<Tensor>& dy2, const c10::optional<Tensor>& fc2n) {
+#define DMLC_FC_PARAMS                                                                                    \
+  const Tensor &p2, const Tensor &fc1n, const Tensor &h1part, const Tensor &b1, const Tensor &w2t,          \
+      const Tensor &b2, const Tensor &w3t, const Tensor &b3, const Tensor &w3d, const Tensor &labels,       \
+      const Tensor &idx, const c10::optional<Tensor> &counter, int64_t period, double inv_batch,            \
+      bool relu_logits, const Tensor &h1, const Tensor &h2, const Tensor &dl, const Tensor &dh1,            \
+      const Tensor &dh2, const Tensor &loss_part, const Tensor &correct_part, const Tensor &dp2,            \
+      const Tensor &gw1, const Tensor &gw2, const Tensor &gw3, const Tensor &gb1, const Tensor &gb2,        \
+      const Tensor &gb3, bool fuse_sgd, at::ArrayRef<double> sched, int64_t nvalid, const Tensor &step,     \
+      const c10::optional<Tensor> &step_copy, const Tensor &sync, const Tensor &err, bool dw_tasks,         \
+      const c10::optional<Tensor> &am2, const c10::optional<Tensor> &w2d, const c10::optional<Tensor> &dp1, \
+      const c10::optional<Tensor> &dy2, const c10::optional<Tensor> &fc2n
+#define DMLC_FC_ARGS                                                                                      \
+  p2, fc1n, h1part, b1, w2t, b2, w3t, b3, w3d, labels, idx, counter, period, inv_batch, relu_logits, h1, h2, dl, \
+      dh1, dh2, loss_part, correct_part, dp2, gw1, gw2, gw3, gb1, gb2, gb3, fuse_sgd, sched, nvalid, step,       \
+      step_copy, sync, err, dw_tasks, am2, w2d, dp1, dy2, fc2n
+
+static bool make_fc(DMLC_FC_PARAMS, DmlcFcArgs& a, DmlcConv2DgradArgs& g) {
   const int64_t B = p2.size(0);
   TORCH_CHECK(B >= 16 && B <= 256 && B % 16 == 0, "fc_chain: batch must be a multiple of 16 in [16, 256]");
   check(p2, "p2", at::kBFloat16, {B, 2304});
@@ -468,8 +475,6 @@
   TORCH_CHECK(sched.size() == 6, "fc_chain: sched = {lr0, decay, decay_steps, staircase, warmup, grad_scale}");
   if (nvalid < 0) nvalid = B;
   TORCH_CHECK(nvalid >= 1 && nvalid <= B, "fc_chain: nvalid must be in [1, B]");
-  c10::DeviceGuard guard(p2.device());
-  DmlcFcArgs a;
   memset(&a, 0, sizeof(a));
   a.B = (int)B; a.nvalid = (int)nvalid; a.mtiles = (int)((B + 63) / 64);
   a.p2 = p2.data_ptr(); a.w1 = fc1n.data_ptr(); a.h1part = h1part.data_ptr<float>();
@@ -507,7 +512,6 @@
   const bool dg_on = am2.has_value();
   TORCH_CHECK(dg_on == w2d.has_value() && dg_on == dp1.has_value() && dg_on == dy2.has_value(),
               "fc_chain: am2, w2d, dp1, dy2 come together");
-  DmlcConv2DgradArgs g;
   memset(&g, 0, sizeof(g));
   if (dg_on) {
     check(*am2, "am2", at::kByte, {B, 6, 6, 64});
@@ -518,6 +522,14 @@
     g.dp1 = dp1->data_ptr(); g.dy2 = dy2->data_ptr(); g.B = (int)B;
     g.split = B <= 128 ? 1 : 0;
   }
+  return dg_on;
+}
+
+void fc_chain(DMLC_FC_PARAMS) {
+  DmlcFcArgs a;
+  DmlcConv2DgradArgs g;
+  const bool dg_on = make_fc(DMLC_FC_ARGS, a, g);
+  c10::DeviceGuard guard(p2.device());
   CHECK_HIP(dmlc_fc_chain(&a, dg_on ? &g : nullptr, stream_of(p2)));
 }
 
@@ -658,10 +670,15 @@
   CHECK_HIP(dmlc_sgd(&a, stream_of(master)));
 }
 
-void wgrad_sgd(const Tensor& data, const Tensor& idx, const c10::optional<Tensor>& counter, int64_t period, int64_t cy,
-               int64_t cx, const Tensor& dp1, const Tensor& am1, const Tensor& p1, const Tensor& dy2,
-               int64_t groups2, const Tensor& xraw, const Tensor& bar, DMLC_SGD_PARAMS,
-               const c10::optional<at::TensorList> fc_acts, bool fc_sgd_done, const c10::optional<at::TensorList> fp8) {
+#define DMLC_WGRAD_SGD_PARAMS                                                                              \
+  const Tensor &data, const Tensor &idx, const c10::optional<Tensor> &counter, int64_t period, int64_t cy,   \
+      int64_t cx, const Tensor &dp1, const Tensor &am1, const Tensor &p1, const Tensor &dy2,                 \
+      int64_t groups2, const Tensor &xraw, const Tensor &bar, DMLC_SGD_PARAMS,                               \
+      const c10::optional<at::TensorList> fc_acts, bool fc_sgd_done, const c10::optional<at::TensorList> fp8
+#define DMLC_WGRAD_SGD_ARGS                                                                                \
+  data, idx, counter, period, cy, cx, dp1, am1, p1, dy2, groups2, xraw, bar, DMLC_SGD_ARGS, fc_acts, fc_sgd_done, fp8
+
+static DmlcWgradArgs make_wgrad_sgd(DMLC_WGRAD_SGD_PARAMS) {
   DmlcWgradArgs a = make_wgrad(data, idx, counter, period, cy, cx, dp1, am1, part1, partb1, p1, dy2, part2, partb2,
                                groups2, xraw, fp8);
   TORCH_CHECK((mode == 0 && fc1_fused && step_rd.has_value() && roles == 0 && finalize &&
@@ -704,8 +721,31 @@
     f.err = a.bar + 10 * 32;
     a.fc_in_launch = 1;
   }
+  return a;
+}
+
+void wgrad_sgd(DMLC_WGRAD_SGD_PARAMS) {
+  const DmlcWgradArgs a = make_wgrad_sgd(DMLC_WGRAD_SGD_ARGS);
   c10::DeviceGuard guard(dp1.device());
   CHECK_HIP(dmlc_wgrad(&a, stream_of(dp1)));
+}
+
+static thread_local DmlcWgradArgs staged_wgrad;
+static thread_local bool staged_wgrad_set = false;
+void backward_fused_wgrad(DMLC_WGRAD_SGD_PARAMS) {
+  staged_wgrad = make_wgrad_sgd(DMLC_WGRAD_SGD_ARGS);
+  staged_wgrad_set = true;
+}
+void backward_fused(const Tensor& hand, DMLC_FC_PARAMS) {
+  TORCH_CHECK(staged_wgrad_set, "backward_fused: backward_fused_wgrad must come first");
+  staged_wgrad_set = false;
+  check_numel(hand, "hand", at::kInt, DMLC_HAND_WORDS);
+  DmlcFcArgs a;
+  DmlcConv2DgradArgs g;
+  const bool dg_on = make_fc(DMLC_FC_ARGS, a, g);
+  TORCH_CHECK(dg_on, "backward_fused: the conv2 dgrad (am2, w2d, dp1, dy2) runs in the launch");
+  c10::DeviceGuard guard(p2.device());
+  CHECK_HIP(dmlc_backward(&a, &g, &staged_wgrad, reinterpret_cast<unsigned int*>(hand.data_ptr<int>()), stream_of(p2)));
 }
 
 }
@@ -753,6 +793,23 @@
         "bool finalize, int batch, Tensor(q!)? bidx=None, Tensor? order=None, float warmup=0.0, "
         "bool fc1_fused=False, Tensor? step_rd=None, Tensor(v!)? xnext=None, Tensor? xdata=None, "
         "Tensor[]? fc_acts=None, bool fc_sgd_done=False, Tensor[]? fp8=None) -> ()");
+  m.def("backward_fused_wgrad(Tensor data, Tensor idx, Tensor? counter, int period, int cy, int cx, Tensor dp1, Tensor am1, "
+        "Tensor p1, Tensor dy2, int groups2, Tensor xraw, Tensor(z!) bar, "
+        "Tensor(a!) master, Tensor(b!) grad, int mode, float grad_scale, int[] off, Tensor(r!) part1, Tensor(s!) partb1, "
+        "Tensor(t!) part2, Tensor(u!) partb2, Tensor(c!) w1f, Tensor(d!) w2f, Tensor(e!) w2d, Tensor(f!) fc1n, "
+        "Tensor(g!) fc2t, Tensor(h!) fc2n, Tensor(i!) fc3t, Tensor(j!) fc3d, Tensor(k!) step, float lr0, float decay, "
+        "float decay_steps, bool staircase, Tensor(l!) ticket, Tensor loss_part, Tensor correct_part, "
+        "Tensor(m!) stats, Tensor(n!)? w2f8, Tensor(o!)? amax_w, Tensor(p!)? scale_w, int roles, "
+        "bool finalize, int batch, Tensor(q!)? bidx=None, Tensor? order=None, float warmup=0.0, "
+        "bool fc1_fused=False, Tensor? step_rd=None, Tensor(v!)? xnext=None, Tensor? xdata=None, "
+        "Tensor[]? fc_acts=None, bool fc_sgd_done=False, Tensor[]? fp8=None) -> ()");
+  m.def("backward_fused(Tensor(w!) hand, Tensor p2, Tensor(a!) fc1n, Tensor(b!) h1part, Tensor b1, Tensor w2t, Tensor b2, "
+        "Tensor w3t, Tensor b3, Tensor w3d, Tensor labels, Tensor idx, Tensor? counter, int period, float inv_batch, "
+        "bool relu_logits, Tensor(c!) h1, Tensor(d!) h2, Tensor(e!) dl, Tensor(f!) dh1, Tensor(g!) dh2, "
+        "Tensor(h!) loss_part, Tensor(i!) correct_part, Tensor(j!) dp2, Tensor(k!) gw1, Tensor(l!) gw2, "
+        "Tensor(m!) gw3, Tensor(n!) gb1, Tensor(o!) gb2, Tensor(p!) gb3, bool fuse_sgd, float[] sched, "
+        "int nvalid, Tensor step, Tensor(q!)? step_copy, Tensor(r!) sync, Tensor(s!) err, bool dw_tasks=True, "
+        "Tensor? am2=None, Tensor? w2d=None, Tensor(t!)? dp1=None, Tensor(u!)? dy2=None, Tensor(v!)? fc2n=None) -> ()");
   m.def("sgd(Tensor(a!) master, Tensor(b!) grad, int mode, float grad_scale, int[] off, Tensor part1, Tensor partb1, "
         "Tensor part2, Tensor partb2, Tensor(c!) w1f, Tensor(d!) w2f, Tensor(e!) w2d, Tensor(f!) fc1n, "
         "Tensor(g!) fc2t, Tensor(h!) fc2n, Tensor(i!) fc3t, Tensor(j!) fc3d, Tensor(k!) step, float lr0, float decay, "
@@ -788,4 +845,6 @@
   m.impl("sgd", &sgd);
   m.impl("xgmi_allreduce_sgd", &xgmi_allreduce_sgd);
   m.impl("wgrad_sgd", &wgrad_sgd);
-}
+  m.impl("backward_fused_wgrad", &backward_fused_wgrad);
+  m.impl("backward_fused", &backward_fused);
+}
diff --git a/csrc/kernels/api.h b/csrc/kernels/api.h
--- a/csrc/kernels/api.h
+++ b/csrc/kernels/api.h
@@ -223,6 +223,11 @@
 hipError_t dmlc_wgrad(const DmlcWgradArgs* a, hipStream_t s);
 hipError_t dmlc_gemm_grouped(DmlcGemmGroup* g, hipStream_t s);
 hipError_t dmlc_fc_chain(const DmlcFcArgs* a, const DmlcConv2DgradArgs* dg, hipStream_t s);
+hipError_t dmlc_fc_chain_check(const DmlcFcArgs* a, const DmlcConv2DgradArgs* dg);
+hipError_t dmlc_wgrad_check(const DmlcWgradArgs* a);
+#define DMLC_HAND_WORDS (2 * 256 * 32)
+hipError_t dmlc_backward(const DmlcFcArgs* a, const DmlcConv2DgradArgs* dg, const DmlcWgradArgs* w,
+                         unsigned int* hand, hipStream_t s);
 hipError_t dmlc_head(const DmlcHeadArgs* a, hipStream_t s);
 hipError_t dmlc_sgd(DmlcSgdArgs* a, hipStream_t s);
 
diff --git a/csrc/kernels/cnn_bwd.hip b/csrc/kernels/cnn_bwd.hip
--- /dev/null
+++ b/csrc/kernels/cnn_bwd.hip
@@ -0,0 +1,79 @@
+#define DMLC_FC_BODY_ONLY
+#define DMLC_WGRAD_BODY_ONLY
+#include "cnn_fc.hip"
+#include "cnn_wgrad.hip"
+
+namespace dmlc {
+
+static_assert(kWtStores, "dY2 / dP1 are handed off inside the launch: write-through stores only");
+constexpr size_t BWD_LDS = (size_t)FC_LDS_ALL > WG_LDS ? (size_t)FC_LDS_ALL : WG_LDS;
+static_assert(BWD_LDS + 64 <= 160 * 1024, "k_backward: one workgroup per CU");
+
+constexpr unsigned ka_align(unsigned off, unsigned al) { return (off + al - 1) / al * al; }
+constexpr unsigned KA_DG = kernarg_second<DmlcFcArgs, DmlcConv2DgradArgs>();
+constexpr unsigned KA_WG = ka_align(KA_DG + sizeof(DmlcConv2DgradArgs), alignof(DmlcWgradArgs));
+constexpr unsigned KA_HAND = ka_align(KA_WG + sizeof(DmlcWgradArgs), alignof(unsigned*));
+static_assert(KA_HAND + sizeof(unsigned*) <= 4096, "k_backward: the kernarg segment stays under 4 KB");
+
+DEV int bwd_role(int blk, int g1) {
+#ifdef DMLC_BWD_IDENTITY_MAP
+  return blk;
+#else
+  const int n2 = FC_BLOCKS - g1;
+  return blk < n2 ? g1 + blk : blk - n2;
+#endif
+}
+
+__global__ __launch_bounds__(FT, 1) void k_backward(DmlcFcArgs a, DmlcConv2DgradArgs dg, DmlcWgradArgs wa,
+                                                    unsigned* hand) {
+  extern __shared__ __attribute__((aligned(16))) char smem[];
+  __shared__ unsigned s_gen[2];
+  const int tid = threadIdx.x, blk = blockIdx.x;
+  const int64_t step = *a.step;
+  auto late_fc = [&]() __attribute__((always_inline)) -> const DmlcFcArgs& { return late_kernarg<DmlcFcArgs>(0); };
+  auto late_wg = [&]() __attribute__((always_inline)) -> const DmlcWgradArgs& {
+    return late_kernarg<DmlcWgradArgs>(KA_WG);
+  };
+  const unsigned epoch = fc_chain_phase<true>(a, late_fc, step, smem);
+  const DmlcFcArgs& L = late_fc();
+  const DmlcConv2DgradArgs& D = late_kernarg<DmlcConv2DgradArgs>(KA_DG);
+  const Hand h = {late_kernarg<unsigned*>(KA_HAND), epoch + 1u, L.err};
+  if (tid == 0) {
+    const DmlcWgradArgs& W = late_wg();
+    unsigned g0 = 0, hg0 = 0;
+    wgrad_gens(W, bwd_role(blk, W.w1.g1), g0, hg0);
+    s_gen[0] = g0;
+    s_gen[1] = hg0;
+  }
+  if (blk < D.B) conv2_dgrad_image<true>(D, blk, smem, seamD(L, epoch, blk >> 6), L.err, h);
+  if (blk < a.B / FC_RB) DMLC_STAMP(DMLC_TK_HEAD, 7);
+  else DMLC_STAMP(DMLC_TK_GEMM, 6);
+  const DmlcWgradArgs& W = late_wg();
+  unsigned g0 = 0, hg0 = 0;
+  if (tid == 0) { g0 = s_gen[0]; hg0 = s_gen[1]; }
+  wgrad_role<true>(W, late_wg, bwd_role(blk, W.w1.g1), smem, g0, hg0, step, h);
+}
+
+}
+
+using namespace dmlc;
+
+extern "C" hipError_t dmlc_backward(const DmlcFcArgs* a, const DmlcConv2DgradArgs* dg, const DmlcWgradArgs* w,
+                                    unsigned int* hand, hipStream_t s) {
+  if (!dg || !hand) return hipErrorInvalidValue;
+  hipError_t e = dmlc_fc_chain_check(a, dg);
+  if (e == hipSuccess) e = dmlc_wgrad_check(w);
+  if (e != hipSuccess) return e;
+  const DmlcSgdArgs& g = w->sgd;
+  if (dg->split || a->B <= 128 || a->fuse_sgd != 2 || !a->dw_tasks || !a->step || a->grad_bf16) return hipErrorInvalidValue;
+  if (!w->apply || g.mode != 0 || w->fc_in_launch || !w->fc_done || g.w2f8 || w->w2.x8 || g.grad16)
+    return hipErrorInvalidValue;
+  if (w->w1.g1 + 4 * w->w2.g2 != FC_BLOCKS || w->w1.g1 % 8 || w->w2.g2 % 8 || w->w1.g1 > a->B) return hipErrorInvalidValue;
+  if (w->w1.B != a->B || w->w2.B != a->B || g.step != a->step || w->bar + 10 * 32 != a->err) return hipErrorInvalidValue;
+  if (w->w1.dp1 != dg->dp1 || w->w2.dy2 != dg->dy2 || g.w2d != dg->wd || g.loss_part != a->loss_part ||
+      g.correct_part != a->correct_part || g.nhead != a->B / FC_RB)
+    return hipErrorInvalidValue;
+  DMLC_LDS_OPTIN(&k_backward, BWD_LDS);
+  hipLaunchKernelGGL(k_backward, dim3(FC_BLOCKS), dim3(FT), BWD_LDS, s, *a, *dg, *w, hand);
+  return hipGetLastError();
+}
diff --git a/csrc/kernels/cnn_fc.hip b/csrc/kernels/cnn_fc.hip
--- a/csrc/kernels/cnn_fc.hip
+++ b/csrc/kernels/cnn_fc.hip
@@ -6,13 +6,13 @@
 
 namespace dmlc {
 
-constexpr int W2_LD = 384, H1_LD = 392, H2_LD = 200, DL_LD = 40;
+constexpr int HW2_LD = 384, H1_LD = 392, H2_LD = 200, DL_LD = 40;
 DEV int w2swz(int row, int col) {
-  return row * W2_LD + (((col >> 3) ^ (2 * (row & 3) + 8 * ((row >> 3) & 1))) << 3) + (col & 7);
+  return row * HW2_LD + (((col >> 3) ^ (2 * (row & 3) + 8 * ((row >> 3) & 1))) << 3) + (col & 7);
 }
 struct HL {
   static constexpr int W2 = 0;
-  static constexpr int H1 = W2 + 192 * W2_LD * 2;
+  static constexpr int H1 = W2 + 192 * HW2_LD * 2;
   static constexpr int H2 = H1 + (FC_RB + 1) * H1_LD * 2;
   static constexpr int DH2 = H2 + (FC_RB + 1) * H2_LD * 2;
   static constexpr int DL = DH2 + (FC_RB + 1) * H2_LD * 2;
@@ -91,6 +91,7 @@
                (float)h[2] > 0.f ? acc[2] : 0.f, (float)h[3] > 0.f ? acc[3] : 0.f);
 }
 
+template <bool WT = false>
 DEV void head_task(const DmlcFcArgs& a, int hb, char* smem, int tid) {
   bf16* w2s = reinterpret_cast<bf16*>(smem + HL::W2);
   bf16* h1s = reinterpret_cast<bf16*>(smem + HL::H1);
@@ -229,8 +230,13 @@
     }
     const float ls = wave_sum(rowok ? loss : 0.f), cs = wave_sum(corr);
     if (lane == 0) {
-      a.loss_part[hb] = ls;
-      a.correct_part[hb] = (int)(cs + 0.5f);
+      if constexpr (WT) {
+        st_sc1(buf_rsrc(a.loss_part), (uint32_t)hb * 4, ls);
+        st_sc1(buf_rsrc(a.correct_part), (uint32_t)hb * 4, __builtin_bit_cast(float, (int)(cs + 0.5f)));
+      } else {
+        a.loss_part[hb] = ls;
+        a.correct_part[hb] = (int)(cs + 0.5f);
+      }
     }
   }
   lds_barrier();
@@ -286,26 +292,17 @@
   DMLC_STAMP(DMLC_TK_HEAD, 5);
 }
 
-
-#ifdef DMLC_EAGER_ARGS
-#define late_fc() a
-#define late_dg() dg
-#else
-#define late_fc() late_kernarg<DmlcFcArgs>(0)
-#define late_dg() late_kernarg<DmlcConv2DgradArgs>(kernarg_second<DmlcFcArgs, DmlcConv2DgradArgs>())
-#endif
-__global__ __launch_bounds__(FT, 1) void k_fc_chain(DmlcFcArgs a, DmlcConv2DgradArgs dg) {
-  extern __shared__ __attribute__((aligned(16))) char smem[];
+template <bool WT, class LateFc>
+DEV unsigned fc_chain_phase(const DmlcFcArgs& a, LateFc late_fc, const int64_t step, char* smem) {
   const int tid = threadIdx.x, blk = blockIdx.x;
   const int H = a.B / FC_RB;
-  const int64_t step = a.step ? *a.step : 0;
   const int parity = (int)(step & 1);
   if (blk == 0 && tid == 0 && a.step_copy) *a.step_copy = step;
   __shared__ unsigned s_epoch;
   unsigned e0 = 0;
   if (tid == 0) e0 = ld_relaxed(epochW(a));
   if (blk < H) {
-    head_task(a, blk, smem, tid);
+    head_task<WT>(a, blk, smem, tid);
     if (tid == 0) s_epoch = e0;
     const DmlcFcArgs& L = late_fc();
     const int G = FC_BLOCKS - H, nc = ctask_count(L);
@@ -355,6 +352,25 @@
       __hip_atomic_store(epochW(L), epoch + 1, __ATOMIC_RELAXED, __HIP_MEMORY_SCOPE_AGENT);
     }
   }
+  return epoch;
+}
+
+#ifndef DMLC_FC_BODY_ONLY
+#ifdef DMLC_EAGER_ARGS
+#define late_fc() a
+#define late_dg() dg
+#else
+#define late_fc() late_kernarg<DmlcFcArgs>(0)
+#define late_dg() late_kernarg<DmlcConv2DgradArgs>(kernarg_second<DmlcFcArgs, DmlcConv2DgradArgs>())
+#endif
+__global__ __launch_bounds__(FT, 1) void k_fc_chain(DmlcFcArgs a, DmlcConv2DgradArgs dg) {
+  extern __shared__ __attribute__((aligned(16))) char smem[];
+  const int blk = blockIdx.x;
+  const int H = a.B / FC_RB;
+  const int64_t step = a.step ? *a.step : 0;
+  const unsigned epoch = fc_chain_phase<false>(
+      a, [&]() __attribute__((always_inline)) -> const DmlcFcArgs& { return late_fc(); }, step, smem);
+  const DmlcFcArgs& L = late_fc();
   const DmlcConv2DgradArgs& D = late_dg();
   if (D.split) {
     if (blk < 2 * D.B) {
@@ -373,15 +389,12 @@
 
 using namespace dmlc;
 
-extern "C" hipError_t dmlc_fc_chain(const DmlcFcArgs* a, const DmlcConv2DgradArgs* dg, hipStream_t s) {
+extern "C" hipError_t dmlc_fc_chain_check(const DmlcFcArgs* a, const DmlcConv2DgradArgs* dg) {
   if (a->B < 16 || a->B > 256 || a->B % 16 != 0 || a->mtiles != (a->B + 63) / 64 || !a->sync || !a->err)
     return hipErrorInvalidValue;
-  DmlcConv2DgradArgs d;
-  memset(&d, 0, sizeof(d));
   if (dg) {
     if (dg->B != a->B || dg->dp2 != a->dp2 || !dg->am2 || !dg->wd || !dg->dp1 || !dg->dy2) return hipErrorInvalidValue;
     if (dg->split && (2 * dg->B > FC_BLOCKS || dg->B % 8)) return hipErrorInvalidValue;
-    d = *dg;
   }
   static int cus = 0;
   if (!cus) {
@@ -390,7 +403,19 @@
       return hipErrorInvalidValue;
   }
   if (cus < FC_BLOCKS) return hipErrorInvalidValue;
+  return hipSuccess;
+}
+
+extern "C" hipError_t dmlc_fc_chain(const DmlcFcArgs* a, const DmlcConv2DgradArgs* dg, hipStream_t s) {
+  const hipError_t e = dmlc_fc_chain_check(a, dg);
+  if (e != hipSuccess) return e;
+  DmlcConv2DgradArgs d;
+  memset(&d, 0, sizeof(d));
+  if (dg) d = *dg;
   DMLC_LDS_OPTIN(&k_fc_chain, FC_LDS_ALL);
   hipLaunchKernelGGL(k_fc_chain, dim3(FC_BLOCKS), dim3(FT), d.B ? FC_LDS_ALL : FC_LDS, s, *a, d);
   return hipGetLastError();
 }
+#else
+}
+#endif
diff --git a/csrc/kernels/cnn_wgrad.hip b/csrc/kernels/cnn_wgrad.hip
--- a/csrc/kernels/cnn_wgrad.hip
+++ b/csrc/kernels/cnn_wgrad.hip
@@ -7,7 +7,9 @@
 constexpr size_t W1_LDS = (size_t)(W1_DYT + W1_XS + 9216) * 2 + 3072 + 9216;
 static_assert(W1_FL_BYTES <= (W1_DYT + W1_XS) * 2, "flush buffer over dY1 + planes");
 
-DEV void conv1_wgrad_block(const DmlcConv1WgradArgs& a, const int grp, char* smem, bool coh = false) {
+template <bool INL = false>
+DEV void conv1_wgrad_block(const DmlcConv1WgradArgs& a, const int grp, char* smem, bool coh = false,
+                           Hand hand = Hand{nullptr, 0u, nullptr}) {
   bf16* dyt = reinterpret_cast<bf16*>(smem);
   bf16* xs = dyt + W1_DYT;
   bf16* dps = xs + W1_XS;
@@ -29,18 +31,50 @@
 
   const int cI = tid % 192, cD2 = 1024 + (tid & 127), cA1 = 512 + (tid & 63);
   uint4 vI, vD0, vD1, vD2, vA0, vA1;
-  auto load = [&](int idx, int bb) {
+  auto load_free = [&](int idx, int bb) {
     const uint4* si = reinterpret_cast<const uint4*>(a.xraw ? a.xraw + (size_t)bb * 3072 : a.data + (size_t)idx * 3072);
-    const uint4* sd = reinterpret_cast<const uint4*>(reinterpret_cast<const bf16*>(a.dp1) + (size_t)bb * 9216);
     const uint4* sa = reinterpret_cast<const uint4*>(a.am1 + (size_t)bb * 9216);
     vI = si[cI];
-    vD0 = sd[tid]; vD1 = sd[tid + 512]; vD2 = sd[cD2];
     vA0 = sa[tid]; vA1 = sa[cA1];
   };
+  auto load_dp1 = [&](int bb) {
+    if constexpr (INL) {
+      const rsrc_t r = buf_rsrc(a.dp1);
+      const uint32_t o = (uint32_t)bb * 18432u;
+      vD0 = ld16(r, o + 16u * tid); vD1 = ld16(r, o + 16u * (tid + 512)); vD2 = ld16(r, o + 16u * cD2);
+    } else {
+      const uint4* sd = reinterpret_cast<const uint4*>(reinterpret_cast<const bf16*>(a.dp1) + (size_t)bb * 9216);
+      vD0 = sd[tid]; vD1 = sd[tid + 512]; vD2 = sd[cD2];
+    }
+  };
+  auto load = [&](int idx, int bb) {
+    if constexpr (INL) {
+      load_free(idx, bb);
+      load_dp1(bb);
+    } else {
+      const uint4* si = reinterpret_cast<const uint4*>(a.xraw ? a.xraw + (size_t)bb * 3072 : a.data + (size_t)idx * 3072);
+      const uint4* sd = reinterpret_cast<const uint4*>(reinterpret_cast<const bf16*>(a.dp1) + (size_t)bb * 9216);
+      const uint4* sa = reinterpret_cast<const uint4*>(a.am1 + (size_t)bb * 9216);
+      vI = si[cI];
+      vD0 = sd[tid]; vD1 = sd[tid + 512]; vD2 = sd[cD2];
+      vA0 = sa[tid]; vA1 = sa[cA1];
+    }
+  };
   auto row_index = [&](int bb) { return a.xraw ? 0 : batch_index(a.src, a.B, bb); };
-  load(row_index(b0 < last ? b0 : last), b0 < last ? b0 : last);
+  if constexpr (INL) {
+    const int bf = b0 < last ? b0 : last;
+    load_free(row_index(bf), bf);
+    if (tid == 0 && b0 < a.B) hand_wait(hand, bf, HAND_DP1);
+    lds_barrier();
+    load_dp1(bf);
+  } else {
+    load(row_index(b0 < last ? b0 : last), b0 < last ? b0 : last);
+  }
   int nidx = row_index(b0 + G < last ? b0 + G : last);
   for (int b = b0; b < a.B; b += G) {
+    if constexpr (INL) {
+      if (tid == 0 && b + G <= last) hand_wait(hand, b + G, HAND_DP1);
+    }
     lds_barrier();
     reinterpret_cast<uint4*>(img)[cI] = vI;
     reinterpret_cast<uint4*>(dps)[tid] = vD0;
@@ -210,7 +244,9 @@
   for (int j = 0; j < 8; ++j) bsum[j] = c4 == 0 && tid < 8 ? btile[8 * tid + j] : 0.f;
 }
 
-DEV void conv2_wgrad_block(const DmlcConv2WgradArgs& a, const int blk, const int base, char* smem, bool coh = false) {
+template <bool INL = false>
+DEV void conv2_wgrad_block(const DmlcConv2WgradArgs& a, const int blk, const int base, char* smem, bool coh = false,
+                           Hand hand = Hand{nullptr, 0u, nullptr}) {
   bf16* xt = reinterpret_cast<bf16*>(smem);
   bf16* dyt = xt + W2_XT;
   const int tid = threadIdx.x, lane = tid & 63, w = wave_id();
@@ -234,12 +270,24 @@
   bf16* xdst = xt + ((xy + 2) * 16 + pxl - xy * 12 + 2) * W2_LDX + 8 * (kx & 1);
   const int kd[3] = {tid, tid + 512, 1024 + (tid & 127)};
   uint4 vx, vd[3];
+  auto load_x = [&](int b) {
+    const uint4* x = reinterpret_cast<const uint4*>(reinterpret_cast<const bf16*>(a.p1) + (size_t)b * 9216);
+    vx = x[pxl * 8 + 2 * c4 + (kx & 1)];
+  };
+  auto load_dy = [&](int b) {
+    if constexpr (INL) {
+      const rsrc_t r = buf_rsrc(a.dy2);
+#pragma unroll
+      for (int i = 0; i < 3; ++i) vd[i] = ld16(r, (uint32_t)b * 18432u + 16u * kd[i]);
+    } else {
+      const uint4* d = reinterpret_cast<const uint4*>(reinterpret_cast<const bf16*>(a.dy2) + (size_t)b * 9216);
+#pragma unroll
+      for (int i = 0; i < 3; ++i) vd[i] = d[kd[i]];
+    }
+  };
   auto load = [&](int b) {
-    const uint4* x = reinterpret_cast<const uint4*>(reinterpret_cast<const bf16*>(a.p1) + (size_t)b * 9216);
-    const uint4* d = reinterpret_cast<const uint4*>(reinterpret_cast<const bf16*>(a.dy2) + (size_t)b * 9216);
-    vx = x[pxl * 8 + 2 * c4 + (kx & 1)];
-#pragma unroll
-    for (int i = 0; i < 3; ++i) vd[i] = d[kd[i]];
+    load_x(b);
+    load_dy(b);
   };
 
   int xa[5], xb[5];
@@ -254,8 +302,19 @@
   for (int j = 0; j < 3; ++j) toff[j] = ((3 * w + j) / 5 * 16 + (3 * w + j) % 5) * W2_LDX;
   constexpr int T24 = (4 * 16 + 4) * W2_LDX;
 
-  load(b0 < last ? b0 : last);
+  if constexpr (INL) {
+    const int bf = b0 < last ? b0 : last;
+    load_x(bf);
+    if (tid == 0 && b0 < a.B) hand_wait(hand, bf, HAND_DY2);
+    lds_barrier();
+    load_dy(bf);
+  } else {
+    load(b0 < last ? b0 : last);
+  }
   for (int b = b0; b < a.B; b += G) {
+    if constexpr (INL) {
+      if (tid == 0 && b + G <= last) hand_wait(hand, b + G, HAND_DY2);
+    }
     lds_barrier();
     *reinterpret_cast<uint4*>(xdst) = vx;
 #pragma unroll
@@ -432,7 +491,9 @@
 }
 DEV unsigned* w2_claim(const DmlcWgradArgs& A, int c4, int grp) { return A.bar + 11 * 32 + c4 * A.w2.g2 + grp; }
 
-DEV void conv2_apply(const DmlcWgradArgs& A, int c4, int grp, char* smem, unsigned g0, int64_t step) {
+template <bool INL = false>
+DEV void conv2_apply(const DmlcWgradArgs& A, int c4, int grp, char* smem, unsigned g0, int64_t step,
+                     Hand hand = Hand{nullptr, 0u, nullptr}) {
   const DmlcSgdArgs& s = A.sgd;
   const int tid = threadIdx.x, n = A.w2.g2;
   int* flag = reinterpret_cast<int*>(smem);
@@ -441,6 +502,9 @@
   if (tid == 0) {
     bar_arrive(wbar(A.bar, 2 + c4), wbar(A.bar, 6 + c4), g0, (unsigned)n);
     bar_wait(wbar(A.bar, 6 + c4), g0, wbar(A.bar, 10));
+  }
+  if constexpr (INL) {
+    if (tid >= 64 && tid < 128) hand_wait_all(hand, HAND_DP1, A.w2.B, tid - 64);
   }
   __syncthreads();
   DMLC_STAMP(DMLC_TK_W2, 6);
@@ -496,6 +560,7 @@
   __syncthreads();
   if (threadIdx.x == 0) bar_arrive(wbar(A.bar, 0), wbar(A.bar, 1), g0, (unsigned)A.w1.g1);
 }
+template <bool INL = false>
 DEV void conv1_apply(const DmlcWgradArgs& A, int grp, char* smem, unsigned g0, int64_t step, bool arrived = false) {
   const DmlcSgdArgs& s = A.sgd;
   const int tid = threadIdx.x, n = A.w1.g1;
@@ -508,15 +573,19 @@
     fc_role(s, r, lr, step, lds, tid);
     lds_barrier();
   }
-  if (s.mode == 0 && grp == 0 && tid < 64) publish_step(s, step, lr, tid);
-  if (s.mode == 0 && s.bidx) {
-    const int r = grp * W1T + tid;
-    if (r < s.bidx_n) s.bidx[r] = order_row(s.next, step + 1, r);
-  }
+  auto finish_step = [&]() __attribute__((always_inline)) {
+    if (s.mode == 0 && grp == 0 && tid < 64) publish_step<INL>(s, step, lr, tid);
+    if (s.mode == 0 && s.bidx) {
+      const int r = grp * W1T + tid;
+      if (r < s.bidx_n) s.bidx[r] = order_row(s.next, step + 1, r);
+    }
+  };
+  if constexpr (!INL) finish_step();
   DMLC_STAMP(DMLC_TK_SGD, 0);
   if (tid == 0) bar_wait(wbar(A.bar, 1), g0, wbar(A.bar, 10));
   __syncthreads();
   DMLC_STAMP(DMLC_TK_SGD, 1);
+  if constexpr (INL) finish_step();
   const int per = (1200 + n - 1) / n, ol = tid & 15, sp = tid >> 4;
   const rsrc_t part1 = buf_rsrc(A.w1.part1);
   for (int f0 = 0; f0 < per; f0 += 16) {
@@ -555,65 +624,82 @@
   DMLC_STAMP(DMLC_TK_SGD, 2);
 }
 
-#ifdef DMLC_EAGER_ARGS
-#define late_args() a
-#else
-#define late_args() late_kernarg<DmlcWgradArgs>(0)
-#endif
-
 constexpr size_t WG_LDS = W1_LDS > W2_LDS ? W1_LDS : W2_LDS;
 static_assert(WG_LDS >= W8_LDS, "the fp8 conv2 body's double buffer fits the launch's LDS");
 static_assert(WG_LDS >= (size_t)L_RED + 8 * 64 * 4 && WG_LDS >= 40960 + 64 * 136 * 2,
               "the fc dW tiles reuse the weight-gradient launch's LDS");
 static_assert(W1T == FT, "the fc dW tiles run with the weight-gradient launch's block size");
 static_assert(WG_LDS >= SGD_LDS4 * 16, "apply mode reuses the block's LDS for the SGD roles");
-__global__ __launch_bounds__(W1T, 1) void k_wgrad(DmlcWgradArgs a) {
-  extern __shared__ __attribute__((aligned(16))) char smem[];
-  const bool conv1 = (int)blockIdx.x < a.w1.g1;
+static_assert(W1T == W2T, "both bodies run with one block size");
+
+DEV void wgrad_gens(const DmlcWgradArgs& a, int vb, unsigned& g0, unsigned& hg0) {
+  const bool conv1 = vb < a.w1.g1;
   int c4 = 0, grp = 0;
-  if (!conv1) w2_block_pos(a.w2, blockIdx.x - a.w1.g1, a.w1.g1, c4, grp);
-  unsigned g0 = 0, hg0 = 0;
-  int64_t step = 0;
-  const bool helper = a.apply && conv1 && w2_helpers(a) && (int)blockIdx.x < 4 * a.w2.g2;
-  if (a.apply) {
-    if (threadIdx.x == 0) g0 = bar_gen(wbar(a.bar, conv1 ? 1 : 6 + c4));
-    if (helper && threadIdx.x == 0) {
-      int hc4, hgrp;
-      w2_block_pos(a.w2, blockIdx.x, a.w1.g1, hc4, hgrp);
-      hg0 = bar_gen(wbar(a.bar, 6 + hc4));
-    }
-    step = *a.sgd.step_rd;
-  }
+  if (!conv1) w2_block_pos(a.w2, vb - a.w1.g1, a.w1.g1, c4, grp);
+  const bool helper = a.apply && conv1 && w2_helpers(a) && vb < 4 * a.w2.g2;
+  g0 = bar_gen(wbar(a.bar, conv1 ? 1 : 6 + c4));
+  if (helper) {
+    int hc4, hgrp;
+    w2_block_pos(a.w2, vb, a.w1.g1, hc4, hgrp);
+    hg0 = bar_gen(wbar(a.bar, 6 + hc4));
+  }
+}
+
+template <bool INL, class LateArgs>
+DEV void wgrad_role(const DmlcWgradArgs& a, LateArgs late_args, const int vb, char* smem, unsigned g0, unsigned hg0,
+                    const int64_t step, Hand hand = Hand{nullptr, 0u, nullptr}) {
+  const bool conv1 = vb < a.w1.g1;
+  int c4 = 0, grp = 0;
+  if (!conv1) w2_block_pos(a.w2, vb - a.w1.g1, a.w1.g1, c4, grp);
+  const bool helper = a.apply && conv1 && w2_helpers(a) && vb < 4 * a.w2.g2;
   if (conv1) {
-    conv1_wgrad_block(a.w1, blockIdx.x, smem, a.apply != 0);
+    conv1_wgrad_block<INL>(a.w1, vb, smem, a.apply != 0, hand);
     const DmlcWgradArgs& L = late_args();
-    if (a.apply && L.fc_in_launch) {
+    if (!INL && a.apply && L.fc_in_launch) {
       const int parity = (int)(step & 1);
-      if (blockIdx.x >= FC_DW_TASKS) conv1_arrive(L, g0);
-      for (int d = blockIdx.x; d < FC_DW_TASKS; d += L.w1.g1) {
+      if (vb >= FC_DW_TASKS) conv1_arrive(L, g0);
+      for (int d = vb; d < FC_DW_TASKS; d += L.w1.g1) {
         const CTask T = dw_ctask(d);
         PreRegs R;
         pre_issue(L.fc, T, parity, R, threadIdx.x);
-        const bool first = d == (int)blockIdx.x;
+        const bool first = d == vb;
         dw_task<false>(L.fc, T, R, step, smem, threadIdx.x, [&]() {
           if (first) conv1_arrive(L, g0);
         });
       }
       DMLC_STAMP(DMLC_TK_SGD, 3);
-      conv1_apply(L, blockIdx.x, smem, g0, step, true);
+      conv1_apply(L, vb, smem, g0, step, true);
     } else if (a.apply) {
-      conv1_apply(L, blockIdx.x, smem, g0, step);
-    }
-    if (helper) conv2_help(L, blockIdx.x, smem, hg0, step);
+      conv1_apply<INL>(L, vb, smem, g0, step);
+    }
+    if (helper) conv2_help(L, vb, smem, hg0, step);
     if (a.apply && L.sgd.mode == 0 && L.sgd.xnext)
-      for (int r = blockIdx.x; r < L.sgd.bidx_n; r += L.w1.g1) copy_next_row(L.sgd, step, r, threadIdx.x);
+      for (int r = vb; r < L.sgd.bidx_n; r += L.w1.g1) copy_next_row(L.sgd, step, r, threadIdx.x);
     DMLC_STAMP(DMLC_TK_SGD, 4);
   } else {
-    conv2_wgrad_block(a.w2, blockIdx.x - a.w1.g1, a.w1.g1, smem, a.apply != 0);
-    if (a.apply) conv2_apply(late_args(), c4, grp, smem, g0, step);
-  }
-}
-static_assert(W1T == W2T, "k_wgrad runs both bodies with one block size");
+    conv2_wgrad_block<INL>(a.w2, vb - a.w1.g1, a.w1.g1, smem, a.apply != 0, hand);
+    if (a.apply) conv2_apply<INL>(late_args(), c4, grp, smem, g0, step, hand);
+  }
+}
+
+#ifndef DMLC_WGRAD_BODY_ONLY
+#ifdef DMLC_EAGER_ARGS
+#define late_args() a
+#else
+#define late_args() late_kernarg<DmlcWgradArgs>(0)
+#endif
+
+__global__ __launch_bounds__(W1T, 1) void k_wgrad(DmlcWgradArgs a) {
+  extern __shared__ __attribute__((aligned(16))) char smem[];
+  unsigned g0 = 0, hg0 = 0;
+  int64_t step = 0;
+  if (a.apply) {
+    if (threadIdx.x == 0) wgrad_gens(a, blockIdx.x, g0, hg0);
+    step = *a.sgd.step_rd;
+  }
+  wgrad_role<false>(a, [&]() __attribute__((always_inline)) -> const DmlcWgradArgs& { return late_args(); },
+                    blockIdx.x, smem, g0, hg0, step);
+}
 
 }
 
@@ -621,9 +707,7 @@
 
 extern "C" {
 
-hipError_t dmlc_wgrad(const DmlcWgradArgs* a, hipStream_t s) {
-  DMLC_LDS_OPTIN(&k_wgrad, WG_LDS);
-  const int blocks = a->w1.g1 + 4 * a->w2.g2;
+hipError_t dmlc_wgrad_check(const DmlcWgradArgs* a) {
   if (a->apply) {
     static int cus = 0;
     if (!cus) {
@@ -643,8 +727,19 @@
         g.part2 != a->w2.part2 || g.g1 != a->w1.g1 || g.g2 != a->w2.g2 || g.bidx_n > a->w1.g1 * W1T)
       return hipErrorInvalidValue;
   }
+  return hipSuccess;
+}
+
+hipError_t dmlc_wgrad(const DmlcWgradArgs* a, hipStream_t s) {
+  DMLC_LDS_OPTIN(&k_wgrad, WG_LDS);
+  const int blocks = a->w1.g1 + 4 * a->w2.g2;
+  const hipError_t e = dmlc_wgrad_check(a);
+  if (e != hipSuccess) return e;
   hipLaunchKernelGGL(k_wgrad, dim3(blocks), dim3(W1T), WG_LDS, s, *a);
   return hipGetLastError();
 }
 
 }
+#else
+}
+#endif
diff --git a/csrc/kernels/common.h b/csrc/kernels/common.h
--- a/csrc/kernels/common.h
+++ b/csrc/kernels/common.h
@@ -194,6 +194,40 @@
     if (__all(ok)) break;
     if (it >= DMLC_SPIN_LIMIT) {
       if (lane == 0) __hip_atomic_fetch_or(err, errbit, __ATOMIC_RELAXED, __HIP_MEMORY_SCOPE_AGENT);
+      break;
+    }
+    __builtin_amdgcn_s_sleep(1);
+  }
+}
+
+constexpr int HAND_DY2 = 0, HAND_DP1 = 1;
+struct Hand { unsigned* w; unsigned gen; unsigned* err; };
+DEV unsigned* hand_word(const Hand& h, int b, int k) { return h.w + 32 * (2 * b + k); }
+DEV void hand_post(const Hand& h, int b, int k) {
+  __hip_atomic_store(hand_word(h, b, k), h.gen, __ATOMIC_RELAXED, __HIP_MEMORY_SCOPE_AGENT);
+}
+DEV void hand_wait(const Hand& h, int b, int k) {
+  unsigned* p = hand_word(h, b, k);
+  for (unsigned it = 0; __hip_atomic_load(p, __ATOMIC_RELAXED, __HIP_MEMORY_SCOPE_AGENT) != h.gen; ++it) {
+    if (it >= DMLC_SPIN_LIMIT) {
+      __hip_atomic_fetch_or(h.err, 4u, __ATOMIC_RELAXED, __HIP_MEMORY_SCOPE_AGENT);
+      break;
+    }
+    __builtin_amdgcn_s_sleep(1);
+  }
+}
+DEV void hand_wait_all(const Hand& h, int k, int B, int lane) {
+  for (unsigned it = 0;; ++it) {
+    bool ok = true;
+#pragma unroll
+    for (int u = 0; u < 4; ++u) {
+      const int b = lane + 64 * u;
+      const unsigned v = __hip_atomic_load(hand_word(h, b < B ? b : 0, k), __ATOMIC_RELAXED, __HIP_MEMORY_SCOPE_AGENT);
+      ok = ok && (b >= B || v == h.gen);
+    }
+    if (__all(ok)) break;
+    if (it >= DMLC_SPIN_LIMIT) {
+      if (lane == 0) __hip_atomic_fetch_or(h.err, 4u, __ATOMIC_RELAXED, __HIP_MEMORY_SCOPE_AGENT);
       break;
     }
     __builtin_amdgcn_s_sleep(1);
diff --git a/csrc/kernels/conv2_core.h b/csrc/kernels/conv2_core.h
--- a/csrc/kernels/conv2_core.h
+++ b/csrc/kernels/conv2_core.h
@@ -34,7 +34,8 @@
 
 template <bool EXTRA>
 DEV void conv2_core(const bf16* Wg, const bf16* xin, bf16* ws, f32x4 (&acc)[2][2], f32x4& accx, int pg, int cp,
-                    int xsel, int g, int li, int tid, const bf16* s0, int tk = -1) {
+                    int xsel, int g, int li, int tid, const bf16* s0, int tk = -1, unsigned* post = nullptr,
+                    unsigned post_gen = 0u) {
   constexpr int NPX = EXTRA ? 3 : 2;
   const int w = wave_id(), lane = tid & 63, sw = li & 7;
   int xo[NPX][8][2];
@@ -56,7 +57,9 @@
   accx = zero4();
   if (!s0) ws_dma(Wg, 0, ws, w, lane);
   const bf16* sb0 = s0 ? s0 : ws;
+  if (post) wait_vm_all();
   __syncthreads();
+  if (post && tid == 0) __hip_atomic_store(post, post_gen, __ATOMIC_RELAXED, __HIP_MEMORY_SCOPE_AGENT);
   auto load_chunk = [&](int kh, int j, bf16x8& a0, bf16x8& a1, bf16x8 (&bx)[NPX]) {
     const int kw = j >> 1, s = j & 1;
     const bf16* wr = slice_buf(sb0, ws, kh) + kw * 64 + ao[s];
@@ -93,14 +96,14 @@
 
 template <class F>
 DEV void conv2_tiles(const bf16* Wg, const bf16* xin, bf16* ws, int w, int g, int li, int tid, const bf16* s0,
-                     F&& fn, int tk = -1) {
+                     F&& fn, int tk = -1, unsigned* post = nullptr, unsigned post_gen = 0u) {
   const int cp = w & 1, pg = w >> 1;
   f32x4 acc[2][2], accx;
   if (w < 4) {
-    conv2_core<true>(Wg, xin, ws, acc, accx, pg, cp, pg, g, li, tid, s0, tk);
+    conv2_core<true>(Wg, xin, ws, acc, accx, pg, cp, pg, g, li, tid, s0, tk, post, post_gen);
     fn(2 * cp + pg, 8, accx);
   } else {
-    conv2_core<false>(Wg, xin, ws, acc, accx, pg, cp, 0, g, li, tid, s0, tk);
+    conv2_core<false>(Wg, xin, ws, acc, accx, pg, cp, 0, g, li, tid, s0, tk, post, post_gen);
   }
 #pragma unroll
   for (int t = 0; t < 2; ++t) { fn(2 * cp, pg + 4 * t, acc[0][t]); fn(2 * cp + 1, pg + 4 * t, acc[1][t]); }
@@ -110,7 +113,7 @@
 
 template <bool IN_LAUNCH>
 DEV void conv2_dgrad_image(const DmlcConv2DgradArgs& a, int b, char* smem, Seam seam = Seam{nullptr, 0, 0u},
-                           unsigned* err = nullptr) {
+                           unsigned* err = nullptr, Hand hand = Hand{nullptr, 0u, nullptr}) {
   bf16* dyp = reinterpret_cast<bf16*>(smem);
   bf16* outs = dyp + C2_XIN;
   bf16* dp2 = outs + C2_OUT;
@@ -166,7 +169,7 @@
     const int px = 16 * t + li, cb = 16 * ct + 4 * g;
     const bf16x4 v = pack4(acc[0], acc[1], acc[2], acc[3]);
     *reinterpret_cast<bf16x4*>(outs + swz128(px, cb >> 3) + ((cb >> 2) & 1) * 4) = v;
-  });
+  }, -1, hand.w ? hand_word(hand, b, HAND_DY2) : nullptr, hand.gen);
   __syncthreads();
   DMLC_STAMP(DMLC_TK_DGRAD, 3);
   bf16* dp1 = reinterpret_cast<bf16*>(a.dp1) + (size_t)b * 9216;
@@ -175,6 +178,11 @@
     st_out16(dp1, (uint32_t)(p * 64 + c * 8) * 2, __builtin_bit_cast(uint4, lds_b128(outs + swz128(p, c))));
   }
   DMLC_STAMP(DMLC_TK_DGRAD, 4);
+  if (hand.w) {
+    wait_vm_all();
+    __syncthreads();
+    if (tid == 0) hand_post(hand, b, HAND_DP1);
+  }
 }
 
 }
diff --git a/csrc/kernels/sgd_common.h b/csrc/kernels/sgd_common.h
--- a/csrc/kernels/sgd_common.h
+++ b/csrc/kernels/sgd_common.h
@@ -215,9 +215,18 @@
       reinterpret_cast<const uint4*>(a.xdata + (size_t)src * 3072)[tid];
 }
 
+template <bool COH = false>
 DEV void publish_step(const DmlcSgdArgs& a, int64_t step, float lr, int lane) {
   float loss = 0.f, corr = 0.f;
-  for (int q = lane; q < a.nhead; q += 64) { loss += a.loss_part[q]; corr += (float)a.correct_part[q]; }
+  for (int q = lane; q < a.nhead; q += 64) {
+    if constexpr (COH) {
+      loss += __builtin_bit_cast(float, __builtin_amdgcn_raw_buffer_load_b32(buf_rsrc(a.loss_part), (uint32_t)q * 4, 0, kSC1));
+      corr += (float)(int)__builtin_amdgcn_raw_buffer_load_b32(buf_rsrc(a.correct_part), (uint32_t)q * 4, 0, kSC1);
+    } else {
+      loss += a.loss_part[q];
+      corr += (float)a.correct_part[q];
+    }
+  }
   loss = wave_sum(loss);
   corr = wave_sum(corr);
   if (lane == 0) {
diff --git a/distributed-machine-learning-using-cnn-cifar-10-dataset-_amd/_build.py b/distributed-machine-learning-using-cnn-cifar-10-dataset-_amd/_build.py
--- a/distributed-machine-learning-using-cnn-cifar-10-dataset-_amd/_build.py
+++ b/distributed-machine-learning-using-cnn-cifar-10-dataset-_amd/_build.py
@@ -97,10 +97,12 @@
         if TIMING:
             hip_flags += ["-DDMLC_TIMING", "-fgpu-rdc"]
         hip_flags += VARIANT_FLAGS
+        hip_includes = {"cnn_bwd.hip": ["cnn_fc.hip", "cnn_wgrad.hip"]}
         for src in sorted(glob.glob(os.path.join(CSRC, "kernels", "*.hip"))):
             o = os.path.join(OBJ_DIR, os.path.basename(src) + (f"{_SUFFIX.replace('_', '.')}.o" if _SUFFIX else ".o"))
             hip_objs.append(o)
-            jobs_list.append((src, headers, o, [hipcc], hip_flags))
+            deps = headers + [os.path.join(CSRC, "kernels", d) for d in hip_includes.get(os.path.basename(src), [])]
+            jobs_list.append((src, deps, o, [hipcc], hip_flags))
         bheaders = headers + glob.glob(os.path.join(CSRC, "bindings", "*.h"))
         for bsrc in sorted(glob.glob(os.path.join(CSRC, "bindings", "*.cpp"))):
             o = os.path.join(OBJ_DIR, os.path.basename(bsrc) + ".o")
diff --git a/distributed-machine-learning-using-cnn-cifar-10-dataset-_amd/engine/fused.py b/distributed-machine-learning-using-cnn-cifar-10-dataset-_amd/engine/fused.py
--- a/distributed-machine-learning-using-cnn-cifar-10-dataset-_amd/engine/fused.py
+++ b/distributed-machine-learning-using-cnn-cifar-10-dataset-_amd/engine/fused.py
@@ -45,9 +45,11 @@
     "fwd12_split": True,
     "fc_sgd_in_chain": None,
     "grad16": True,
+    "bwd_fused": None,
 }
 TICKET_WORDS = 9 * 32
 WBAR_WORDS = 20 * 32
+HAND_WORDS = 2 * 256 * 32
 SEG = {M.short(s.name): s for s in M.PARAM_SPECS}
 
 
@@ -247,6 +249,15 @@
         fsc = V["fc_sgd_in_chain"]
         self.fc_sgd_in_chain = (self.fc_fused and self.wgrad_apply and not self.fc_dw_in_wgrad
                                 and (bool(fsc) if fsc is not None else B < 256))
+        bwf = V["bwd_fused"]
+        bwd_ok = (self.fc_fused and self.fc_dgrad and 128 < B <= 256 and self.dgrad_split == 1
+                  and self.wgrad_apply and not self.fc_dw_in_wgrad and not self.fp8 and world_size == 1
+                  and self.xraw_prefetch and fsc is not False and self.g1 + 4 * self.g2 == 256
+                  and self.g1 % 8 == 0 and self.g2 % 8 == 0)
+        self.bwd_fused = bool(bwd_ok and (bool(bwf) if bwf is not None else True))
+        if self.bwd_fused:
+            self.fc_sgd_in_chain = True
+        self.bwd_hand = torch.zeros(HAND_WORDS if self.bwd_fused else 1, dtype=torch.int32, device=dev)
         self._fc_bwd_sgd = dict(fb, C=[fb["C"][0], p["full_weight_1"]] + fb["C"][2:],
                                 params=fb["params"][:14] + _gemm_params(2304, 384, B, 2304, 0, 384, 0, 384, 4,
                                                                         s_par=FC1_NUMEL)
@@ -361,6 +372,10 @@
             raise RuntimeError("_fc_chain must follow a training _forward")
         if self._dgrad_done:
             raise RuntimeError("the previous fc chain's conv backward never ran")
+        self.ops.fc_chain(*self._fc_chain_args(fused_sgd))
+        self._dgrad_done = self.fc_dgrad
+
+    def _fc_chain_args(self, fused_sgd: bool) -> tuple:
         idx, counter, period = self._fc_src
         self._fc_src = None
         p, gv = self.pv, self.gv
@@ -369,17 +384,27 @@
         if not fused_sgd:
             gv = self.gv_chain
         g = p if all_sgd else gv
-        self.ops.fc_chain(self.p2.view(self.B, 2304), self.fc1n, self.h1part8, p["full_bias_1"], self.fc2t,
-                          p["full_bias_2"], self.fc3t, p["full_bias_3"], self.fc3d, self.labels, idx, counter, period,
-                          1.0 / (self.Bv * self.world_size), self.relu_logits, self.h1, self.h2, self.dl, self.dh1,
-                          self.dh2, self.loss_part, self.correct_part, self.dp2.view(self.B, 2304),
-                          p["full_weight_1"] if fused_sgd else gv["full_weight_1"], g["full_weight_2"],
-                          g["full_weight_3"], g["full_bias_1"], g["full_bias_2"], g["full_bias_3"], fused_sgd,
-                          sched, self.Bv, self.step_t, self.step_sgd, self.fc_sync, self.wbar[10 * 32:10 * 32 + 1],
-                          not (fused_sgd and self.fc_dw_in_wgrad),
-                          *((self.am2, self.w2d, self.dp1, self.dy2) if self.fc_dgrad else (None, None, None, None)),
-                          self.fc2n if all_sgd else None)
-        self._dgrad_done = self.fc_dgrad
+        return (self.p2.view(self.B, 2304), self.fc1n, self.h1part8, p["full_bias_1"], self.fc2t,
+                p["full_bias_2"], self.fc3t, p["full_bias_3"], self.fc3d, self.labels, idx, counter, period,
+                1.0 / (self.Bv * self.world_size), self.relu_logits, self.h1, self.h2, self.dl, self.dh1,
+                self.dh2, self.loss_part, self.correct_part, self.dp2.view(self.B, 2304),
+                p["full_weight_1"] if fused_sgd else gv["full_weight_1"], g["full_weight_2"],
+                g["full_weight_3"], g["full_bias_1"], g["full_bias_2"], g["full_bias_3"], fused_sgd,
+                sched, self.Bv, self.step_t, self.step_sgd, self.fc_sync, self.wbar[10 * 32:10 * 32 + 1],
+                not (fused_sgd and self.fc_dw_in_wgrad),
+                *((self.am2, self.w2d, self.dp1, self.dy2) if self.fc_dgrad else (None, None, None, None)),
+                self.fc2n if all_sgd else None)
+
+    def _backward_fused(self):
+        if self._fc_src is None:
+            raise RuntimeError("_backward_fused must follow a training _forward")
+        if self._dgrad_done:
+            raise RuntimeError("the previous fc chain's conv backward never ran")
+        fc = self._fc_chain_args(True)
+        self.ops.backward_fused_wgrad(self.data, self.bidx, None, 1, self.cy, self.cx, self.dp1, self.am1,
+                                      self.p1, self.dy2, self.groups2, self.xraw, self.wbar,
+                                      *self._sgd_args(mode=0, fc1_fused=True), fc_acts=None, fc_sgd_done=True)
+        self.ops.backward_fused(self.bwd_hand, *fc)
 
     def _conv_backward(self, src=None, apply: bool = False, reduce: bool = False):
         o = self.ops
@@ -443,6 +468,9 @@
             if e & 2:
                 parts.append("k_fc_chain / k_conv12_fwd_split: a hand-off wait timed out; rerun with "
                              "DMLC_FC_FUSED=0 / DMLC_FWD12_SPLIT=0")
+            if e & 4:
+                parts.append("k_backward: a per-image dY2 / dP1 hand-off wait timed out; rerun with the engine "
+                             "variant bwd_fused=0")
             if self.fwd12_split:
                 self.c12_flags.zero_()
             raise RuntimeError("; ".join(parts) + f" (blocks not co-resident, error word {e})")
@@ -562,6 +590,9 @@
         if not self.dp:
             if self.fc1_epilogue:
                 self._forward(self.bidx, None, 1, train=True)
+                if self.bwd_fused:
+                    self._backward_fused()
+                    return
                 self._fc_backward(fused_sgd=True)
                 if self.wgrad_apply:
                     self._conv_backward(apply=True)
```

Result: faster. 3.798 million images/sec, median of 6 (+5.2%).
